# Cibiv/NextGenMap

Measured on AMD Instinct MI355X. Metric: mapped reads/sec + SW Gcells/sec, 150bp vs GRCh38, at 1/2/4/8 MI355X, higher is better.
Workload: dtype int32

## Files before the change

### include/ngm_pipeline.h

```cpp
#ifndef NGM_PIPELINE_H
#define NGM_PIPELINE_H

#include <stddef.h>
#include <stdint.h>

#ifdef __cplusplus
extern "C" {
#endif

typedef struct ngm_ref ngm_ref;
typedef struct ngm_mapper ngm_mapper;

typedef struct ngm_ref_params {
	int kmer;
	int kmer_skip;
	int bin_size;
} ngm_ref_params;

const char *ngm_pipeline_last_error(void);

ngm_ref *ngm_ref_create(int device, const ngm_ref_params *p, int n_contigs, const char *const *names,
		const uint8_t *const *seqs, const uint64_t *lens);
ngm_ref *ngm_ref_create_from_fasta(int device, const ngm_ref_params *p, const char *path);
ngm_ref *ngm_ref_create_from_cache(int device, const ngm_ref_params *params, const char *fasta_path);
// ... 150 lines not shown
int ngm_coverage_finish(ngm_coverage *c);
long long ngm_coverage_next(ngm_coverage *c, void *out, size_t out_cap);
int ngm_coverage_stats(const ngm_coverage *c, uint64_t counts[4], float ms[4]);
int ngm_mapper_set_coverage(ngm_mapper *m, ngm_coverage *c);

typedef struct ngm_snp ngm_snp;
typedef struct ngm_snp_params {
	int device;
	int n_ref;
	const uint32_t *ref_len;
	const char *const *ref_name;
	const char *const *ref_seq;
	uint32_t min_cov;
	double min_frac;
	int min_qual;
	const char *min_frac_text;
	size_t scan_chunk;
} ngm_snp_params;
ngm_snp *ngm_snp_create(const ngm_snp_params *p);
ngm_snp *ngm_snp_create_for_ref(const ngm_ref *r, const ngm_snp_params *p);
void ngm_snp_destroy(ngm_snp *s);
int ngm_snp_add(ngm_snp *s, const int32_t *ref_id, const int32_t *pos0, const uint32_t *cigar_off , const char *cigar_text,
                const uint32_t *seq_off , const char *seq_text, const char *qual_text, size_t n);
int ngm_snp_finish(ngm_snp *s);
long long ngm_snp_next(ngm_snp *s, void *out, size_t out_cap);
int ngm_snp_stats(const ngm_snp *s, uint64_t counts[5], float ms[4]);
int ngm_mapper_set_snp(ngm_mapper *m, ngm_snp *s);

void *ngm_host_alloc(size_t bytes);
void ngm_host_free(void *p);

int ngm_host_pin_to_device_node(int device);

int ngm_mapper_set_reference_score_buffer(ngm_mapper *m, int entries);
int ngm_mapper_lost_pairs(ngm_mapper *m, uint64_t *out);
int ngm_mapper_set_reference_cs_batch(ngm_mapper *m, int reads);

int ngm_mapper_path_counters(ngm_mapper *m, uint64_t out[8]);

int ngm_mapper_order_table_reads(ngm_mapper *m, uint64_t *out);

int ngm_debug_pair_walk(uint32_t cnt_a, int len_a, uint32_t cnt_b, int len_b, const uint32_t *loc, const uint32_t *sv, const float *score, const uint32_t *rank,
		float cutoff, int min_insert, int max_insert, uint32_t *out_a, uint32_t *out_b, int *mq_a, int *mq_b, uint64_t cap, float *combo_score, int *combo_dist, int *combo_a, int *combo_b,
		uint64_t *n_combo);

int ngm_debug_pair_eval(uint64_t n, const float *pair_score, const int *dist, const int *ia, const int *ib, int avg, int out_all[6], int out_kept[6]);

int ngm_debug_select_top1(int device, int n_reads, const uint32_t *base, const uint32_t *count, uint64_t n_cand, const float *scores, const uint32_t *loc,
		const uint32_t *strand_votes, uint32_t *winner, int32_t *mapq, int32_t *n_best, float *best_score);

int ngm_debug_align_finish(void *engine , int mode, int n, const char *const *ref, const char *const *qry, void *out ,
		uint64_t *n_fallback);

int ngm_debug_expand_pairs(int device, int n_reads, const uint32_t *base, const uint32_t *count, uint64_t n_cand, uint32_t *out);

int ngm_debug_pair_select(int device, int n_pairs, const uint32_t *base, const uint32_t *count, uint64_t n_cand, const float *scores, const uint32_t *loc,
		const uint16_t *read_len, int min_insert, int max_insert, float cutoff, int32_t *info, int32_t *mapq, int32_t *n_best, uint32_t counts[4], void *entries, void *tops);

int ngm_mapper_heavy_counters(ngm_mapper *m, uint64_t out[4]);

int ngm_mapper_search_turn_counters(ngm_mapper *m, uint64_t out[3]);

int ngm_mapper_cs_counters(ngm_mapper *m, uint64_t out[3]);

typedef struct ngm_stats_comm ngm_stats_comm;
int ngm_stats_unique_id(char hex[257]);
ngm_stats_comm *ngm_stats_comm_create(int device, int rank, int world, const char *hex);
int ngm_stats_allreduce(ngm_stats_comm *c, int64_t v[8]);
void ngm_stats_comm_destroy(ngm_stats_comm *c);
int ngm_mapper_last_pair_stats(ngm_mapper *m, uint64_t out[3]);

int ngm_mapper_last_kernel_ms(ngm_mapper *m, float ms[8]);
float ngm_mapper_last_order_replay_ms(ngm_mapper *m);

int ngm_mapper_set_argos(ngm_mapper *m, float min_score);
long long ngm_mapper_map_argos(ngm_mapper *m, int n, const char *reads, const char *names, size_t names_bytes, const ngm_sam_read *meta,
		char *out, size_t out_cap, uint64_t stats[3], float *kernel_ms);
int ngm_argos_prolog(const ngm_ref *ref, uint64_t total_reads, char *out, size_t cap);
int ngm_mapper_argos_counters(ngm_mapper *m, uint64_t out[4]);
int ngm_mapper_argos_path_counters(ngm_mapper *m, uint64_t out[2]);
int ngm_debug_argos_order(uint32_t n, const float *score, const uint32_t *rank, float min_score, int read_len, int match_bonus, uint32_t *order, uint32_t out[3]);

#ifdef __cplusplus
}
#endif
#endif
```

### nextgenmap_amd/csrc/affine_device.h

```cpp
#pragma once

#include <hip/hip_runtime.h>
#include <stdint.h>

#include "sw_device.h"

namespace ngm {

struct AffConst {
	int tM;
	int tZ;
	int open;
	int ext;
	int vopen;
	int vext;
};

constexpr int kAffNeg = -(1 << 28);
__host__ __device__ constexpr int aff_dir_words(int CP) { return (CP + 3) / 4; }

enum { kTDiag = 1, kTHori = 2, kTVert = 4, kTHoriOpen = 8, kTVertOpen = 16, kTMaxH = 32, kTMaxV = 64 };

__device__ __forceinline__ uint2 aff_row_table(int rc, const AffConst &K) {
	uint32_t b[8];
// ... 108 lines not shown
					tr = none ? 0u : tr;
					dw[d >> 2] |= tr << (8 * (d & 3));
				}
				const int key = ((sc - fl) << 8) | (255 - d);
				if (!ENDFREE) {
					if (key > rowkey) { rowkey = key; rowflags = ((ev == sc) ? 1 : 0) | ((eh == sc) ? 2 : 0); }
				}
				if (ENDFREE && ALIGN) ehq[d >> 5] |= (eh == sc) ? (1u << (d & 31)) : 0u;
				S[d] = sc;
				Ev[d] = ev;
				leftS = sc;
				leftEh = eh;
			}
			if (ALIGN && i < q) {
#pragma unroll
				for (int w = 0; w < DW; ++w) dout[((size_t) i * DW + w) * kSlots] = dw[w];
			}
			if (!ENDFREE) {
				const int rs = rowkey >> 8, rd_ = 255 - (rowkey & 255), rh = i + 1 + rd_;
				if (i < lenV && (rs > best || (rs == best && rs > 0 && rh < bh))) { best = rs; bh = rh; bv = i + 1; bflags = rowflags; }
			} else if (i + 1 == lenV) {
				const int dlim = lenH - lenV;
				const int kv = -fl;
#pragma unroll
				for (int d = 0; d < CP; ++d) {
					const int v = S[d] + kv;
					if (d <= dlim && v > best) {
						best = v; bh = lenV + d; bv = lenV;
						bflags = ((Ev[d] == S[d]) ? 1 : 0) | ((ALIGN && ((ehq[d >> 5] >> (d & 31)) & 1u)) ? 2 : 0);
					}
				}
			}
			fl += K.tZ;
		}
#pragma unroll
		for (int r = 0; r + 2 < NRG; ++r) RG[r] = RG[r + 2];
		RG[NRG - 2] = fx & 0x0F0F0F0Fu;
		RG[NRG - 1] = (fx >> 4) & 0x0F0F0F0Fu;
	}

	if (pair < n) {
		if (lenV < 1 || lenH < 1) { best = 0; bh = bv = 0; bflags = 0; }
		if (!ALIGN) {
			scores[pair] = (float) best;
		} else {
			int32_t *rec = records + (size_t) pair * 8;
			rec[0] = 0; rec[1] = 0; rec[2] = 0; rec[3] = bflags; rec[4] = 0; rec[5] = best; rec[6] = bh; rec[7] = bv;
		}
	}
}

constexpr int kAffNeg16 = -20000;

template <int CP, bool ENDFREE>
__global__ __launch_bounds__(256) void sw_affine_score_pk_kernel(const uint32_t *__restrict__ packed, const uint16_t *__restrict__ lens,
		const uint16_t *__restrict__ blk_rows, float *__restrict__ scores, int n, int n_blocks, int RW, AffConst K) {
	__shared__ uint2 s_tab[8];
	if (threadIdx.x < 8) s_tab[threadIdx.x] = aff_row_table(threadIdx.x, K);
	__syncthreads();
	const int lane = threadIdx.x & 63;
	const int blkA = 2 * (blockIdx.x * 4 + (threadIdx.x >> 6));
	if (blkA >= n_blocks) return;
	const bool hasB = blkA + 1 < n_blocks;
	const int blkB = hasB ? blkA + 1 : blkA;
	constexpr int NRG = sel_regs(CP);
	const int FW = RW + NRG / 2;
	const uint32_t *rdA = packed + (size_t) blkA * (RW + FW) * kSlots + lane, *rdB = packed + (size_t) blkB * (RW + FW) * kSlots + lane;
	const uint32_t *fdA = rdA + (size_t) RW * kSlots, *fdB = rdB + (size_t) RW * kSlots;
	const int pairA = blkA * kSlots + lane, pairB = blkB * kSlots + lane;
	const int lenVA = (pairA < n) ? (int) lens[pairA] : 0, lenVB = (pairB < n) ? (int) lens[pairB] : 0;
	const int rows = max(__builtin_amdgcn_readfirstlane((int) blk_rows[blkA]), __builtin_amdgcn_readfirstlane((int) blk_rows[blkB]));
	const int ngroups = (rows + 7) >> 3;

	auto window_len = [&](const uint32_t *fd) {
		int len = FW * 8;
		for (int m = FW - 1; m >= 0; --m) {
			const uint32_t x = fd[(size_t) m * kSlots];
			const uint32_t lo = x & 0x0F0F0F0Fu, hi = (x >> 4) & 0x0F0F0F0Fu;
#pragma unroll
			for (int j = 7; j >= 0; --j) {
				const uint32_t cls = (j < 4) ? (lo >> (8 * j)) & 15u : (hi >> (8 * (j - 4))) & 15u;
				if (cls == 6u) len = m * 8 + j;
			}
		}
		return len;
	};
	const int lenHA = ENDFREE ? window_len(fdA) : FW * 8, lenHB = ENDFREE ? window_len(fdB) : FW * 8;

	v2s S[CP], Ev[CP];
#pragma unroll
	for (int d = 0; d < CP; ++d) { S[d] = pk_splat(0); Ev[d] = pk_splat(ENDFREE ? kAffNeg16 : 0); }
	uint32_t RGA[NRG], RGB[NRG];
#pragma unroll
	for (int r = 0; r < NRG / 2; ++r) {
		const uint32_t xa = fdA[(size_t) r * kSlots], xb = fdB[(size_t) r * kSlots];
		RGA[2 * r] = xa & 0x0F0F0F0Fu; RGA[2 * r + 1] = (xa >> 4) & 0x0F0F0F0Fu;
		RGB[2 * r] = xb & 0x0F0F0F0Fu; RGB[2 * r + 1] = (xb >> 4) & 0x0F0F0F0Fu;
	}
	int fl = K.tZ;
	v2s best2 = pk_splat(0);
	int bestA = kAffNeg, bestB = kAffNeg;
	const v2s ext2 = pk_splat(K.ext), open2 = pk_splat(K.open), vext2 = pk_splat(K.vext), vopen2 = pk_splat(K.vopen);
	const v2s neg2 = pk_splat(kAffNeg16), one2 = pk_splat(1), zero2 = pk_splat(0);
	uint32_t rnA = (ngroups > 0) ? rdA[0] : 0x66666666u, rnB = (ngroups > 0) ? rdB[0] : 0x66666666u;

	for (int g = 0; g < ngroups; ++g) {
		const uint32_t rxA = rnA, rxB = rnB;
		rnA = (g + 1 < ngroups) ? rdA[(size_t) (g + 1) * kSlots] : 0x66666666u;
		rnB = (g + 1 < ngroups) ? rdB[(size_t) (g + 1) * kSlots] : 0x66666666u;
		const uint32_t fxA = fdA[(size_t) (g + NRG / 2) * kSlots], fxB = fdB[(size_t) (g + NRG / 2) * kSlots];
		const uint32_t rsA[2] = {rxA & 0x0F0F0F0Fu, (rxA >> 4) & 0x0F0F0F0Fu}, rsB[2] = {rxB & 0x0F0F0F0Fu, (rxB >> 4) & 0x0F0F0F0Fu};
#pragma unroll
		for (int s = 0; s < 8; ++s) {
			const int i = g * 8 + s;
			uint32_t rcA = (rsA[s >> 2] >> (8 * (s & 3))) & 0xFFu, rcB = (rsB[s >> 2] >> (8 * (s & 3))) & 0xFFu;
			rcA = (i < lenVA) ? rcA : 6u;
			rcB = (i < lenVB) ? rcB : 6u;
			const uint2 TA = s_tab[rcA], TB = s_tab[rcB];
			uint32_t PA[NRG], PB[NRG];
#pragma unroll
			for (int r = 0; r < NRG; ++r) {
				const bool used = (s + CP - 1) / 4 >= r && s / 4 <= r;
				PA[r] = used ? __builtin_amdgcn_perm(TA.y, TA.x, RGA[r]) : 0u;
				PB[r] = used ? __builtin_amdgcn_perm(TB.y, TB.x, RGB[r]) : 0u;
			}
			const v2s fl2 = pk_splat(fl);
			v2s leftS = neg2, leftEh = neg2;
			v2s rowmax = fl2;
#pragma unroll
			for (int d = 0; d < CP; ++d) {
				const int bi = s + d, kb = bi & 3;
				const uint32_t sel = 0x0C000C00u | (uint32_t) kb | ((uint32_t) (4 + kb) << 16);
				const v2s t = __builtin_bit_cast(v2s, __builtin_amdgcn_perm(PB[bi >> 2], PA[bi >> 2], sel));
				const v2s dg = S[d] + t;
				v2s eh = (d == 0) ? neg2 : pk_max(leftEh + ext2, leftS + open2);
				v2s ev = (d < CP - 1) ? pk_max(Ev[d + 1] + vext2, S[d + 1] + vopen2) : neg2;
				v2s sc = pk_max(pk_max(ev, eh), dg);
				if (!ENDFREE) {
					sc = pk_max(sc, fl2);
					rowmax = pk_max(rowmax, sc);
				}
				S[d] = sc;
				Ev[d] = ev;
				leftS = sc;
				leftEh = eh;
			}
			if (!ENDFREE) {
				best2 = pk_max(best2, rowmax - fl2);
			} else if (i + 1 == lenVA || i + 1 == lenVB) {
				const int kv = -fl;
				if (i + 1 == lenVA) {
					const int dlim = lenHA - lenVA;
#pragma unroll
					for (int d = 0; d < CP; ++d) { const int v = (int) S[d].x + kv; if (d <= dlim && v > bestA) bestA = v; }
				}
				if (i + 1 == lenVB) {
					const int dlim = lenHB - lenVB;
#pragma unroll
					for (int d = 0; d < CP; ++d) { const int v = (int) S[d].y + kv; if (d <= dlim && v > bestB) bestB = v; }
				}
			}
			fl += K.tZ;
		}
#pragma unroll
		for (int r = 0; r + 2 < NRG; ++r) { RGA[r] = RGA[r + 2]; RGB[r] = RGB[r + 2]; }
		RGA[NRG - 2] = fxA & 0x0F0F0F0Fu; RGA[NRG - 1] = (fxA >> 4) & 0x0F0F0F0Fu;
		RGB[NRG - 2] = fxB & 0x0F0F0F0Fu; RGB[NRG - 1] = (fxB >> 4) & 0x0F0F0F0Fu;
	}
	if (!ENDFREE) { bestA = best2.x; bestB = best2.y; }
	if (pairA < n) { if (lenVA < 1 || lenHA < 1) bestA = 0; scores[pairA] = (float) bestA; }
	if (hasB && pairB < n) { if (lenVB < 1 || lenHB < 1) bestB = 0; scores[pairB] = (float) bestB; }
}

template <int CP>
__global__ __launch_bounds__(256) void sw_affine_score_pk_split_kernel(const uint32_t *__restrict__ packed, const uint16_t *__restrict__ lens,
		const uint16_t *__restrict__ blk_rows, float *__restrict__ scores, int n, int n_blocks, int RW, AffConst K) {
	__shared__ uint2 s_tab[8];
	if (threadIdx.x < 8) s_tab[threadIdx.x] = aff_row_table(threadIdx.x, K);
	__syncthreads();
	constexpr int CL = ((CP + 1) / 2 + 6) / 8 * 8 + 1;
	constexpr int CR = CP - CL;
	static_assert(CR >= 1 && CR <= CL, "band too narrow to split");
	constexpr int NRG = sel_regs(CL);
	constexpr int WOFF = (CL - 1) / 8;
	const int lane = threadIdx.x & 63;
	const bool isR = (lane & 1) != 0;
	const int unit = blockIdx.x * 4 + (threadIdx.x >> 6);
	const int blkA = 2 * (unit >> 1);
	if (blkA >= n_blocks) return;
	const bool hasB = blkA + 1 < n_blocks;
	const int blkB = hasB ? blkA + 1 : blkA;
	const int slot = (lane >> 1) + 32 * (unit & 1);
	const int FW = RW + sel_regs(CP) / 2;
	const uint32_t *rdA = packed + (size_t) blkA * (RW + FW) * kSlots + slot, *rdB = packed + (size_t) blkB * (RW + FW) * kSlots + slot;
	const uint32_t *fdA = rdA + (size_t) RW * kSlots, *fdB = rdB + (size_t) RW * kSlots;
	const int pairA = blkA * kSlots + slot, pairB = blkB * kSlots + slot;
	const int lenVA = (pairA < n) ? (int) lens[pairA] : 0, lenVB = (pairB < n) ? (int) lens[pairB] : 0;
	const int rows = max(__builtin_amdgcn_readfirstlane((int) blk_rows[blkA]), __builtin_amdgcn_readfirstlane((int) blk_rows[blkB]));
	const int ngroups = (rows + 7) >> 3, ngroups2 = (rows + 1 + 7) >> 3;
	const int woff = isR ? WOFF : 0;
	auto swap2 = [](v2s x) -> v2s { return __builtin_bit_cast(v2s, __builtin_amdgcn_update_dpp(0, __builtin_bit_cast(int, x), 0xB1, 0xf, 0xf, false)); };

	v2s S[CL], Ev[CL];
#pragma unroll
	for (int d = 0; d < CL; ++d) { S[d] = pk_splat(0); Ev[d] = pk_splat(0); }
	uint32_t RGA[NRG], RGB[NRG];
#pragma unroll
	for (int r = 0; r < NRG / 2; ++r) {
		const int w = min(r + woff, FW - 1);
		const uint32_t xa = fdA[(size_t) w * kSlots], xb = fdB[(size_t) w * kSlots];
		RGA[2 * r] = xa & 0x0F0F0F0Fu; RGA[2 * r + 1] = (xa >> 4) & 0x0F0F0F0Fu;
		RGB[2 * r] = xb & 0x0F0F0F0Fu; RGB[2 * r + 1] = (xb >> 4) & 0x0F0F0F0Fu;
	}
	int fl = K.tZ;
	const int rz = isR ? K.tZ : 0;
	v2s best2 = pk_splat(0);
	const v2s ext2 = pk_splat(K.ext), open2 = pk_splat(K.open), vext2 = pk_splat(K.vext), vopen2 = pk_splat(K.vopen);
	const v2s neg2 = pk_splat(kAffNeg16), zero2 = pk_splat(0);
	v2s saveS = neg2, saveEh = neg2;
	uint32_t prevA = 6u, prevB = 6u;
	uint32_t rnA = (ngroups > 0) ? rdA[0] : 0x66666666u, rnB = (ngroups > 0) ? rdB[0] : 0x66666666u;

// ... 21 lines not shown
				PB[r] = used ? __builtin_amdgcn_perm(TB.y, TB.x, RGB[r]) : 0u;
			}
			const v2s fl2 = pk_splat(fl - rz);
			const v2s gotS = swap2(saveS), gotEh = swap2(saveEh);
			v2s leftS = isR ? gotS : neg2, leftEh = isR ? gotEh : neg2;
			v2s nxS = neg2, nxEv = neg2;
			v2s rowmax = fl2;
#pragma unroll
			for (int d = 0; d < CL; ++d) {
				const int bi = s + d, kb = bi & 3;
				const uint32_t sel = 0x0C000C00u | (uint32_t) kb | ((uint32_t) (4 + kb) << 16);
				const v2s t = __builtin_bit_cast(v2s, __builtin_amdgcn_perm(PB[bi >> 2], PA[bi >> 2], sel));
				const v2s dg = S[d] + t;
				const v2s eh = pk_max(leftEh + ext2, leftS + open2);
				v2s ev = (d < CL - 1) ? pk_max(Ev[d + 1] + vext2, S[d + 1] + vopen2) : pk_max(nxEv + vext2, nxS + vopen2);
				v2s sc = pk_max(pk_max(pk_max(ev, eh), dg), fl2);
				if (d >= CR) { sc = isR ? neg2 : sc; ev = isR ? neg2 : ev; }
				rowmax = pk_max(rowmax, sc);
				S[d] = sc;
				Ev[d] = ev;
				leftS = sc;
				leftEh = eh;
				if (d == 0) {
					v2s xS = swap2(sc), xEv = swap2(ev);
					if (s == 0 && g == 0) { xS = zero2; xEv = zero2; }
					nxS = isR ? neg2 : xS; nxEv = isR ? neg2 : xEv;
				}
				if (d == CL - 1) { saveS = sc; saveEh = eh; }
			}
			best2 = pk_max(best2, rowmax - fl2);
			if (s == 0 && g == 0) {
#pragma unroll
				for (int d = 0; d < CL; ++d) { S[d] = isR ? zero2 : S[d]; Ev[d] = isR ? zero2 : Ev[d]; }
				best2 = isR ? zero2 : best2;
			}
			fl += K.tZ;
		}
#pragma unroll
		for (int r = 0; r + 2 < NRG; ++r) { RGA[r] = RGA[r + 2]; RGB[r] = RGB[r + 2]; }
		RGA[NRG - 2] = fxA & 0x0F0F0F0Fu; RGA[NRG - 1] = (fxA >> 4) & 0x0F0F0F0Fu;
		RGB[NRG - 2] = fxB & 0x0F0F0F0Fu; RGB[NRG - 1] = (fxB >> 4) & 0x0F0F0F0Fu;
	}
	best2 = pk_max(best2, swap2(best2));
	if (isR) return;
	int bestA = best2.x, bestB = best2.y;
	if (pairA < n) { if (lenVA < 1) bestA = 0; scores[pairA] = (float) bestA; }
	if (hasB && pairB < n) { if (lenVB < 1) bestB = 0; scores[pairB] = (float) bestB; }
}

__host__ __device__ constexpr int aff_nib_words(int CP) { return (CP + 7) / 8; }

template <int CP, bool WINDOW>
__global__ __launch_bounds__(256) void sw_affine_align_pk_kernel(const uint32_t *__restrict__ packed, const uint16_t *__restrict__ lens,
		const uint16_t *__restrict__ blk_rows, uint32_t *__restrict__ dirs, int32_t *__restrict__ records, int n, int n_blocks, int RW, int q, AffConst K) {
	static_assert(WINDOW ? CP <= 128 : CP <= 32, "the row key keeps the band column in 7 / 5 bits");
	__shared__ uint2 s_tab[8];
	if (threadIdx.x < 8) s_tab[threadIdx.x] = aff_row_table(threadIdx.x, K);
	__syncthreads();
	const int lane = threadIdx.x & 63;
	const int blkA = 2 * (blockIdx.x * 4 + (threadIdx.x >> 6));
	if (blkA >= n_blocks) return;
	const bool hasB = blkA + 1 < n_blocks;
	const int blkB = hasB ? blkA + 1 : blkA;
	constexpr int NRG = sel_regs(CP);
	constexpr int DW = aff_nib_words(CP);
	const int FW = RW + NRG / 2;
	const uint32_t *rdA = packed + (size_t) blkA * (RW + FW) * kSlots + lane, *rdB = packed + (size_t) blkB * (RW + FW) * kSlots + lane;
	const uint32_t *fdA = rdA + (size_t) RW * kSlots, *fdB = rdB + (size_t) RW * kSlots;
	uint32_t *doutA = dirs + (size_t) blkA * q * DW * kSlots + lane, *doutB = dirs + (size_t) blkB * q * DW * kSlots + lane;
	const int pairA = blkA * kSlots + lane, pairB = blkB * kSlots + lane;
	const int lenVA = (pairA < n) ? (int) lens[pairA] : 0, lenVB = (pairB < n) ? (int) lens[pairB] : 0;
	const int rows = max(__builtin_amdgcn_readfirstlane((int) blk_rows[blkA]), __builtin_amdgcn_readfirstlane((int) blk_rows[blkB]));
	const int ngroups = (rows + 7) >> 3;

	v2s S[CP], Ev[CP];
#pragma unroll
	for (int d = 0; d < CP; ++d) { S[d] = pk_splat(0); Ev[d] = pk_splat(0); }
	uint32_t RGA[NRG], RGB[NRG];
#pragma unroll
	for (int r = 0; r < NRG / 2; ++r) {
		const uint32_t xa = fdA[(size_t) r * kSlots], xb = fdB[(size_t) r * kSlots];
		RGA[2 * r] = xa & 0x0F0F0F0Fu; RGA[2 * r + 1] = (xa >> 4) & 0x0F0F0F0Fu;
		RGB[2 * r] = xb & 0x0F0F0F0Fu; RGB[2 * r + 1] = (xb >> 4) & 0x0F0F0F0Fu;
	}
	int fl = K.tZ;
	int bestA = 0, bhA = 0, bvA = 0, bestB = 0, bhB = 0, bvB = 0;
	const v2s ext2 = pk_splat(K.ext), open2 = pk_splat(K.open), vext2 = pk_splat(K.vext), vopen2 = pk_splat(K.vopen);
	const v2s neg2 = pk_splat(kAffNeg16), one2 = pk_splat(1), zero2 = pk_splat(0), two2 = pk_splat(2), four2 = pk_splat(4), k32 = pk_splat(WINDOW ? 128 : 32);
	const v2s win_lo2 = pk_splat(K.tZ + 1), win_max2 = pk_splat(63);
	v2s prevmax2 = pk_splat(0);
	uint32_t rnA = (ngroups > 0) ? rdA[0] : 0x66666666u, rnB = (ngroups > 0) ? rdB[0] : 0x66666666u;

	for (int g = 0; g < ngroups; ++g) {
		const uint32_t rxA = rnA, rxB = rnB;
		rnA = (g + 1 < ngroups) ? rdA[(size_t) (g + 1) * kSlots] : 0x66666666u;
		rnB = (g + 1 < ngroups) ? rdB[(size_t) (g + 1) * kSlots] : 0x66666666u;
		const uint32_t fxA = fdA[(size_t) (g + NRG / 2) * kSlots], fxB = fdB[(size_t) (g + NRG / 2) * kSlots];
		const uint32_t rsA[2] = {rxA & 0x0F0F0F0Fu, (rxA >> 4) & 0x0F0F0F0Fu}, rsB[2] = {rxB & 0x0F0F0F0Fu, (rxB >> 4) & 0x0F0F0F0Fu};
#pragma unroll
		for (int s = 0; s < 8; ++s) {
			const int i = g * 8 + s;
			uint32_t rcA = (rsA[s >> 2] >> (8 * (s & 3))) & 0xFFu, rcB = (rsB[s >> 2] >> (8 * (s & 3))) & 0xFFu;
			rcA = (i < lenVA) ? rcA : 6u;
			rcB = (i < lenVB) ? rcB : 6u;
			const uint2 TA = s_tab[rcA], TB = s_tab[rcB];
			uint32_t PA[NRG], PB[NRG];
#pragma unroll
			for (int r = 0; r < NRG; ++r) {
// ... 147 lines not shown
```

### nextgenmap_amd/csrc/cigar_device.h

```cpp
#pragma once

#include <hip/hip_runtime.h>
#include <stdint.h>

#include "sw_device.h"
#include "affine_device.h"

namespace ngm {

struct CigarDevOut {
	uint32_t cig_off, md_off;
	uint16_t cig_len, md_len;
	int32_t position_offset, qstart, qend, nm;
	float identity, score_token;
	int32_t flags;
};

__device__ __forceinline__ uint32_t packed_class(const uint32_t *base, int m_base, int j) {
	const uint32_t w = base[(size_t) (m_base + (j >> 3)) * kSlots];
	const int b = j & 7;
	return (b < 4) ? (w >> (8 * b)) & 15u : (w >> (8 * (b - 4) + 4)) & 15u;
}
__device__ __forceinline__ char class_to_char(uint32_t c) {
	switch (c) { case 0: return 'A'; case 1: return 'C'; case 2: return 'G'; case 3: return 'T'; case 4: return 'x'; case 5: return 'N'; default: return 0; }
// ... 108 lines not shown
				if (m_len > 0) { co += dev_put_num(cg + co, m_len); cg[co++] = 'M'; }
				if (trail > 0) {
					if (hard_clip == 1) { co += dev_put_num(cg + co, trail); cg[co++] = 'H'; }
					else if (silent_clip != 1) { co += dev_put_num(cg + co, trail); cg[co++] = 'S'; }
					o.qend = trail;
				}
			}
			o.identity = (float) match * 1.0f / (float) total;
			o.nm = mismatch;
			o.score_token = (float) read_i;
			o.position_offset = ref0;
			o.flags = ((fits && !odd_symbol) ? 1 : 0) | 2;
		}
	}
	}
	o.cig_len = (uint16_t) co; o.md_len = (uint16_t) mo;
	const uint32_t need = (live && (o.flags & 1)) ? (uint32_t) (co + mo) : 0u;
	uint32_t incl = need;
	const int lane = threadIdx.x & 63, wv = threadIdx.x >> 6;
#pragma unroll
	for (int d = 1; d < 64; d <<= 1) { const uint32_t t = __shfl_up(incl, d); if (lane >= d) incl += t; }
	if (lane == 63) s_wave[wv] = incl;
	__syncthreads();
	uint32_t before = incl - need, total = 0;
#pragma unroll
	for (int w2 = 0; w2 < 4; ++w2) { if (w2 < wv) before += s_wave[w2]; total += s_wave[w2]; }
	if (threadIdx.x == 0) s_base = total ? atomicAdd(cursor, (unsigned long long) total) : 0ull;
	__syncthreads();
	const unsigned long long base = s_base;
	if (!live) return;
	if (need) {
		if (base + total > capacity) o.flags &= ~1;
		else {
			const unsigned long long off = base + before;
			o.cig_off = (uint32_t) off; o.md_off = (uint32_t) off + o.cig_len;
			for (int t = 0; t < co; ++t) bytes[off + t] = cg[t];
			for (int t = 0; t < mo; ++t) bytes[off + co + t] = mdp[t];
		}
	}
	out[j] = o;
}

constexpr int kFinishRows = 8;

__device__ __forceinline__ uint32_t finish_sel8(uint32_t w0, uint32_t w1, uint32_t w2, uint32_t w3, uint32_t w4, uint32_t w5, uint32_t w6, uint32_t w7, int k) {
	const uint32_t a0 = (k & 1) ? w1 : w0, a1 = (k & 1) ? w3 : w2, a2 = (k & 1) ? w5 : w4, a3 = (k & 1) ? w7 : w6;
	const uint32_t b0 = (k & 2) ? a1 : a0, b1 = (k & 2) ? a3 : a2;
	return (k & 4) ? b1 : b0;
}

template <bool NIBBLES>
__global__ __launch_bounds__(256) void affine_finish_kernel(int n, const uint32_t *__restrict__ dirs, const int32_t *__restrict__ records,
		const uint32_t *__restrict__ packed, const uint16_t *__restrict__ lens, int q, int CP, int RW, int FW, CigarDevOut *__restrict__ out,
		char *__restrict__ bytes, unsigned long long capacity, unsigned long long *__restrict__ counters) {
	__shared__ char s_rows[256 * kCigarRow];
	__shared__ uint32_t s_wave[4];
	__shared__ unsigned long long s_base;
	const int j = blockIdx.x * blockDim.x + threadIdx.x;
	const bool live = j < n;
	const int lane = threadIdx.x & 63, wv = threadIdx.x >> 6;
	constexpr int lim = kCigarRow - 16;
	constexpr int WS = NIBBLES ? 3 : 2;
	const int DW = NIBBLES ? aff_nib_words(CP) : aff_dir_words(CP);
	char *row = s_rows + (size_t) threadIdx.x * kCigarRow;
	int pos = kCigarRow;
	auto put_back = [&](int num, char tag) {
		row[--pos] = tag;
		unsigned u = (unsigned) num;
		do { row[--pos] = (char) ('0' + u % 10u); u /= 10u; } while (u);
	};
	bool fits = true;
	int h = 0, v = 0, flags = 0, len_v = 0;
	if (live) {
		const int32_t *rec = records + (size_t) j * 8;
		flags = rec[3]; h = rec[6]; v = rec[7];
		len_v = (int) lens[j];
	}
	const int qend = len_v - v;
	if (live && qend > 0) put_back(qend, 'S');
	const int trail = kCigarRow - pos;
	const uint32_t *dp = dirs + (size_t) (j >> 6) * q * DW * kSlots + lane;
	const uint32_t *pk = packed + (size_t) (j >> 6) * (RW + FW) * kSlots + lane;
	int cur = -1, curlen = 0, total = 0, n_match = 0, n_mis = 0;
	bool done = !live, first = true, in_v = false, in_h = false;
	auto flush = [&]() {
		if (cur < 0) return;
		if (kCigarRow - pos - trail > lim) { fits = false; done = true; return; }
		put_back(curlen, cur == 1 ? 'M' : cur == 2 ? 'I' : 'D');
		total += cur == 1 ? curlen : 1;
	};
	auto emit = [&](int op) {
		if (op == cur) { ++curlen; return; }
		flush();
		cur = op; curlen = 1;
	};
	int gtop = (v - 1) >> 3;
#pragma unroll
	for (int s = 1; s < 64; s <<= 1) gtop = max(gtop, __shfl_xor(gtop, s));
	for (int g = gtop; g >= 0; --g) {
		const int r0 = g * kFinishRows;
		const bool act = !done && v - 1 >= r0;
		const int d0 = h - v;
		const int wi = min(max(d0 >> WS, 0), DW - 1);
		const int f0 = min(max((r0 + d0) >> 3, 0), FW - 1);
		uint32_t W[kFinishRows];
#pragma unroll
		for (int k = 0; k < kFinishRows; ++k) W[k] = (act && r0 + k <= v - 1) ? dp[((size_t) (r0 + k) * DW + wi) * kSlots] : 0u;
		const uint32_t rdw = act ? pk[(size_t) g * kSlots] : 0u;
		const uint32_t fw0 = act ? pk[(size_t) (RW + f0) * kSlots] : 0u;
		const uint32_t fw1 = (act && f0 + 1 < FW) ? pk[(size_t) (RW + f0 + 1) * kSlots] : 0u;
// ... 44 lines not shown
					emit(1);
					const int jr = (v - 1) & 7, jf = (h - 1) & 7, fi = (h - 1) >> 3;
					const uint32_t fx = (fi == f0) ? fw0 : (fi == f0 + 1) ? fw1 : pk[(size_t) (RW + fi) * kSlots];
					const uint32_t rc = (rdw >> (4 * ((jr & 3) * 2 + (jr >> 2)))) & 15u, fc = (fx >> (4 * ((jf & 3) * 2 + (jf >> 2)))) & 15u;
					if (rc == fc && rc <= 5u && rc != 4u) ++n_match; else ++n_mis;
					--h; --v;
					continue;
				}
				if ((tv & kTMaxV) && (tv & kTVert)) in_v = true;
				else if ((tv & kTMaxV) && (tv & kTVertOpen)) { emit(2); --v; continue; }
				else if ((tv & kTMaxH) && (tv & kTHori)) in_h = true;
				else if ((tv & kTMaxH) && (tv & kTHoriOpen)) { emit(3); --h; continue; }
				else { done = true; break; }
			}
			if (in_v) { in_v = (!(tv & kTVertOpen) || (tv & kTVert)) && v != 1; emit(2); --v; }
			else { in_h = (!(tv & kTHoriOpen) || (tv & kTHori)) && h != 1; emit(3); --h; }
		}
	}
	int co = 0;
	if (live) {
		if (fits) flush();
		int lead = 0;
		if (v > 0) { lead = 2; for (int t = v; t >= 10; t /= 10) ++lead; }
		if (kCigarRow - pos - trail + lead > lim) fits = false;
		if (fits && v > 0) put_back(v, 'S');
		co = kCigarRow - pos;
	}
	constexpr int mo = 3;
	const uint32_t need = (live && fits) ? (uint32_t) (co + mo) : 0u;
	uint32_t incl = need;
#pragma unroll
	for (int d = 1; d < 64; d <<= 1) { const uint32_t t = __shfl_up(incl, d); if (lane >= d) incl += t; }
	if (lane == 63) s_wave[wv] = incl;
	__syncthreads();
	uint32_t before = incl - need, total_b = 0;
#pragma unroll
	for (int w2 = 0; w2 < 4; ++w2) { if (w2 < wv) before += s_wave[w2]; total_b += s_wave[w2]; }
	if (threadIdx.x == 0) s_base = total_b ? atomicAdd(&counters[0], (unsigned long long) total_b) : 0ull;
	__syncthreads();
	const unsigned long long base = s_base;
	if (!live) return;
	uint32_t cig_off = 0;
	if (need) {
		if (base + total_b > capacity) fits = false;
		else {
			const unsigned long long off = base + before;
			cig_off = (uint32_t) off;
			const char *cg = row + pos;
			for (int t = 0; t < co; ++t) bytes[off + t] = cg[t];
			for (int t = 0; t < mo; ++t) bytes[off + co + t] = '!';
		}
	}
	if (!fits) atomicAdd(&counters[1], 1ull);
	CigarDevOut *o = out + j;
	o->cig_off = cig_off; o->md_off = fits ? cig_off + (uint32_t) co : 0u;
	o->cig_len = (uint16_t) co; o->md_len = (uint16_t) mo;
	o->position_offset = h; o->qstart = v; o->qend = qend; o->nm = n_mis;
	o->identity = (float) n_match * 1.0f / (float) total;
	o->score_token = 0.f;
	o->flags = (fits ? 1 : 0) | 2;
}

}
```

### nextgenmap_amd/csrc/engine_internal.h

```cpp
#pragma once

#include <algorithm>

#include <hip/hip_runtime.h>

#include <cstdint>
#include <string>

#include "../../include/ngm_hip.h"
#include "sw_device.h"
#include "affine_device.h"
#include "cigar_device.h"
#include "jit.h"

namespace ngm {
template <typename T>
struct DevBuf {
	T *p = nullptr;
	size_t cap = 0;
	int reserve(size_t n) {
		if (n <= cap) return 0;
		if (p) (void) hipFree(p);
		p = nullptr;
		cap = 0;
// ... 6 lines not shown
	void release() { if (p) (void) hipFree(p); p = nullptr; cap = 0; }
};

template <typename T>
struct PinnedBuf {
	T *p = nullptr;
	size_t cap = 0;
	int reserve(size_t n) {
		if (n <= cap) return 0;
		if (p) (void) hipHostFree(p);
		p = nullptr;
		cap = 0;
		const size_t want = n + std::min<size_t>(n / 8, ((size_t) 64 << 20) / sizeof(T));
		if (hipHostMalloc(&p, want * sizeof(T), hipHostMallocDefault) == hipSuccess) { cap = want; return 0; }
		if (hipHostMalloc(&p, n * sizeof(T), hipHostMallocDefault) != hipSuccess) return -1;
		cap = n;
		return 0;
	}
	void release() { if (p) (void) hipHostFree(p); p = nullptr; cap = 0; }
};

}

struct ngm_hip_ctx {
	int device = 0;
	ngm_hip_params prm{};
	ngm::SwConst K{};
	ngm::AffConst KA{};
	const ngm::JitKernels *jit = nullptr;
	int q = 0, c = 0, rl = 0, RW = 0, FW = 0;
	int max_batch = 0;
	hipStream_t stream = nullptr;
	ngm::DevBuf<uint32_t> packed;
	ngm::DevBuf<uint16_t> lens, blk_rows;
	ngm::DevBuf<uint8_t> d_ref, d_qry, d_pair_dir;
	const uint8_t *pair_dir = nullptr;
	ngm::DevBuf<float> d_scores;
	ngm::DevBuf<uint32_t> dirs;
	ngm::DevBuf<int32_t> d_records;
	ngm::DevBuf<uint16_t> d_runs;
	ngm::PinnedBuf<uint8_t> h_ref, h_qry;
	ngm::PinnedBuf<float> h_scores;
	ngm::PinnedBuf<int32_t> h_records;
	ngm::PinnedBuf<uint16_t> h_runs;
	bool profiling = false;
	hipEvent_t ev[4] = {nullptr, nullptr, nullptr, nullptr};
	bool ev_valid[3] = {false, false, false};
	bool trace_nibbles = false;
	std::string error;
};

namespace ngm {
int engine_reserve(ngm_hip_ctx *ctx, int n);
int engine_score_packed(ngm_hip_ctx *ctx, int mode, int n, float *d_scores, hipStream_t st);
struct AlignFinish {
	CigarDevOut *out;
	char *bytes;
	unsigned long long capacity;
	unsigned long long *counters;
};
int engine_align_packed(ngm_hip_ctx *ctx, int mode, int n, int32_t *d_records, uint16_t *d_runs, int run_stride, hipStream_t st, const AlignFinish *fin = nullptr);
int engine_affine_traceback_packed(ngm_hip_ctx *ctx, int n, int32_t *d_records, uint16_t *d_runs, int run_stride, hipStream_t st);
}
```

### nextgenmap_amd/csrc/gather_device.h

```cpp
#pragma once

#include <hip/hip_runtime.h>
#include <stdint.h>

#include "sw_device.h"

namespace ngm {

struct WindowGeom {
	uint64_t concat_len;
	int buffer_len;
	int half_corridor;
};

__device__ __forceinline__ uint32_t window_class(const uint32_t *__restrict__ genome, const WindowGeom &G, uint64_t offset, int j) {
	uint64_t len = (uint64_t) G.buffer_len - 2;
	if (offset >= G.concat_len) return 5u;
	uint64_t end = 0;
	if (offset + len > G.concat_len) { end = offset + len - G.concat_len; len -= end; }
	const uint64_t emitted = ((offset & 1) ? 1 : 0) + 2 * ((len + 1) / 2);
	const uint64_t jj = (uint64_t) j;
	if (jj < emitted) {
		if ((len & 1) && jj == emitted - 1) return 4u;
		const uint64_t pos = offset + jj;
		return (genome[pos >> 3] >> (4 * (pos & 7))) & 15u;
	}
	if (jj < emitted + end) return 4u;
	return 6u;
}

__device__ __forceinline__ uint32_t read_class_fwd(uint32_t ch) {
	uint32_t k = 5;
	k = (ch == 'A') ? 0u : k;
	k = (ch == 'C') ? 1u : k;
	k = (ch == 'G') ? 2u : k;
	k = (ch == 'T') ? 3u : k;
	k = (ch == 0) ? 6u : k;
	return k;
}

__global__ __launch_bounds__(256) void gather_pairs_kernel(const uint8_t *__restrict__ reads, const uint16_t *__restrict__ read_len,
		int q, const uint32_t *__restrict__ genome, WindowGeom G, const uint32_t *__restrict__ pair_read,
		const uint32_t *__restrict__ pair_loc, const uint32_t *__restrict__ pair_sv, int n_pairs, int RW, int FW,
		uint32_t *__restrict__ out, uint16_t *__restrict__ lens, uint16_t *__restrict__ blk_rows, int alt_dir = 0) {
	__shared__ int s_rows;
	const int tid = threadIdx.x;
	const int blk = blockIdx.x;
	const int slot = tid & 63, part = tid >> 6;
	const int pair = blk * kSlots + slot;
	if (tid == 0) s_rows = 0;
	__syncthreads();
	uint32_t *ob = out + (size_t) blk * (RW + FW) * kSlots + slot;
	const bool live = pair < n_pairs;
	const uint32_t ridx = live ? pair_read[pair] : 0u;
	const bool rev = live ? (pair_sv[pair] & 1u) : false;
	const int L = live ? (int) read_len[ridx] : 0;
	const uint8_t *rp = reads + (size_t) ridx * q;
	uint32_t dbit = 0;
	if (alt_dir && live) { const bool second = alt_dir == 2 && (ridx & 1u); dbit = (rev ? !second : second) ? 8u : 0u; }
	struct __attribute__((packed, aligned(1))) U32 { uint32_t v; };
	for (int m = part; m < RW; m += 4) {
		uint32_t k[8];
		const int first = rev ? L - 8 * m - 8 : 8 * m;
		uint32_t lo4 = 0, hi4 = 0;
		const bool fast = live && first >= 0 && first + 8 <= q;
		if (fast) { lo4 = reinterpret_cast<const U32 *>(rp + first)->v; hi4 = reinterpret_cast<const U32 *>(rp + first + 4)->v; }
#pragma unroll
		for (int j = 0; j < 8; ++j) {
			const int i = m * 8 + j;
			uint32_t c = 6u;
			if (live && i < L) {
				uint32_t ch;
				if (fast) { const int b = rev ? 7 - j : j; ch = ((b < 4 ? lo4 : hi4) >> (8 * (b & 3))) & 0xFFu; }
				else ch = rev ? rp[L - 1 - i] : rp[i];
				c = read_class_fwd(ch);
				if (rev) c = (c <= 3u) ? 3u - c : c;
			}
			k[j] = c | dbit;
		}
		ob[(size_t) m * kSlots] = pack8(k);
	}
	const uint64_t offset = live ? (uint64_t) pair_loc[pair] - (uint64_t) G.half_corridor : 0;
	uint64_t plain = 0;
	if (live && offset < G.concat_len) {
		uint64_t len = (uint64_t) G.buffer_len - 2, end = 0;
		if (offset + len > G.concat_len) { end = offset + len - G.concat_len; len -= end; }
		const uint64_t emitted = ((offset & 1) ? 1 : 0) + 2 * ((len + 1) / 2);
		plain = (len & 1) ? emitted - 1 : emitted;
	}
	for (int m = part; m < FW; m += 4) {
		uint32_t word;
		if ((uint64_t) (m * 8 + 8) <= plain) {
			const uint64_t pos = offset + (uint64_t) m * 8;
			const uint32_t w0 = genome[pos >> 3], w1 = genome[(pos >> 3) + 1];
			const uint32_t r = 4u * (uint32_t) (pos & 7);
			const uint32_t v = r ? ((w0 >> r) | (w1 << (32u - r))) : w0;
			uint32_t lo = v & 0xFFFFu, hi = v >> 16;
			lo = (lo | (lo << 8)) & 0x00FF00FFu; lo = (lo | (lo << 4)) & 0x0F0F0F0Fu;
			hi = (hi | (hi << 8)) & 0x00FF00FFu; hi = (hi | (hi << 4)) & 0x0F0F0F0Fu;
			word = lo | (hi << 4);
// ... 194 lines not shown
```

### nextgenmap_amd/csrc/mapper.cpp

```cpp
#define NGM_SAM_KERNELS
#include "mapper_internal.h"
#define NGM_COV_BATCH_KERNELS
#include "coverage_device.h"
#include "snp_device.h"
#include <rocprim/rocprim.hpp>
#include "align_device.h"
#include "gather_device.h"

using ngm::DevGuard;
using ngm::GpuStage;
using ngm::run_cs;
using ngm::cs_host_arrays;
using ngm::candidate_order;
using ngm::candidate_order_wait;

namespace ngm {
StageLock g_stage_lock[16][2];
std::atomic<long long> g_stage_hold_us[3], g_stage_wait_us[3];
}
using ngm::g_stage_hold_us;
using ngm::g_stage_wait_us;

namespace {

int upload_reads(ngm_mapper *m, int n, const char *reads) {
	const size_t bytes = (size_t) n * m->prm.qry_max_len;
	if (m->d_reads.reserve(bytes)) { ngm::pipeline_set_error("out of device memory (reads)"); return -12; }
	MAP_HIP_TRY(hipMemcpyAsync(m->d_reads.p, reads, bytes, hipMemcpyHostToDevice, m->st));
	return 0;
}

std::atomic<int> g_live_mappers{0};
template <typename F>
void parallel_for(int n, F f, int min_grain = 0) {
	ngm::ThreadPool::instance().parallel_for(n, f, min_grain > 0 ? min_grain : 2048);
}

char class_char(uint8_t c) {
	static const char t[8] = {'A', 'C', 'G', 'T', 'x', 'N', 0, 0};
	return t[c & 7];
}

void host_window(const ngm_ref *r, uint64_t offset, int buffer_len, int want, char *out) {
	const uint64_t concat_len = r->n_bases - 1;
	uint64_t len = (uint64_t) buffer_len - 2;
	if (offset >= concat_len) { memset(out, 'N', want); return; }
	uint64_t end = 0;
	if (offset + len > concat_len) { end = offset + len - concat_len; len -= end; }
	const uint64_t emitted = ((offset & 1) ? 1 : 0) + 2 * ((len + 1) / 2);
	for (int j = 0; j < want; ++j) {
		const uint64_t jj = (uint64_t) j;
		char ch;
		if (jj < emitted) ch = ((len & 1) && jj == emitted - 1) ? 'x' : class_char(r->host_cls[offset + jj]);
		else if (jj < emitted + end) ch = 'x';
		else ch = 0;
		out[j] = ch;
	}
}

}

namespace ngm {
int score_candidates(ngm_mapper *m, int n, uint64_t np, int alt_dir) {
	const ngm_ref *r = m->ref;
	ngm_hip_ctx *eng = m->eng;
	const int q = m->prm.qry_max_len, c = m->prm.corridor;
	hipLaunchKernelGGL(ngm::expand_pairs_kernel, dim3((n + 255) / 256), dim3(256), 0, m->st, n, m->d_cand_base.p, m->d_cand_count.p, m->d_pair_read.p);
	const int nb = (int) ((np + ngm::kSlots - 1) / ngm::kSlots);
	ngm::WindowGeom Gs{r->n_bases - 1, ((q + c) | 1) + 1, c >> 1};
	hipLaunchKernelGGL(ngm::gather_pairs_kernel, dim3(nb), dim3(256), 0, m->st, m->d_reads.p, m->d_read_len.p, q, r->d_genome, Gs,
			m->d_pair_read.p, m->d_out_loc.p, m->d_out_sv.p, (int) np, eng->RW, eng->FW, eng->packed.p, eng->lens.p, eng->blk_rows.p, alt_dir);
	MAP_HIP_TRY(hipGetLastError());
	MAP_HIP_TRY(hipEventRecord(m->ev[2], m->st));
	if (int rc = ngm::engine_score_packed(eng, m->prm.mode, (int) np, m->d_scores.p, m->st)) { ngm::pipeline_set_error("%s", ngm_hip_last_error(eng)); return rc; }
	MAP_HIP_TRY(hipEventRecord(m->ev[3], m->st));
	return 0;
}
}

extern "C" {

int ngm_ref_decode(const ngm_ref *r, uint64_t offset, int buffer_len, char *out) {
	DevGuard g(r->device);
	if (buffer_len < 2) return -22;
	const uint64_t concat_len = r->n_bases - 1;
	if (offset >= concat_len) { memset(out, 0, buffer_len); return 0; }
	const int q = 8, c = buffer_len;
	const int RW = ngm::read_words(q), FW = (q + c + 7) / 8 + 1;
	uint32_t *d_out; uint16_t *d_lens, *d_rows, *d_rl; uint8_t *d_reads; uint32_t *d_pr, *d_pl, *d_ps;
	MAP_HIP_TRY(hipMalloc(&d_out, (size_t) (RW + FW) * 64 * 4)); MAP_HIP_TRY(hipMalloc(&d_lens, 128)); MAP_HIP_TRY(hipMalloc(&d_rows, 8));
	MAP_HIP_TRY(hipMalloc(&d_rl, 8)); MAP_HIP_TRY(hipMalloc(&d_reads, q)); MAP_HIP_TRY(hipMalloc(&d_pr, 4)); MAP_HIP_TRY(hipMalloc(&d_pl, 4)); MAP_HIP_TRY(hipMalloc(&d_ps, 4));
	MAP_HIP_TRY(hipMemset(d_rl, 0, 8)); MAP_HIP_TRY(hipMemset(d_reads, 0, q)); MAP_HIP_TRY(hipMemset(d_pr, 0, 4)); MAP_HIP_TRY(hipMemset(d_ps, 0, 4));
	const uint32_t loc = (uint32_t) offset;
	MAP_HIP_TRY(hipMemcpy(d_pl, &loc, 4, hipMemcpyHostToDevice));
	ngm::WindowGeom G{concat_len, buffer_len, 0};
	hipLaunchKernelGGL(ngm::gather_pairs_kernel, dim3(1), dim3(256), 0, 0, d_reads, d_rl, q, r->d_genome, G, d_pr, d_pl, d_ps, 1, RW, FW, d_out, d_lens, d_rows);
	MAP_HIP_TRY(hipGetLastError());
	std::vector<uint32_t> h((size_t) (RW + FW) * 64);
	MAP_HIP_TRY(hipMemcpy(h.data(), d_out, h.size() * 4, hipMemcpyDeviceToHost));
	for (int j = 0; j < buffer_len; ++j) {
		const uint32_t w = h[(size_t) (RW + j / 8) * 64];
		const int b = j & 7;
		const uint32_t cls = (b < 4) ? (w >> (8 * b)) & 15u : (w >> (8 * (b - 4) + 4)) & 15u;
		out[j] = class_char((uint8_t) cls);
	}
	(void) hipFree(d_out); (void) hipFree(d_lens); (void) hipFree(d_rows); (void) hipFree(d_rl); (void) hipFree(d_reads); (void) hipFree(d_pr); (void) hipFree(d_pl); (void) hipFree(d_ps);
	return 1;
}

ngm_mapper *ngm_mapper_create(const ngm_ref *ref, const ngm_mapper_params *p) {
	if (!ref || !p) { ngm::pipeline_set_error("ngm_mapper_create: null argument"); return nullptr; }
	DevGuard g(ref->device);
	if (p->qry_max_len < ref->prm.kmer + 1 || p->qry_max_len > 1024) { ngm::pipeline_set_error("ngm_mapper_create: qry_max_len %d out of range", p->qry_max_len); return nullptr; }
	ngm_hip_params ep{};
	ep.abi_version = NGM_HIP_ABI_VERSION;
	ep.qry_max_len = p->qry_max_len; ep.corridor = p->corridor;
	ep.match_bonus = p->match_bonus; ep.mismatch_penalty = p->mismatch_penalty; ep.gap_read_penalty = p->gap_read_penalty; ep.gap_ref_penalty = p->gap_ref_penalty;
	ep.variant = p->variant; ep.hard_clip = p->hard_clip; ep.silent_clip = p->silent_clip; ep.max_batch = 0;
	ep.personality = p->personality; ep.gap_extend_penalty = p->gap_extend_penalty;
	if (p->bs_mapping) {
		if (ref->prm.kmer_skip != 0) { ngm::pipeline_set_error("ngm_mapper_create: bisulfite mapping needs a reference index built with kmer_skip 0 (src/PrefixTable.cpp:199-207)"); return nullptr; }
		if (p->mode != 0) { ngm::pipeline_set_error("ngm_mapper_create: '--bs-mapping' and '--end-to-end' can't be used at the same time"); return nullptr; }
		ep.alt_scoring = ep.alt_cigar = NGM_ALT_BISULFITE; ep.match_bonus_tt = p->match_bonus_tt; ep.match_bonus_tc = p->match_bonus_tc;
	}
	if (p->slam_seq) {
		if (p->bs_mapping) { ngm::pipeline_set_error("ngm_mapper_create: '--bs-mapping' and '--slam-seq' can't be used at the same time!"); return nullptr; }
		if (p->personality != NGM_PERSONALITY_LINEAR) { ngm::pipeline_set_error("ngm_mapper_create: '--slam-seq' needs the default (linear-gap) personality: EndToEndAffine produces no per-base records (Align::ExtendedData)"); return nullptr; }
		ep.alt_cigar = NGM_ALT_SLAMSEQ;
		if (p->slam_seq & 2) { ep.alt_scoring = NGM_ALT_SLAMSEQ; ep.match_bonus_tt = p->match_bonus_tt; ep.match_bonus_tc = p->match_bonus_tc; }
	}
	ngm_hip_ctx *eng = ngm_hip_create(ref->device, &ep);
	if (!eng) { ngm::pipeline_set_error("%s", ngm_hip_last_error(nullptr)); return nullptr; }
	ngm_mapper *m = new ngm_mapper();
	++g_live_mappers;
	m->ref = ref; m->prm = *p; m->eng = eng; m->st = eng->stream;
	{
		int lo = 0, hi = 0;
		(void) hipDeviceGetStreamPriorityRange(&lo, &hi);
		if (hipStreamCreateWithPriority(&m->st_hi, hipStreamNonBlocking, hi) != hipSuccess) m->st_hi = nullptr;
	}
	m->max_kfreq = p->max_kfreq > 0 ? p->max_kfreq : ref->auto_max_kfreq;
	for (auto &e : m->ev) (void) hipEventCreate(&e);
	for (auto &e : m->cev) (void) hipEventCreate(&e);
	for (auto &e : m->oev) (void) hipEventCreate(&e);
	if (const char *e = getenv("NGM_HIP_CS_EAGER_ARRAYS")) m->cs_eager_arrays = atoi(e) != 0;
	if (ngm::cs_configure(m, p) != 0) { ngm_mapper_destroy(m); return nullptr; }
	return m;
}

void ngm_mapper_destroy(ngm_mapper *m) {
	if (!m) return;
	if (--g_live_mappers == 0 && getenv("NGM_HIP_HOST_TIMING"))
		fprintf(stderr, "[ngm-hip] GPU stage lock, ms summed over all mappers: search + score held %.1f (waited %.1f) | align held %.1f (waited %.1f) | SAM text held %.1f (waited %.1f)\n",
				g_stage_hold_us[0] / 1e3, g_stage_wait_us[0] / 1e3, g_stage_hold_us[1] / 1e3, g_stage_wait_us[1] / 1e3, g_stage_hold_us[2] / 1e3, g_stage_wait_us[2] / 1e3);
	DevGuard g(m->ref->device);
	(void) hipStreamSynchronize(m->st);
	ngm_bgzf_destroy(m->bz);
	if (m->st_hi) { (void) hipStreamSynchronize(m->st_hi); (void) hipStreamDestroy(m->st_hi); }
	ngm::cs_release(m);
	ngm::argos_release(m);
	m->d_reads.release(); m->d_scores.release(); m->d_best.release(); m->d_pair_read.release();
	m->d_winner.release(); m->d_a_read.release(); m->d_a_loc.release(); m->d_a_sv.release(); m->d_mapq.release(); m->d_nbest.release();
	m->d_records.release(); m->d_runs.release(); m->d_runs_c.release();
	m->d_pair_info.release(); m->p_pair_info.release(); m->d_sam_contig_start.release();
	m->d_pair_out.release(); m->d_pair_top.release(); m->d_pair_tied_n.release(); m->d_pair_list.release(); m->p_pair_out.release(); m->p_pair_top.release(); m->p_pair_tied_n.release();
	m->d_sam_contig_names.release(); m->d_sam_rg.release(); m->d_sam_names.release(); m->d_sam_text.release(); m->d_sam_contig_off.release(); m->d_sam_len.release(); m->d_sam_off.release();
	m->d_sam_quals.release(); m->d_sam_polya.release(); m->d_sam_meta.release(); m->d_sam_refs.release(); m->d_sam_hits.release(); m->p_sam_hits.release(); m->p_sam_refs.release(); m->p_sam_extra.release();
	for (auto &e : m->ev) if (e) (void) hipEventDestroy(e);
	for (auto &e : m->cev) if (e) (void) hipEventDestroy(e);
	for (auto &e : m->oev) if (e) (void) hipEventDestroy(e);
	m->p_winner.release(); m->p_loc.release(); m->p_sv.release(); m->p_mapq.release(); m->p_nbest.release(); m->p_rec.release();
	m->p_best.release(); m->p_scores.release(); m->p_runs.release();
	m->d_str.release(); m->d_cigout.release(); m->p_cigout.release(); m->p_str.release();
	ngm_hip_destroy(m->eng);
	delete m;
}

int ngm_mapper_cs(ngm_mapper *m, int n, const char *reads, uint32_t *cand_offsets, float *max_votes) {
	if (!m || n < 0) return -22;
	DevGuard g(m->ref->device);
	if (n == 0) { cand_offsets[0] = 0; m->n_reads = 0; m->n_cand = 0; return 0; }
	if (int r = upload_reads(m, n, reads)) return r;
	m->cs_paired = false;
	if (int r = run_cs(m, n)) return r;
	if (int r = cs_host_arrays(m)) return r;
	uint32_t acc = 0;
	for (int i = 0; i < n; ++i) { cand_offsets[i] = acc; acc += m->h_count[i]; max_votes[i] = m->h_maxv[i]; }
	cand_offsets[n] = acc;
	return 0;
}

int ngm_mapper_cs_fetch(ngm_mapper *m, uint64_t *loc, uint8_t *strand, float *votes) {
	if (!m) return -22;
	DevGuard g(m->ref->device);
	if (m->n_cand == 0) return 0;
	std::vector<uint32_t> hl(m->n_cand), hs(m->n_cand);
	MAP_HIP_TRY(hipMemcpy(hl.data(), m->d_out_loc.p, m->n_cand * 4, hipMemcpyDeviceToHost));
	MAP_HIP_TRY(hipMemcpy(hs.data(), m->d_out_sv.p, m->n_cand * 4, hipMemcpyDeviceToHost));
	size_t w = 0;
	std::vector<uint32_t> order;
	for (int i = 0; i < m->n_reads; ++i) {
		const uint32_t b = m->h_base[i], c = m->h_count[i];
		order.resize(c);
		std::iota(order.begin(), order.end(), b);
		std::sort(order.begin(), order.end(), [&](uint32_t x, uint32_t y) {
			const uint64_t kx = ((uint64_t) hl[x] << 1) | (hs[x] & 1), ky = ((uint64_t) hl[y] << 1) | (hs[y] & 1);
			return kx < ky;
		});
		for (uint32_t j : order) { loc[w] = hl[j]; strand[w] = (uint8_t) (hs[j] & 1); votes[w] = (float) (hs[j] >> 1); ++w; }
	}
	return 0;
}

struct SamCall { const char *quals; const char *names; size_t names_bytes; const ngm::SamMeta *meta; const uint16_t *polya; char *out; size_t out_cap; uint64_t *stats; long long text_bytes; float kernel_ms; };
static int map_impl(ngm_mapper *m, int n, const char *reads, const void *d_reads_ext, ngm_hit *hits, char *cigars, char *mds, bool paired, SamCall *sam = nullptr);

// ... 355 lines not shown
			m->pair_dist_sum = m->ps->dist_sum; m->pair_dist_count = m->ps->dist_count; m->scores_so_far = m->ps->scores_so_far; m->reads_so_far = m->ps->reads_so_far;
			held = true;
		}
		void release() {
			if (!active || released) return;
			acquire();
			{ std::lock_guard<std::mutex> lk(m->ps->mu); m->ps->dist_sum = m->pair_dist_sum; m->ps->dist_count = m->pair_dist_count; m->ps->scores_so_far = m->scores_so_far; m->ps->reads_so_far = m->reads_so_far; m->ps->next = m->batch_seq + 1; }
			m->ps->cv.notify_all();
			released = true;
		}
		bool released = false;
		~PairTurn() { release(); }
	} pair_turn{m, paired && m->ps != nullptr};
	if (n < 0) return -22;
	if (paired && m->prm.topn > 1) { ngm::pipeline_set_error("Paired end mode with topn > 1 not yet supported."); return -38; }
	if (paired && (n & 1)) { ngm::pipeline_set_error("paired-end batches need an even number of reads"); return -22; }
	if (n == 0) return 0;
	const ngm_ref *r = m->ref;
	DevGuard g(r->device);
	ngm_hip_ctx *eng = m->eng;
	const int q = m->prm.qry_max_len, c = m->prm.corridor, mode = m->prm.mode;
	const size_t str_stride = (size_t) 4 * std::max(1, q);
	for (auto &x : m->ms) x = 0.f;
	m->order_ms = 0.f;

	ngm::DevBuf<uint8_t> own = m->d_reads;
	struct Restore { ngm_mapper *m; ngm::DevBuf<uint8_t> own; bool on; ~Restore() { if (on) m->d_reads = own; } } restore{m, own, d_reads_ext != nullptr};
	if (d_reads_ext) { m->d_reads.p = (uint8_t *) d_reads_ext; m->d_reads.cap = (size_t) n * q; }
	const bool host_timing = getenv("NGM_HIP_HOST_TIMING") != nullptr;
	const int alt_cigar = m->prm.bs_mapping ? NGM_ALT_BISULFITE : (m->prm.slam_seq ? NGM_ALT_SLAMSEQ : NGM_ALT_NONE);
	const int alt_dir = alt_cigar ? (paired ? 2 : 1) : 0;
	auto now = [] { return std::chrono::steady_clock::now(); };
	auto tp0 = now();
	double t_stage[6] = {0, 0, 0, 0, 0, 0};
	auto lap = [&](int k) { auto t = now(); t_stage[k] += std::chrono::duration<double, std::milli>(t - tp0).count(); tp0 = t; };
	MAP_HIP_TRY(hipEventRecord(m->ev[0], m->st));
	if (!d_reads_ext) if (int rc = upload_reads(m, n, reads)) return rc;
	if (sam) {
		if (!m->sam_ready || (!paired) != (!m->sam_opt.paired) || m->prm.topn > 1) { ngm::pipeline_set_error("ngm_mapper_map_sam: call ngm_mapper_set_sam_options first (single alignments only; paired as configured)"); return -22; }
		if ((unsigned long long) n * (unsigned long long) (2 * q + 1024) + sam->names_bytes >= 0xFFFFFFFFull) { ngm::pipeline_set_error("ngm_mapper_map_sam: the text of %d reads may exceed the 32-bit offsets of a batch: use smaller batches", n); return -75; }
		if (m->d_sam_quals.reserve((size_t) n * q) || m->d_sam_names.reserve(sam->names_bytes + 16) || m->d_sam_meta.reserve(n) || m->p_sam_hits.reserve(n) || m->p_sam_refs.reserve(n) ||
				m->d_sam_hits.reserve(n) || m->d_sam_refs.reserve(n)) { ngm::pipeline_set_error("out of memory (SAM stage)"); return -12; }
		MAP_HIP_TRY(hipMemcpyAsync(m->d_sam_quals.p, sam->quals, (size_t) n * q, hipMemcpyHostToDevice, m->st));
		if (sam->names_bytes) MAP_HIP_TRY(hipMemcpyAsync(m->d_sam_names.p, sam->names, sam->names_bytes, hipMemcpyHostToDevice, m->st));
		MAP_HIP_TRY(hipMemcpyAsync(m->d_sam_meta.p, sam->meta, (size_t) n * sizeof(ngm::SamMeta), hipMemcpyHostToDevice, m->st));
		if (sam->polya && n > 0) {
			if (m->d_sam_polya.reserve((size_t) n)) { ngm::pipeline_set_error("out of memory (SAM stage)"); return -12; }
			MAP_HIP_TRY(hipMemcpyAsync(m->d_sam_polya.p, sam->polya, (size_t) n * sizeof(uint16_t), hipMemcpyHostToDevice, m->st));
		}
		hits = m->p_sam_hits.p;
	}
	if (m->p_winner.reserve(n) || m->p_mapq.reserve(n) || m->p_nbest.reserve(n) || m->p_best.reserve(n)) { ngm::pipeline_set_error("out of pinned host memory"); return -12; }
	if (m->d_winner.reserve(n) || m->d_mapq.reserve(n) || m->d_nbest.reserve(n) || m->d_best.reserve(n)) { ngm::pipeline_set_error("out of device memory (score stage)"); return -12; }
	uint64_t regrown = 0;
	auto reserve_for_candidates = [&](uint64_t cnt, bool device, bool count) -> int {
		auto grow = [&](auto &buf, size_t want) { if (count && buf.cap < want) ++regrown; return buf.reserve(want); };
		if (grow(m->p_loc, cnt + 1) || grow(m->p_sv, cnt + 1) || (paired && grow(m->p_scores, cnt + 1))) { ngm::pipeline_set_error("out of pinned host memory"); return -12; }
		if (!device) return 0;
		if (grow(m->d_pair_read, cnt) || grow(m->d_scores, cnt)) { ngm::pipeline_set_error("out of device memory (score stage)"); return -12; }
		const size_t had = eng->packed.cap + eng->lens.cap + eng->blk_rows.cap;
		if (int rc = ngm::engine_reserve(eng, (int) cnt)) { ngm::pipeline_set_error("%s", ngm_hip_last_error(eng)); return rc; }
		if (count && eng->packed.cap + eng->lens.cap + eng->blk_rows.cap != had) ++regrown;
		return 0;
	};
	if (int rc = reserve_for_candidates(std::min<uint64_t>(std::max<uint64_t>((uint64_t) n, m->np_seen_max + m->np_seen_max / 4), 0x7FFFFFFFull), true, false)) return rc;
	uint32_t *h_winner = m->p_winner.p, *h_loc = nullptr, *h_sv = nullptr;
	int32_t *h_mapq = m->p_mapq.p, *h_nbest = m->p_nbest.p;
	float *h_best = m->p_best.p, *h_scores = nullptr;
	std::vector<int> pair_flags(n, 0);
	auto reference_buffer_walk = [&]() {
		uint64_t tot = m->scores_so_far, at = m->reads_so_far;
		const uint64_t rb = m->ref_cs_batch > 0 ? (uint64_t) m->ref_cs_batch : 0;
		const uint64_t sb = m->ref_score_buffer > 0 ? (uint64_t) m->ref_score_buffer : 0;
		uint64_t next_flush = rb ? (at + rb - 1) / rb * rb : ~0ull;
		uint64_t fill = sb ? tot % sb : 0;
		for (int pi = 0; pi < n / 2; ++pi, at += 2) {
			while (at > next_flush) next_flush += rb;
			if (at == next_flush) { tot = 0; fill = 0; next_flush += rb; }
			const uint32_t c1 = m->h_count[2 * pi], c2 = m->h_count[2 * pi + 1];
			tot += (uint64_t) c1 + c2;
			if (!sb) continue;
			fill += c1;
			const bool full_at_first_mate = c1 > 0 && fill % sb == 0;
			fill = (fill + c2) % sb;
			if (full_at_first_mate && c2 == 0) {
				++m->lost_pairs;
				pair_flags[2 * pi] = pair_flags[2 * pi + 1] = NGM_PAIR_LOST;
				h_winner[2 * pi] = h_winner[2 * pi + 1] = 0xFFFFFFFFu;
			}
		}
		m->scores_so_far = tot; m->reads_so_far = at;
	};
	GpuStage stage_cs(m, 0, false);
	m->cs_paired = paired;
	m->turn_dbg[2] = 0;
	if (int rc = run_cs(m, n, &stage_cs, true)) return rc;
	MAP_HIP_TRY(hipEventRecord(m->ev[1], m->st));
	const uint64_t np = m->n_cand;
	m->np_seen_max = std::max(m->np_seen_max, np);
	lap(0);
	if (const char *dump = getenv("NGM_HIP_DUMP_COUNTS")) {
		if (int rc = cs_host_arrays(m)) return rc;
		if (FILE *f = fopen(dump, "ab")) { fwrite(m->h_count.data(), 4, (size_t) n, f); fclose(f); }
	}

	if (int rc = reserve_for_candidates(np, np > 0, true)) return rc;
	m->turn_dbg[2] = regrown;
	h_loc = m->p_loc.p; h_sv = m->p_sv.p; h_scores = m->p_scores.p;
	if (np == 0) { if (int rc = cs_host_arrays(m)) return rc; for (int i = 0; i < n; ++i) { h_winner[i] = 0xFFFFFFFFu; h_mapq[i] = 0; h_nbest[i] = 0; h_best[i] = 0.f; } }
	if (np > 0) {
		stage_cs.acquire();
		if (int rc = ngm::score_candidates(m, n, np, alt_dir)) return rc;
		hipLaunchKernelGGL(ngm::select_top1_kernel, dim3((n + 255) / 256), dim3(256), 0, m->st, n, m->d_cand_base.p, m->d_cand_count.p,
				m->d_scores.p, m->d_out_loc.p, m->d_out_sv.p, m->d_winner.p, m->d_mapq.p, m->d_nbest.p, m->d_best.p);
		MAP_HIP_TRY(hipGetLastError());
		const bool pe_select = paired && !m->fast_pairing;
		const bool simple_on_gpu = pe_select && m->prm.strata == 0;
		static const bool pair_choice_host = getenv("NGM_HIP_HOST_PAIR_CHOICE") != nullptr, pair_choice_force = getenv("NGM_HIP_GPU_PAIR_CHOICE") != nullptr;
		const bool choice_on_gpu = simple_on_gpu && !pair_choice_host && (pair_choice_force || np >= 3ull * (uint64_t) n);
		if (simple_on_gpu) {
			const size_t npairs = (size_t) n / 2;
			if (m->d_pair_info.reserve(npairs + 1) || m->p_pair_info.reserve(npairs + 1)) { ngm::pipeline_set_error("out of memory (pair selection)"); return -12; }
			if (choice_on_gpu) {
				if (m->d_pair_out.reserve(2 * npairs + 2) || m->d_pair_top.reserve(npairs + 1) || m->d_pair_tied_n.reserve(4) || m->p_pair_tied_n.reserve(4) || m->d_pair_list.reserve(3 * npairs + 2)) {
					ngm::pipeline_set_error("out of memory (pair selection)"); return -12; }
			}
			if (int rc = launch_pair_select(m->st, npairs, m->d_cand_base.p, m->d_cand_count.p, m->d_scores.p, m->d_out_loc.p, m->d_read_len.p, m->prm.min_insert_size, m->prm.max_insert_size,
					m->prm.pair_score_cutoff, m->d_mapq.p, m->d_nbest.p, m->d_pair_info.p, choice_on_gpu, m->d_pair_tied_n.p, m->d_pair_list.p, m->d_pair_out.p, m->d_pair_top.p)) return rc;
			if (choice_on_gpu) {
				MAP_HIP_TRY(hipMemcpyAsync(m->p_pair_tied_n.p, m->d_pair_tied_n.p, 16, hipMemcpyDeviceToHost, m->st));
			}
			MAP_HIP_TRY(hipMemcpyAsync(m->p_pair_info.p, m->d_pair_info.p, (size_t) (n / 2) * 4, hipMemcpyDeviceToHost, m->st));
		}
		MAP_HIP_TRY(hipEventRecord(m->ev[4], m->st));
		MAP_HIP_TRY(hipMemcpyAsync(h_winner, m->d_winner.p, (size_t) n * 4, hipMemcpyDeviceToHost, m->st));
		MAP_HIP_TRY(hipMemcpyAsync(h_mapq, m->d_mapq.p, (size_t) n * 4, hipMemcpyDeviceToHost, m->st));
		MAP_HIP_TRY(hipMemcpyAsync(h_nbest, m->d_nbest.p, (size_t) n * 4, hipMemcpyDeviceToHost, m->st));
		MAP_HIP_TRY(hipMemcpyAsync(h_best, m->d_best.p, (size_t) n * 4, hipMemcpyDeviceToHost, m->st));
		MAP_HIP_TRY(hipMemcpyAsync(h_loc, m->d_out_loc.p, np * 4, hipMemcpyDeviceToHost, m->st));
		MAP_HIP_TRY(hipMemcpyAsync(h_sv, m->d_out_sv.p, np * 4, hipMemcpyDeviceToHost, m->st));
		if (paired) MAP_HIP_TRY(hipMemcpyAsync(h_scores, m->d_scores.p, np * 4, hipMemcpyDeviceToHost, m->st));
		if (int rc = ngm::cs_enqueue_host_arrays(m)) return rc;
		stage_cs.done_after(m->ev[4]);
		MAP_HIP_TRY(hipStreamSynchronize(m->st));
		if (int rc = cs_host_arrays(m)) return rc;
		if (choice_on_gpu) {
			const size_t npairs = (size_t) n / 2;
			const size_t n_small = std::min<size_t>(m->p_pair_tied_n.p[1], npairs), n_large = std::min<size_t>(m->p_pair_tied_n.p[2], npairs), nt = std::min<size_t>(m->p_pair_tied_n.p[0], npairs);
			if (m->p_pair_out.reserve(2 * npairs + 2) || m->p_pair_top.reserve(nt + 1)) { ngm::pipeline_set_error("out of pinned host memory"); return -12; }
			if (n_small) MAP_HIP_TRY(hipMemcpyAsync(m->p_pair_out.p, m->d_pair_out.p, n_small * sizeof(ngm::PairOut), hipMemcpyDeviceToHost, m->st));
			if (n_large) MAP_HIP_TRY(hipMemcpyAsync(m->p_pair_out.p + npairs, m->d_pair_out.p + npairs, n_large * sizeof(ngm::PairOut), hipMemcpyDeviceToHost, m->st));
			if (nt) MAP_HIP_TRY(hipMemcpyAsync(m->p_pair_top.p, m->d_pair_top.p, nt * sizeof(ngm::PairTop), hipMemcpyDeviceToHost, m->st));
			MAP_HIP_TRY(hipStreamSynchronize(m->st));
		}
		lap(1);
		if ((!paired || m->fast_pairing) && m->prm.topn <= 1) {
			std::vector<uint32_t> tied;
			for (int i = 0; i < n; ++i) if (h_nbest[i] != 1 && m->h_count[i] > 1) tied.push_back((uint32_t) i);
			if (!tied.empty()) {
				uint32_t *h_rank = nullptr;
				if (int rc = candidate_order(m, tied, np, &h_rank)) return rc;
				if (m->p_scores.reserve(np + 1)) { ngm::pipeline_set_error("out of pinned host memory"); return -12; }
				h_scores = m->p_scores.p;
				MAP_HIP_TRY(hipMemcpy(h_scores, m->d_scores.p, np * 4, hipMemcpyDeviceToHost));
				for (uint32_t i : tied) {
// ... 274 lines not shown
					int ns = 0;
					if (ntop <= topn || !m->prm.strata) {
						ns = m->prm.strata ? ntop : std::min<int>((int) cnt, topn);
						int mq = 60;
						if (cnt > 1) { const float bs = h_scores[v[0]], s2 = h_scores[v[1]]; mq = (bs > 0 && s2 >= 0) ? (int) ceilf(60.0f * (bs - s2) / bs) : 0; }
						h_mapq[i] = mq;
					} else {
						h_mapq[i] = 0;
					}
					for (int t = 0; t < ns; ++t) tn_pairs[(size_t) i * topn + t] = v[t];
					h_winner[i] = ns > 0 ? v[0] : 0xFFFFFFFFu;
					h_best[i] = h_scores[v[0]];
				}
			});
		}
	}
	stage_cs.done();
	lap(2);
	std::vector<uint32_t> a_read((size_t) n * topn), a_loc((size_t) n * topn), a_sv((size_t) n * topn), a_out((size_t) n * topn), a_pair((size_t) n * topn);
	int na = 0;
	if (topn == 1 || np == 0) {
		const int slices = std::max(1, std::min(256, n / 4096));
		std::vector<int> first(slices + 1, 0);
		parallel_for(slices, [&](int lo, int hi) {
			for (int s2 = lo; s2 < hi; ++s2) {
				const int i0 = (int) ((long long) n * s2 / slices), i1 = (int) ((long long) n * (s2 + 1) / slices);
				int cnt = 0;
				for (int i = i0; i < i1; ++i) cnt += h_winner[i] != 0xFFFFFFFFu;
				first[s2 + 1] = cnt;
			}
		}, 1);
		for (int s2 = 0; s2 < slices; ++s2) first[s2 + 1] += first[s2];
		na = first[slices];
		parallel_for(slices, [&](int lo, int hi) {
			for (int s2 = lo; s2 < hi; ++s2) {
				const int i0 = (int) ((long long) n * s2 / slices), i1 = (int) ((long long) n * (s2 + 1) / slices);
				int at = first[s2];
				for (int i = i0; i < i1; ++i) if (h_winner[i] != 0xFFFFFFFFu) {
					a_read[at] = (uint32_t) i; a_out[at] = (uint32_t) i; a_pair[at] = h_winner[i]; a_loc[at] = h_loc[h_winner[i]]; a_sv[at] = h_sv[h_winner[i]]; ++at;
				}
			}
		}, 1);
	} else {
		for (int i = 0; i < n; ++i) for (int t = 0; t < topn; ++t) {
			const uint32_t w = tn_pairs[(size_t) i * topn + t];
			if (w == 0xFFFFFFFFu) break;
			a_read[na] = i; a_out[na] = (uint32_t) (i * topn + t); a_pair[na] = w; a_loc[na] = h_loc[w]; a_sv[na] = h_sv[w]; ++na;
		}
	}
	const int rs = ngm::run_stride(q, c);
	if (m->p_rec.reserve((size_t) na * 8 + 8)) { ngm::pipeline_set_error("out of pinned host memory"); return -12; }
	int32_t *h_rec = m->p_rec.p;
	uint16_t *h_runs = nullptr;
	const int align_buf_len = (q + c) | 2;
	static const bool dev_strings = !getenv("NGM_HIP_HOST_CIGAR");
	uint64_t str_base = 0;
	GpuStage stage_align(m, 1, false);
	if (na > 0) {
		if (m->d_a_read.reserve(na) || m->d_a_loc.reserve(na) || m->d_a_sv.reserve(na) || m->d_records.reserve((size_t) na * 8) ||
				m->d_runs.reserve((size_t) na * rs)) { ngm::pipeline_set_error("out of device memory (align stage)"); return -12; }
		if (int rc = ngm::engine_reserve(eng, na)) { ngm::pipeline_set_error("%s", ngm_hip_last_error(eng)); return rc; }
		MAP_HIP_TRY(hipMemcpyAsync(m->d_a_read.p, a_read.data(), (size_t) na * 4, hipMemcpyHostToDevice, m->st));
		MAP_HIP_TRY(hipMemcpyAsync(m->d_a_loc.p, a_loc.data(), (size_t) na * 4, hipMemcpyHostToDevice, m->st));
		MAP_HIP_TRY(hipMemcpyAsync(m->d_a_sv.p, a_sv.data(), (size_t) na * 4, hipMemcpyHostToDevice, m->st));
		static const bool tail_split = getenv("NGM_HIP_ALIGN_TAIL_SPLIT") != nullptr;
		const bool affine = m->prm.personality == NGM_PERSONALITY_AFFINE;
		const bool finish = affine && dev_strings && topn == 1 && !tail_split;
		const unsigned long long scap = (unsigned long long) na * 96ull + 4096ull;
		if (dev_strings && (m->d_cigout.reserve(na) || m->d_str.reserve(scap) || m->p_cigout.reserve(na))) { ngm::pipeline_set_error("out of memory (CIGAR strings)"); return -12; }
		if (finish) MAP_HIP_TRY(hipMemsetAsync(m->d_total.p + 8, 0, 16, m->st));
		MAP_HIP_TRY(hipStreamSynchronize(m->st));
		stage_align.acquire();
		MAP_HIP_TRY(hipEventRecord(m->ev[5], m->st));
		ngm::WindowGeom Ga{r->n_bases - 1, align_buf_len, c >> 1};
		hipLaunchKernelGGL(ngm::gather_pairs_kernel, dim3((na + ngm::kSlots - 1) / ngm::kSlots), dim3(256), 0, m->st, m->d_reads.p, m->d_read_len.p, q,
				r->d_genome, Ga, m->d_a_read.p, m->d_a_loc.p, m->d_a_sv.p, na, eng->RW, eng->FW, eng->packed.p, eng->lens.p, eng->blk_rows.p, alt_dir);
		MAP_HIP_TRY(hipGetLastError());
		MAP_HIP_TRY(hipEventRecord(m->ev[6], m->st));
		const bool was_prof = eng->profiling;
		unsigned long long n_runs_total = 0, n_str_total = 0;
		if (finish) {
			unsigned long long ctr[2] = {0, 0};
			const ngm::AlignFinish fin{m->d_cigout.p, m->d_str.p, scap, m->d_total.p + 8};
			eng->profiling = true;
			if (int rc = ngm::engine_align_packed(eng, mode, na, m->d_records.p, m->d_runs.p, rs, m->st, &fin)) { eng->profiling = was_prof; ngm::pipeline_set_error("%s", ngm_hip_last_error(eng)); return rc; }
			eng->profiling = was_prof;
			MAP_HIP_TRY(hipEventRecord(m->ev[7], m->st));
			MAP_HIP_TRY(hipEventRecord(m->ev[8], m->st));
			MAP_HIP_TRY(hipMemcpyAsync(m->p_cigout.p, m->d_cigout.p, (size_t) na * sizeof(ngm::CigarDevOut), hipMemcpyDeviceToHost, m->st));
			MAP_HIP_TRY(hipMemcpyAsync(ctr, m->d_total.p + 8, 16, hipMemcpyDeviceToHost, m->st));
			stage_align.done_after(m->ev[8]);
			MAP_HIP_TRY(hipStreamSynchronize(m->st));
			n_str_total = std::min<unsigned long long>(ctr[0], scap);
			str_base = n_str_total;
			if (m->p_str.reserve(n_str_total + 1)) { ngm::pipeline_set_error("out of pinned host memory"); return -12; }
			if (n_str_total && !sam) MAP_HIP_TRY(hipMemcpy(m->p_str.p, m->d_str.p, n_str_total, hipMemcpyDeviceToHost));
			if (ctr[1]) {
				if (m->d_runs_c.reserve((size_t) na * rs)) { ngm::pipeline_set_error("out of device memory (runs)"); return -12; }
				MAP_HIP_TRY(hipMemsetAsync(m->d_total.p, 0, 8, m->st));
				if (int rc = ngm::engine_affine_traceback_packed(eng, na, m->d_records.p, m->d_runs.p, rs, m->st)) { ngm::pipeline_set_error("%s", ngm_hip_last_error(eng)); return rc; }
				hipLaunchKernelGGL(ngm::compact_runs_kernel, dim3((na + 255) / 256), dim3(256), 0, m->st, na, m->d_records.p, m->d_runs.p, rs,
						m->d_runs_c.p, m->d_total.p);
				MAP_HIP_TRY(hipGetLastError());
				MAP_HIP_TRY(hipMemcpyAsync(h_rec, m->d_records.p, (size_t) na * 8 * 4, hipMemcpyDeviceToHost, m->st));
				MAP_HIP_TRY(hipMemcpyAsync(&n_runs_total, m->d_total.p, 8, hipMemcpyDeviceToHost, m->st));
				MAP_HIP_TRY(hipStreamSynchronize(m->st));
				if (m->p_runs.reserve(n_runs_total + 1)) { ngm::pipeline_set_error("out of pinned host memory"); return -12; }
				h_runs = m->p_runs.p;
				MAP_HIP_TRY(hipMemcpy(h_runs, m->d_runs_c.p, n_runs_total * 2, hipMemcpyDeviceToHost));
			}
		} else {
		eng->profiling = true;
		if (int rc = ngm::engine_align_packed(eng, mode, na, m->d_records.p, m->d_runs.p, rs, m->st)) { eng->profiling = was_prof; ngm::pipeline_set_error("%s", ngm_hip_last_error(eng)); return rc; }
		eng->profiling = was_prof;
		MAP_HIP_TRY(hipEventRecord(m->ev[7], m->st));
		if (m->d_runs_c.reserve((size_t) na * rs)) { ngm::pipeline_set_error("out of device memory (runs)"); return -12; }
		MAP_HIP_TRY(hipMemsetAsync(m->d_total.p, 0, 8, m->st));
		hipLaunchKernelGGL(ngm::compact_runs_kernel, dim3((na + 255) / 256), dim3(256), 0, m->st, na, m->d_records.p, m->d_runs.p, rs,
				m->d_runs_c.p, m->d_total.p);
		MAP_HIP_TRY(hipGetLastError());
		if (!dev_strings) { MAP_HIP_TRY(hipEventRecord(m->ev[8], m->st)); }
		if (dev_strings) {
			MAP_HIP_TRY(hipMemsetAsync(m->d_total.p + 8, 0, 8, m->st));
			if (affine) hipLaunchKernelGGL(ngm::cigar_strings_kernel<true>, dim3((na + 255) / 256), dim3(256), 0, m->st, na, m->d_records.p, m->d_runs_c.p, eng->packed.p, eng->RW, eng->FW,
					m->d_read_len.p, m->d_a_read.p, m->prm.variant == NGM_VARIANT_OCL_CPU ? 1 : 0, m->prm.hard_clip, m->prm.silent_clip, m->d_cigout.p, m->d_str.p, scap,
					(unsigned long long *) (m->d_total.p + 8), 0);
			else hipLaunchKernelGGL(ngm::cigar_strings_kernel<false>, dim3((na + 255) / 256), dim3(256), 0, m->st, na, m->d_records.p, m->d_runs_c.p, eng->packed.p, eng->RW, eng->FW,
					m->d_read_len.p, m->d_a_read.p, m->prm.variant == NGM_VARIANT_OCL_CPU ? 1 : 0, m->prm.hard_clip, m->prm.silent_clip, m->d_cigout.p, m->d_str.p, scap,
					(unsigned long long *) (m->d_total.p + 8), alt_cigar);
			MAP_HIP_TRY(hipGetLastError());
			MAP_HIP_TRY(hipEventRecord(m->ev[8], m->st));
			MAP_HIP_TRY(hipMemcpyAsync(m->p_cigout.p, m->d_cigout.p, (size_t) na * sizeof(ngm::CigarDevOut), hipMemcpyDeviceToHost, m->st));
			MAP_HIP_TRY(hipMemcpyAsync(&n_str_total, m->d_total.p + 8, 8, hipMemcpyDeviceToHost, m->st));
		}
		MAP_HIP_TRY(hipMemcpyAsync(h_rec, m->d_records.p, (size_t) na * 8 * 4, hipMemcpyDeviceToHost, m->st));
		MAP_HIP_TRY(hipMemcpyAsync(&n_runs_total, m->d_total.p, 8, hipMemcpyDeviceToHost, m->st));
		stage_align.done_after(m->ev[8]);
		MAP_HIP_TRY(hipStreamSynchronize(m->st));
		if (m->p_runs.reserve(n_runs_total + 1)) { ngm::pipeline_set_error("out of pinned host memory"); return -12; }
		h_runs = m->p_runs.p;
		MAP_HIP_TRY(hipMemcpy(h_runs, m->d_runs_c.p, n_runs_total * 2, hipMemcpyDeviceToHost));
		if (dev_strings) {
			n_str_total = std::min<unsigned long long>(n_str_total, scap);
			str_base = n_str_total;
			if (m->p_str.reserve(n_str_total + 1)) { ngm::pipeline_set_error("out of pinned host memory"); return -12; }
			if (n_str_total && !sam) MAP_HIP_TRY(hipMemcpy(m->p_str.p, m->d_str.p, n_str_total, hipMemcpyDeviceToHost));
		}
		}
	}
	stage_align.done();

	lap(3);
	ngm::SamRef *sam_refs = sam ? m->p_sam_refs.p : nullptr;
	std::mutex extra_mu;
	std::vector<char> extra;
	parallel_for(n, [&](int lo, int hi) {
		for (int i = lo; i < hi; ++i) for (int t = 0; t < topn; ++t) {
			const size_t o = (size_t) i * topn + t;
			ngm_hit &h = hits[o];
			memset(&h, 0, sizeof(h));
			h.n_candidates = (int) m->h_count[i];
			h.max_votes = m->h_maxv[i];
			h.mapq = h_mapq[i];
			h.n_best = h_nbest[i];
			h.score = h_best[i];
			h.pair_flags = pair_flags[i];
			if (!sam) { cigars[o * str_stride] = 0; mds[o * str_stride] = 0; }
			else sam_refs[o] = ngm::SamRef{0, 0, 0, 0};
		}
	});
	ngm::CigarParams cp{m->prm.match_bonus, -m->prm.mismatch_penalty, m->prm.variant, m->prm.hard_clip, m->prm.silent_clip, alt_cigar};
	parallel_for(na, [&](int lo, int hi) {
		std::vector<char> win((size_t) q + c + 8), qry((size_t) q + 8), scr(sam ? 2 * str_stride : 0);
		for (int j = lo; j < hi; ++j) {
			const int i = (int) a_read[j];
			const size_t o = a_out[j];
			ngm_hit &h = hits[o];
			if (topn > 1) h.score = h_scores[a_pair[j]];
			const bool rev = a_sv[j] & 1u;
			h.reverse = rev;
			const char *rd = reads + (size_t) i * q;
			int L_cached = -1;
			auto read_length = [&]() { if (L_cached < 0) L_cached = (int) strnlen(rd, q); return L_cached; };
			ngm_hip_align_out ao{};
			ao.cigar = sam ? scr.data() : cigars + o * str_stride;
			ao.md = sam ? scr.data() + str_stride : mds + o * str_stride;
			bool host_strings = true;
			const ngm::CigarDevOut *dv = dev_strings ? &m->p_cigout.p[j] : nullptr;
			if (dv && (dv->flags & 1)) {
				if (!(dv->flags & 2)) { h.mapped = 0; continue; }
				if (sam) { sam_refs[o] = ngm::SamRef{dv->cig_off, dv->md_off, dv->cig_len, dv->md_len}; host_strings = false; }
				else {
					memcpy(ao.cigar, m->p_str.p + dv->cig_off, dv->cig_len); ao.cigar[dv->cig_len] = 0;
					memcpy(ao.md, m->p_str.p + dv->md_off, dv->md_len); ao.md[dv->md_len] = 0;
				}
				ao.identity = dv->identity; ao.nm = dv->nm; ao.qstart = dv->qstart; ao.qend = dv->qend; ao.position_offset = dv->position_offset;
				ao.score_token = dv->score_token;
			} else if (m->prm.personality == NGM_PERSONALITY_AFFINE) {
				ngm::build_cigar_affine(&h_rec[(size_t) j * 8], &h_runs[(size_t) (uint32_t) h_rec[(size_t) j * 8 + 6]], nullptr, nullptr, q, &ao, read_length());
				memcpy(ao.md, "!!!", 4);
			} else {
				const uint64_t offset = (uint64_t) a_loc[j] - (uint64_t) (c >> 1);
				host_window(r, offset, align_buf_len, q + c, win.data());
				memset(qry.data(), 0, qry.size());
				const int L = read_length();
				if (!rev) memcpy(qry.data(), rd, L);
				else for (int t = 0; t < L; ++t) {
					const char ch = rd[L - 1 - t];
					qry[t] = ch == 'A' ? 'T' : ch == 'T' ? 'A' : ch == 'C' ? 'G' : ch == 'G' ? 'C' : ch;
				}
				const bool second = paired && (i & 1);
				ngm::build_cigar_md(cp, &h_rec[(size_t) j * 8], &h_runs[(size_t) (uint32_t) h_rec[(size_t) j * 8 + 6]], win.data(), qry.data(), &ao, cp.alt ? ((rev ? !second : second) ? 1 : 0) : 0);
				if (ao.score_token < 0) { h.mapped = 0; continue; }
			}
			if (sam && host_strings) {
				const size_t cl = strlen(ao.cigar), ml = strlen(ao.md);
				std::lock_guard<std::mutex> lk(extra_mu);
				const size_t at = extra.size();
				extra.insert(extra.end(), ao.cigar, ao.cigar + cl);
				extra.insert(extra.end(), ao.md, ao.md + ml);
				sam_refs[o] = ngm::SamRef{(uint32_t) (str_base + at), (uint32_t) (str_base + at + cl), (uint16_t) cl, (uint16_t) ml};
			}
			h.identity = ao.identity; h.nm = ao.nm; h.qstart = ao.qstart; h.qend = ao.qend;
			const uint64_t final_loc = (uint64_t) a_loc[j] + (uint64_t) (int64_t) ao.position_offset - (uint64_t) (c >> 1);
			int contig = 0; uint64_t cpos = 0;
			if (!ngm_ref_convert(r, final_loc, &contig, &cpos)) { h.mapped = 0; continue; }
			h.mapped = 1; h.contig = contig; h.pos = cpos;
		}
	});

	lap(4);
	if (sam) {
		GpuStage stage_sam(m, 1, false, 2);
		const int units = paired ? n / 2 : n;
		if (!extra.empty()) {
			const size_t need = (size_t) str_base + extra.size();
			if (need > m->d_str.cap) {
				ngm::DevBuf<char> bigger;
				if (bigger.reserve(need + 4096)) { ngm::pipeline_set_error("out of device memory (SAM strings)"); return -12; }
				if (str_base) MAP_HIP_TRY(hipMemcpyAsync(bigger.p, m->d_str.p, (size_t) str_base, hipMemcpyDeviceToDevice, m->st));
				MAP_HIP_TRY(hipStreamSynchronize(m->st));
				std::swap(bigger, m->d_str);
				bigger.release();
			}
			if (m->p_sam_extra.reserve(extra.size())) { ngm::pipeline_set_error("out of pinned host memory"); return -12; }
			memcpy(m->p_sam_extra.p, extra.data(), extra.size());
			MAP_HIP_TRY(hipMemcpyAsync(m->d_str.p + str_base, m->p_sam_extra.p, extra.size(), hipMemcpyHostToDevice, m->st));
		}
		if (m->d_sam_len.reserve((size_t) units + 1) || m->d_sam_off.reserve((size_t) units + 1)) { ngm::pipeline_set_error("out of device memory (SAM stage)"); return -12; }
		MAP_HIP_TRY(hipMemcpyAsync(m->d_sam_hits.p, hits, (size_t) n * sizeof(ngm_hit), hipMemcpyHostToDevice, m->st));
		MAP_HIP_TRY(hipMemcpyAsync(m->d_sam_refs.p, sam_refs, (size_t) n * sizeof(ngm::SamRef), hipMemcpyHostToDevice, m->st));
		MAP_HIP_TRY(hipMemsetAsync(m->d_total.p + 16, 0, 64, m->st));
// ... 351 lines not shown
	DevGuard g(device);
	ngm::DevBuf<uint32_t> d_base, d_count, d_loc, d_tied_n, d_list;
	ngm::DevBuf<uint16_t> d_len;
	ngm::DevBuf<float> d_sc;
	ngm::DevBuf<int32_t> d_mq, d_nb, d_info;
	ngm::DevBuf<ngm::PairOut> d_out;
	ngm::DevBuf<ngm::PairTop> d_top;
	auto run = [&]() -> int {
		if (d_base.reserve(n) || d_count.reserve(n) || d_len.reserve(n) || d_loc.reserve(nc) || d_sc.reserve(nc) || d_mq.reserve(n) || d_nb.reserve(n) || d_info.reserve(npairs + 1) ||
				d_tied_n.reserve(4) || d_list.reserve(3 * npairs + 2) || d_out.reserve(2 * npairs + 2) || d_top.reserve(npairs + 1)) {
			ngm::pipeline_set_error("out of device memory (ngm_debug_pair_select)"); return -12; }
		MAP_HIP_TRY(hipMemcpy(d_base.p, base, n * 4, hipMemcpyHostToDevice));
		MAP_HIP_TRY(hipMemcpy(d_count.p, count, n * 4, hipMemcpyHostToDevice));
		MAP_HIP_TRY(hipMemcpy(d_len.p, read_len, n * 2, hipMemcpyHostToDevice));
		MAP_HIP_TRY(hipMemcpy(d_mq.p, mapq, n * 4, hipMemcpyHostToDevice));
		MAP_HIP_TRY(hipMemcpy(d_nb.p, n_best, n * 4, hipMemcpyHostToDevice));
		if (n_cand) {
			MAP_HIP_TRY(hipMemcpy(d_sc.p, scores, (size_t) n_cand * 4, hipMemcpyHostToDevice));
			MAP_HIP_TRY(hipMemcpy(d_loc.p, loc, (size_t) n_cand * 4, hipMemcpyHostToDevice));
		}
		MAP_HIP_TRY(hipMemset(d_info.p, 0xFF, (npairs + 1) * 4));
		MAP_HIP_TRY(hipMemset(d_out.p, 0xFF, (2 * npairs + 2) * sizeof(ngm::PairOut)));
		MAP_HIP_TRY(hipMemset(d_top.p, 0xFF, (npairs + 1) * sizeof(ngm::PairTop)));
		MAP_HIP_TRY(hipDeviceSynchronize());
		if (int rc = launch_pair_select(0, npairs, d_base.p, d_count.p, d_sc.p, d_loc.p, d_len.p, min_insert, max_insert, cutoff, d_mq.p, d_nb.p, d_info.p, true,
				d_tied_n.p, d_list.p, d_out.p, d_top.p)) return rc;
		MAP_HIP_TRY(hipDeviceSynchronize());
		MAP_HIP_TRY(hipMemcpy(info, d_info.p, npairs * 4, hipMemcpyDeviceToHost));
		MAP_HIP_TRY(hipMemcpy(mapq, d_mq.p, n * 4, hipMemcpyDeviceToHost));
		MAP_HIP_TRY(hipMemcpy(n_best, d_nb.p, n * 4, hipMemcpyDeviceToHost));
		MAP_HIP_TRY(hipMemcpy(counts, d_tied_n.p, 16, hipMemcpyDeviceToHost));
		MAP_HIP_TRY(hipMemcpy(entries, d_out.p, (2 * npairs + 2) * sizeof(ngm::PairOut), hipMemcpyDeviceToHost));
		MAP_HIP_TRY(hipMemcpy(tops, d_top.p, (npairs + 1) * sizeof(ngm::PairTop), hipMemcpyDeviceToHost));
		return 0;
	};
	const int rc = run();
	d_base.release(); d_count.release(); d_loc.release(); d_tied_n.release(); d_list.release(); d_len.release(); d_sc.release(); d_mq.release(); d_nb.release(); d_info.release();
	d_out.release(); d_top.release();
	return rc;
}

int ngm_mapper_heavy_counters(ngm_mapper *m, uint64_t out[4]) {
	if (!m || !out) return -22;
	out[0] = m->st_heavy_second; out[1] = m->st_heavy_restart; out[2] = m->st_heavy_sent_on; out[3] = m->st_pool_regrown;
	return 0;
}

int ngm_mapper_order_table_reads(ngm_mapper *m, uint64_t *out) {
	if (!m || !out) return -22;
	*out = m->st_order_table;
	return 0;
}

int ngm_mapper_search_turn_counters(ngm_mapper *m, uint64_t out[3]) {
	if (!m || !out) return -22;
	out[0] = m->turn_dbg[0]; out[1] = m->turn_dbg[1]; out[2] = m->turn_dbg[2];
	return 0;
}

int ngm_mapper_cs_counters(ngm_mapper *m, uint64_t out[3]) {
	if (!m) return -22;
	out[0] = m->cs_kmers; out[1] = m->cs_hits; out[2] = m->n_cand;
	return 0;
}

float ngm_mapper_last_order_replay_ms(ngm_mapper *m) { return m ? m->order_ms : 0.f; }

int ngm_mapper_last_pair_stats(ngm_mapper *m, uint64_t out[3]) {
	if (!m || !out) return -22;
	out[0] = m->pair_stats[0]; out[1] = m->pair_stats[1]; out[2] = m->pair_stats[2];
	return 0;
}

int ngm_mapper_last_kernel_ms(ngm_mapper *m, float ms[8]) {
	if (!m) return -22;
	for (int i = 0; i < 8; ++i) ms[i] = m->ms[i];
	return 0;
}

}
```

### nextgenmap_amd/csrc/mapper_internal.h

```cpp
#pragma once

#include <algorithm>
#include <atomic>
#include <chrono>
#include <climits>
#include <cmath>
#include <cstdlib>
#include <cstdio>
#include <cstring>
#include <condition_variable>
#include <mutex>
#include <numeric>
#include <thread>
#include <vector>

#include <string.h>
#include <ctype.h>
#include <sched.h>
#include "../../include/ngm_pipeline.h"
#include "refindex.h"
#include "engine_internal.h"
#include "cigar_md.h"
#include "cigar_device.h"
#include "cs_device.h"
// ... 97 lines not shown
	ngm_coverage *coverage = nullptr;
	ngm::DevBuf<uint8_t> d_cov_mask;
	std::vector<uint8_t> cov_mask;
	std::vector<char> cov_text;
	std::vector<int32_t> cov_ref, cov_pos;
	std::vector<uint32_t> cov_off;
	ngm_snp *snp = nullptr;
	std::vector<uint8_t> snp_rows;
	bool sam_ready = false;
	std::string sam_rg;
	ngm::DevBuf<char> d_sam_contig_names, d_sam_rg, d_sam_names, d_sam_text;
	ngm::DevBuf<uint32_t> d_sam_contig_off, d_sam_len, d_sam_off;
	ngm::DevBuf<uint64_t> d_sam_contig_start;
	ngm::DevBuf<uint8_t> d_sam_quals;
	ngm::DevBuf<uint16_t> d_sam_polya;
	ngm::DevBuf<ngm::SamMeta> d_sam_meta;
	ngm::DevBuf<ngm::SamRef> d_sam_refs;
	ngm::DevBuf<ngm_hit> d_sam_hits;
	ngm::PinnedBuf<ngm_hit> p_sam_hits;
	ngm::PinnedBuf<ngm::SamRef> p_sam_refs;
	ngm::PinnedBuf<char> p_sam_extra;
	uint64_t sam_text_bytes = 0;
	bool argos_on = false;
	bool argos_text = false;
	float argos_min = 0.f;
	int argos_n_starts = 0;
	ngm::DevBuf<uint64_t> d_argos_starts, d_argos_loff, d_argos_gkeys;
	ngm::DevBuf<uint32_t> d_argos_ord, d_argos_nsurv, d_argos_npos, d_argos_list, d_argos_llist, d_argos_gvals, d_argos_hord, d_argos_hoff;
	ngm::DevBuf<uint8_t> d_argos_cls;
	ngm::DevBuf<unsigned long long> d_argos_ctr;
	ngm::PinnedBuf<uint8_t> p_argos_cls;
	ngm::PinnedBuf<uint32_t> p_argos_nsurv;
	uint64_t argos_ctr[4] = {0, 0, 0, 0};
	uint64_t argos_long = 0, argos_unknown = 0;
	hipEvent_t aev[4] = {};
	uint64_t pair_stats[3] = {0, 0, 0};
	int n_reads = 0;
	template <typename T> struct HostArr {
		ngm::PinnedBuf<T> b;
		T &operator[](size_t i) { return b.p[i]; }
		const T &operator[](size_t i) const { return b.p[i]; }
		T *data() { return b.p; }
	};
	HostArr<uint32_t> h_base, h_count;
	HostArr<float> h_maxv;
	uint64_t n_cand = 0;
	bool cs_eager_arrays = false;
	int cs_arrays_state = 0;
	int canon_per_cu = 0;
	const void *canon_fn = nullptr;
	size_t canon_lds = 0;
	uint64_t np_seen_max = 0;
	uint64_t turn_dbg[3] = {0, 0, 0};
	hipEvent_t ev[10] = {};
	float ms[8] = {};
};

namespace ngm {

struct DevGuard {
	int prev = -1;
	explicit DevGuard(int d) { if (hipGetDevice(&prev) != hipSuccess) prev = -1; if (prev != d) (void) hipSetDevice(d); else prev = -1; }
	~DevGuard() { if (prev >= 0) (void) hipSetDevice(prev); }
};

struct StageLock { std::mutex mu; };
extern StageLock g_stage_lock[16][2];
extern std::atomic<long long> g_stage_hold_us[3], g_stage_wait_us[3];
struct GpuStage {
	ngm_mapper *m;
	int kind, slot;
	bool held = false;
	StageLock *ch = nullptr;
	std::chrono::steady_clock::time_point t_acq;
	static int mode() { static const int v = getenv("NGM_HIP_GPU_STAGE_LOCK") ? atoi(getenv("NGM_HIP_GPU_STAGE_LOCK")) : 1; return v; }
	GpuStage(ngm_mapper *m_, int kind_ = 0, bool now = true, int slot_ = -1) : m(m_), kind(kind_), slot(slot_ < 0 ? kind_ : slot_) {
		ch = &g_stage_lock[(unsigned) m->ref->device & 15u][mode() == 2 ? kind : 0];
		if (now) acquire();
	}
	~GpuStage() { release(); }
	void acquire() {
		if (mode() == 0 || held) return;
		const auto t0 = std::chrono::steady_clock::now();
		ch->mu.lock();
		held = true;
		t_acq = std::chrono::steady_clock::now();
		g_stage_wait_us[slot] += std::chrono::duration_cast<std::chrono::microseconds>(t_acq - t0).count();
	}
	void release() {
		if (!held) return;
		g_stage_hold_us[slot] += std::chrono::duration_cast<std::chrono::microseconds>(std::chrono::steady_clock::now() - t_acq).count();
		held = false;
		ch->mu.unlock();
	}
	void done_after(hipEvent_t ev) { if (held) (void) hipEventSynchronize(ev); release(); }
	void done() { release(); }
};

int cs_configure(ngm_mapper *m, const ngm_mapper_params *p);
int run_cs(ngm_mapper *m, int n, GpuStage *stage = nullptr, bool defer_host_arrays = false);
int cs_enqueue_host_arrays(ngm_mapper *m);
int cs_host_arrays(ngm_mapper *m);
int candidate_order(ngm_mapper *m, const std::vector<uint32_t> &list, uint64_t np, uint32_t **h_rank, bool wait = true);
int candidate_order_wait(ngm_mapper *m, uint32_t **h_rank);
void cs_release(ngm_mapper *m);
long test_limit(const char *key, long dflt);

int score_candidates(ngm_mapper *m, int n, uint64_t np, int alt_dir);
void argos_release(ngm_mapper *m);

}
```

### nextgenmap_amd/csrc/ngm_hip.cpp

```cpp
#include "../../include/ngm_hip.h"
#include "../../include/ngm_pipeline.h"

#include <hip/hip_runtime.h>

#include <algorithm>

#include <cstdarg>
#include <cstdio>
#include <cstdlib>
#include <cstring>
#include <mutex>
#include <string>
#include <vector>

#define NGM_ENGINE_KERNELS
#include "engine_internal.h"
#include "align_device.h"
#include "affine_device.h"
#include "cigar_md.h"
#include "jit.h"

namespace {

thread_local std::string g_last_error;
// ... 7 lines not shown
			set_error(ctx, "%s failed: %s (%s:%d)", #expr, hipGetErrorString(e_), __FILE__, __LINE__); \
			return -5;                                                                             \
		}                                                                                          \
	} while (0)

}


namespace {

void set_error(ngm_hip_ctx *ctx, const char *fmt, ...) {
	char buf[1024];
	va_list ap;
	va_start(ap, fmt);
	vsnprintf(buf, sizeof(buf), fmt, ap);
	va_end(ap);
	g_last_error = buf;
	if (ctx) ctx->error = buf;
}

#define NGM_CORRIDORS(X) X(8) X(12) X(19) X(20) X(27) X(42) X(80)

struct KernelRef {
	const void *aot = nullptr;
	hipFunction_t jit = nullptr;
	explicit operator bool() const { return aot || jit; }
};

const void *find_aot_kernel(int c, int kind) {
#define X(C) if (c == C) switch (kind) { \
		case 0: return (const void *) ngm::sw_score_kernel<C, false>; case 1: return (const void *) ngm::sw_score_kernel<C, true>; \
		case 2: return (const void *) ngm::sw_align_kernel<C, false>; case 3: return (const void *) ngm::sw_align_kernel<C, true>; \
		case 4: return (const void *) ngm::sw_affine_kernel<C + 1, false, false>; case 5: return (const void *) ngm::sw_affine_kernel<C + 1, true, false>; \
		case 6: return (const void *) ngm::sw_affine_kernel<C + 1, false, true>; default: return (const void *) ngm::sw_affine_kernel<C + 1, true, true>; }
	NGM_CORRIDORS(X)
#undef X
	return nullptr;
}

const void *find_pk_score_kernel(int c, bool endfree) {
#define X(C) if (c == C) return endfree ? (const void *) ngm::sw_score_pk_kernel<C, true> : (const void *) ngm::sw_score_pk_kernel<C, false>;
	NGM_CORRIDORS(X)
#undef X
	return nullptr;
}

const void *find_pk_affine_score_kernel(int c, bool endfree) {
#define X(C) if (c == C) return endfree ? (const void *) ngm::sw_affine_score_pk_kernel<C + 1, true> : (const void *) ngm::sw_affine_score_pk_kernel<C + 1, false>;
	NGM_CORRIDORS(X)
#undef X
	return nullptr;
}

const void *find_pk_affine_score_split_kernel(int c) {
	if (c == 80) return (const void *) ngm::sw_affine_score_pk_split_kernel<81>;
	return nullptr;
}

template <int CP> const void *pk_affine_align_ptr(bool window) {
	if (!window) { if constexpr (CP <= 32) return (const void *) ngm::sw_affine_align_pk_kernel<CP, false>; else return nullptr; }
	if constexpr (CP <= 128) return (const void *) ngm::sw_affine_align_pk_kernel<CP, true>; else return nullptr;
}
const void *find_pk_affine_align_kernel(int c, bool window) {
#define X(C) if (c == C) return pk_affine_align_ptr<C + 1>(window);
	NGM_CORRIDORS(X)
#undef X
	return nullptr;
}

template <int C> const void *pk_align_ptr(bool window) {
	if (!window) { if constexpr (C <= 32) return (const void *) ngm::sw_align_pk_kernel<C, false>; else return nullptr; }
	if constexpr (C <= 128) return (const void *) ngm::sw_align_pk_kernel<C, true>; else return nullptr;
}
const void *find_pk_align_kernel(int c, bool window) {
#define X(C) if (c == C) return pk_align_ptr<C>(window);
	NGM_CORRIDORS(X)
#undef X
	return nullptr;
}

KernelRef find_kernel(ngm_hip_ctx *ctx, int kind) {
	KernelRef k;
	k.aot = find_aot_kernel(ctx->c, kind);
	if (!k.aot && ctx->jit) k.jit = ctx->jit->fn[kind];
	return k;
}

template <typename... Args>
hipError_t launch_kernel(const KernelRef &k, dim3 grid, dim3 block, hipStream_t st, Args... args) {
	void *argv[] = {(void *) &args...};
	if (k.aot) return hipLaunchKernel(k.aot, grid, block, argv, 0, st);
	return hipModuleLaunchKernel(k.jit, grid.x, grid.y, grid.z, block.x, block.y, block.z, 0, st, argv, nullptr);
}

int n_blocks_of(int n) { return (n + ngm::kSlots - 1) / ngm::kSlots; }

}
namespace ngm {
int engine_reserve(ngm_hip_ctx *ctx, int n) {
	const size_t nb = (size_t) n_blocks_of(n);
	if (ctx->packed.reserve(nb * (size_t) (ctx->RW + ctx->FW) * ngm::kSlots) || ctx->lens.reserve(nb * ngm::kSlots) ||
			ctx->blk_rows.reserve(nb)) {
		set_error(ctx, "out of device memory reserving the packed workspace for %d pairs", n);
		return -12;
	}
	return 0;
}

int engine_score_packed(ngm_hip_ctx *ctx, int mode, int n, float *d_scores, hipStream_t st) {
	const int nb = n_blocks_of(n);
	static const bool force32 = getenv("NGM_HIP_SCORE_32BIT") != nullptr;
	if (ctx->prm.personality == NGM_PERSONALITY_AFFINE) {
		const bool ef = (mode & NGM_MODE_ALIGN_MASK) == NGM_MODE_END_TO_END;
		if (!force32 && (long) ctx->q * ctx->KA.tM < 30000 && ctx->prm.gap_read_penalty + (long) ctx->q * (ctx->prm.gap_extend_penalty + ctx->KA.tZ) < 19000) {
			if (const void *sp = ef ? nullptr : find_pk_affine_score_split_kernel(ctx->c)) {
				KernelRef kp; kp.aot = sp;
				const int units = 2 * ((nb + 1) / 2);
				HIP_TRY(ctx, launch_kernel(kp, dim3((units + 3) / 4), dim3(256), st, (const uint32_t *) ctx->packed.p, (const uint16_t *) ctx->lens.p,
						(const uint16_t *) ctx->blk_rows.p, d_scores, n, nb, ctx->RW, ctx->KA));
				return 0;
			}
			if (const void *pk = find_pk_affine_score_kernel(ctx->c, ef)) {
				KernelRef kp; kp.aot = pk;
				HIP_TRY(ctx, launch_kernel(kp, dim3((nb + 7) / 8), dim3(256), st, (const uint32_t *) ctx->packed.p, (const uint16_t *) ctx->lens.p,
						(const uint16_t *) ctx->blk_rows.p, d_scores, n, nb, ctx->RW, ctx->KA));
				return 0;
			}
		}
		const KernelRef ka = find_kernel(ctx, 4 + ((mode & NGM_MODE_ALIGN_MASK) == NGM_MODE_END_TO_END ? 1 : 0));
		HIP_TRY(ctx, launch_kernel(ka, dim3((nb + 3) / 4), dim3(256), st, (const uint32_t *) ctx->packed.p, (const uint16_t *) ctx->lens.p,
				(const uint16_t *) ctx->blk_rows.p, d_scores, (uint32_t *) nullptr, (int32_t *) nullptr, n, nb, ctx->RW, ctx->q, ctx->KA));
		return 0;
	}
	const bool endfree = (mode & NGM_MODE_ALIGN_MASK) == NGM_MODE_END_TO_END;
	if (!force32 && (long) ctx->q * std::max(ctx->K.tM, ctx->K.alt ? std::max(ctx->K.tMA, ctx->K.tXA) : 0) < 30000 && (long) ctx->q * ctx->K.tZ < 14000) {
		if (const void *pk = find_pk_score_kernel(ctx->c, endfree)) {
			KernelRef kp; kp.aot = pk;
			HIP_TRY(ctx, launch_kernel(kp, dim3((nb + 7) / 8), dim3(256), st, (const uint32_t *) ctx->packed.p, (const uint16_t *) ctx->lens.p,
					(const uint16_t *) ctx->blk_rows.p, d_scores, n, nb, ctx->RW, ctx->K));
			return 0;
		}
	}
	const KernelRef k = find_kernel(ctx, endfree ? 1 : 0);
	HIP_TRY(ctx, launch_kernel(k, dim3((nb + 3) / 4), dim3(256), st, (const uint32_t *) ctx->packed.p, (const uint16_t *) ctx->lens.p,
			(const uint16_t *) ctx->blk_rows.p, d_scores, n, nb, ctx->RW, ctx->K));
	return 0;
}

int engine_affine_traceback_packed(ngm_hip_ctx *ctx, int n, int32_t *d_records, uint16_t *d_runs, int run_stride, hipStream_t st) {
	hipLaunchKernelGGL(ngm::affine_traceback_kernel, dim3((n + 255) / 256), dim3(256), 0, st, ctx->dirs.p, d_records, d_runs, n,
			ctx->q, ctx->c + 1, run_stride, (const uint32_t *) ctx->packed.p, ctx->RW, ctx->FW, ctx->trace_nibbles ? 1 : 0);
	HIP_TRY(ctx, hipGetLastError());
	return 0;
}

int engine_align_packed(ngm_hip_ctx *ctx, int mode, int n, int32_t *d_records, uint16_t *d_runs, int run_stride, hipStream_t st, const AlignFinish *fin) {
	const int am = mode & NGM_MODE_ALIGN_MASK;
	const int nb = n_blocks_of(n);
	if (ctx->prm.personality == NGM_PERSONALITY_AFFINE) {
		const int CP = ctx->c + 1, ADW = ngm::aff_dir_words(CP);
		if (ctx->dirs.reserve((size_t) nb * ctx->q * ADW * ngm::kSlots)) { set_error(ctx, "out of device memory for the trace matrix"); return -12; }
		static const bool force32 = getenv("NGM_HIP_ALIGN_32BIT") != nullptr;
		const void *pk = nullptr;
		if (!force32 && am != NGM_MODE_END_TO_END && ctx->KA.open < 0 && ctx->KA.ext < 0 && (long) ctx->q * ctx->KA.tM < 30000 &&
				ctx->prm.gap_read_penalty + (long) ctx->q * (ctx->prm.gap_extend_penalty + ctx->KA.tZ) < 19000) {
			const bool plain_key = (long) ctx->q * ctx->prm.match_bonus < 2048 && ctx->c + 1 <= 32;
			if (plain_key) pk = find_pk_affine_align_kernel(ctx->c, false);
			else if (ctx->KA.tZ > 0 && ctx->KA.tM > 0 && ctx->KA.tM + 1 <= 63) pk = find_pk_affine_align_kernel(ctx->c, true);
		}
		if (pk) {
			KernelRef kp; kp.aot = pk;
			HIP_TRY(ctx, launch_kernel(kp, dim3((nb + 7) / 8), dim3(256), st, (const uint32_t *) ctx->packed.p, (const uint16_t *) ctx->lens.p,
					(const uint16_t *) ctx->blk_rows.p, ctx->dirs.p, d_records, n, nb, ctx->RW, ctx->q, ctx->KA));
		} else {
			const KernelRef ka = find_kernel(ctx, 6 + (am == NGM_MODE_END_TO_END ? 1 : 0));
			HIP_TRY(ctx, launch_kernel(ka, dim3((nb + 3) / 4), dim3(256), st, (const uint32_t *) ctx->packed.p, (const uint16_t *) ctx->lens.p,
					(const uint16_t *) ctx->blk_rows.p, (float *) nullptr, ctx->dirs.p, d_records, n, nb, ctx->RW, ctx->q, ctx->KA));
		}
		if (ctx->profiling) HIP_TRY(ctx, hipEventRecord(ctx->ev[2], st));
		ctx->trace_nibbles = pk != nullptr;
		if (!fin) return engine_affine_traceback_packed(ctx, n, d_records, d_runs, run_stride, st);
		if (pk) hipLaunchKernelGGL(ngm::affine_finish_kernel<true>, dim3((n + 255) / 256), dim3(256), 0, st, n, (const uint32_t *) ctx->dirs.p, (const int32_t *) d_records,
				(const uint32_t *) ctx->packed.p, (const uint16_t *) ctx->lens.p, ctx->q, CP, ctx->RW, ctx->FW, fin->out, fin->bytes, fin->capacity, fin->counters);
		else hipLaunchKernelGGL(ngm::affine_finish_kernel<false>, dim3((n + 255) / 256), dim3(256), 0, st, n, (const uint32_t *) ctx->dirs.p, (const int32_t *) d_records,
				(const uint32_t *) ctx->packed.p, (const uint16_t *) ctx->lens.p, ctx->q, CP, ctx->RW, ctx->FW, fin->out, fin->bytes, fin->capacity, fin->counters);
		HIP_TRY(ctx, hipGetLastError());
		return 0;
	}
	if (fin) { set_error(ctx, "the finishing kernel serves the affine personality only"); return -22; }
	const int DW = ngm::dir_words(ctx->c);
	if (ctx->dirs.reserve((size_t) nb * ctx->q * DW * ngm::kSlots)) { set_error(ctx, "out of device memory for the direction matrix"); return -12; }
	static const bool force32 = getenv("NGM_HIP_ALIGN_32BIT") != nullptr;
	const void *pk = nullptr;
	const int max_gain = std::max(ctx->K.tM, ctx->K.alt ? std::max(ctx->K.tMA, ctx->K.tXA) : 0);
	if (!force32 && am != NGM_MODE_END_TO_END && (long) ctx->q * max_gain < 30000 && (long) ctx->q * ctx->K.tZ < 14000 && ctx->K.gl < 0 && ctx->K.gap_read < 0) {
		const bool plain_key = (long) ctx->q * (max_gain - ctx->K.tZ) < 2048 && ctx->c <= 32;
		if (plain_key) pk = find_pk_align_kernel(ctx->c, false);
		else if (ctx->K.tZ > 0 && max_gain + 1 <= 63) pk = find_pk_align_kernel(ctx->c, true);
	}
	if (pk) {
		KernelRef kp; kp.aot = pk;
		HIP_TRY(ctx, launch_kernel(kp, dim3((nb + 7) / 8), dim3(256), st, (const uint32_t *) ctx->packed.p, (const uint16_t *) ctx->lens.p,
				(const uint16_t *) ctx->blk_rows.p, ctx->dirs.p, d_records, n, nb, ctx->RW, ctx->q, ctx->K));
	} else {
		const KernelRef k = find_kernel(ctx, 2 + (am == NGM_MODE_END_TO_END ? 1 : 0));
		HIP_TRY(ctx, launch_kernel(k, dim3((nb + 3) / 4), dim3(256), st, (const uint32_t *) ctx->packed.p, (const uint16_t *) ctx->lens.p,
				(const uint16_t *) ctx->blk_rows.p, ctx->dirs.p, d_records, n, nb, ctx->RW, ctx->q, ctx->K));
	}
	if (ctx->profiling) HIP_TRY(ctx, hipEventRecord(ctx->ev[2], st));
	hipLaunchKernelGGL(ngm::sw_traceback_kernel, dim3((n + 255) / 256), dim3(256), 0, st, ctx->dirs.p, ctx->lens.p, d_records,
			d_runs, n, ctx->q, ctx->c, run_stride, am == NGM_MODE_END_TO_END ? 1 : 0);
	HIP_TRY(ctx, hipGetLastError());
	return 0;
}
}
namespace {
using ngm::engine_reserve;

struct ScopedDevice {
	int prev = -1;
	explicit ScopedDevice(int dev) { if (hipGetDevice(&prev) != hipSuccess) prev = -1; if (prev != dev) (void) hipSetDevice(dev); else prev = -1; }
	~ScopedDevice() { if (prev >= 0) (void) hipSetDevice(prev); }
};

int launch_pack(ngm_hip_ctx *ctx, int n, const void *d_ref, const void *d_qry, hipStream_t st) {
	const int nb = n_blocks_of(n);
	const size_t lds = (size_t) ngm::kSlots * (ctx->rl + ctx->q);
	hipLaunchKernelGGL(ngm::pack_pairs_kernel, dim3(nb), dim3(256), lds, st, (const uint8_t *) d_ref,
			(const uint8_t *) d_qry, n, ctx->q, ctx->rl, ctx->RW, ctx->FW, ctx->packed.p, ctx->lens.p, ctx->blk_rows.p,
			ctx->prm.personality == NGM_PERSONALITY_AFFINE ? 1 : 0, (ctx->K.alt || ctx->prm.alt_cigar) ? ctx->pair_dir : nullptr);
	HIP_TRY(ctx, hipGetLastError());
	return 0;
}

int stage_dirs(ngm_hip_ctx *ctx, int n, const char *dir) {
	ctx->pair_dir = nullptr;
// ... 242 lines not shown
			ctx->d_qry.reserve((size_t) n * q) || ctx->d_records.reserve((size_t) n * 8) || ctx->d_runs.reserve((size_t) n * rs) ||
			ctx->h_records.reserve((size_t) n * 8) || ctx->h_runs.reserve((size_t) n * rs)) {
		set_error(ctx, "out of memory staging %d pairs", n);
		return -12;
	}
	for (int i = 0; i < n; ++i) {
		memcpy(ctx->h_ref.p + (size_t) i * rl, ref[i], rl);
		memcpy(ctx->h_qry.p + (size_t) i * q, qry[i], q);
	}
	const unsigned long long scap = (unsigned long long) n * ngm::kCigarRow + 4096ull;
	ngm::DevBuf<ngm::CigarDevOut> d_out;
	ngm::DevBuf<char> d_str;
	ngm::DevBuf<unsigned long long> d_ctr;
	std::vector<ngm::CigarDevOut> h_out((size_t) n);
	std::vector<char> h_str((size_t) scap);
	unsigned long long ctr[2] = {0, 0};
	auto run = [&]() -> int {
		if (d_out.reserve(n) || d_str.reserve(scap) || d_ctr.reserve(2)) { set_error(ctx, "out of device memory (ngm_debug_align_finish)"); return -12; }
		HIP_TRY(ctx, hipMemcpyAsync(ctx->d_ref.p, ctx->h_ref.p, (size_t) n * rl, hipMemcpyHostToDevice, ctx->stream));
		HIP_TRY(ctx, hipMemcpyAsync(ctx->d_qry.p, ctx->h_qry.p, (size_t) n * q, hipMemcpyHostToDevice, ctx->stream));
		HIP_TRY(ctx, hipMemsetAsync(d_ctr.p, 0, 16, ctx->stream));
		if (int r = engine_reserve(ctx, n)) return r;
		if (int r = launch_pack(ctx, n, ctx->d_ref.p, ctx->d_qry.p, ctx->stream)) return r;
		const ngm::AlignFinish fin{d_out.p, d_str.p, scap, d_ctr.p};
		if (int r = ngm::engine_align_packed(ctx, mode, n, ctx->d_records.p, ctx->d_runs.p, rs, ctx->stream, &fin)) return r;
		HIP_TRY(ctx, hipMemcpyAsync(h_out.data(), d_out.p, (size_t) n * sizeof(ngm::CigarDevOut), hipMemcpyDeviceToHost, ctx->stream));
		HIP_TRY(ctx, hipMemcpyAsync(ctr, d_ctr.p, 16, hipMemcpyDeviceToHost, ctx->stream));
		HIP_TRY(ctx, hipStreamSynchronize(ctx->stream));
		const unsigned long long used = std::min(ctr[0], scap);
		if (used) HIP_TRY(ctx, hipMemcpy(h_str.data(), d_str.p, (size_t) used, hipMemcpyDeviceToHost));
		if (ctr[1]) {
			if (int r = ngm::engine_affine_traceback_packed(ctx, n, ctx->d_records.p, ctx->d_runs.p, rs, ctx->stream)) return r;
			HIP_TRY(ctx, hipMemcpyAsync(ctx->h_records.p, ctx->d_records.p, sizeof(int32_t) * 8 * (size_t) n, hipMemcpyDeviceToHost, ctx->stream));
			HIP_TRY(ctx, hipMemcpyAsync(ctx->h_runs.p, ctx->d_runs.p, sizeof(uint16_t) * (size_t) rs * n, hipMemcpyDeviceToHost, ctx->stream));
			HIP_TRY(ctx, hipStreamSynchronize(ctx->stream));
		}
		return 0;
	};
	const int rc = run();
	d_out.release(); d_str.release(); d_ctr.release();
	if (rc) return rc;
	*n_fallback = ctr[1];
	for (int i = 0; i < n; ++i) {
		const ngm::CigarDevOut &dv = h_out[(size_t) i];
		if (!(dv.flags & 1)) { ngm::build_cigar_affine(ctx->h_records.p + (size_t) i * 8, ctx->h_runs.p + (size_t) i * rs, ref[i], qry[i], ctx->q, &out[i]); continue; }
		memcpy(out[i].cigar, h_str.data() + dv.cig_off, dv.cig_len); out[i].cigar[dv.cig_len] = 0;
		memcpy(out[i].md, h_str.data() + dv.md_off, dv.md_len); out[i].md[dv.md_len] = 0;
		out[i].position_offset = dv.position_offset; out[i].qstart = dv.qstart; out[i].qend = dv.qend;
		out[i].score_token = dv.score_token; out[i].identity = dv.identity; out[i].nm = dv.nm;
	}
	return n;
}

}
```

### nextgenmap_amd/csrc/sw_device.h

```cpp
#pragma once

#include <hip/hip_runtime.h>
#include <stdint.h>

namespace ngm {

constexpr int kSlots = 64;
constexpr int kShortMin = -16000;

__host__ __device__ constexpr int sel_regs(int C) { return (((C + 7 + 3) / 4) + 1) & ~1; }
__host__ __device__ constexpr int read_words(int q) { return (q + 7) / 8; }
__host__ __device__ constexpr int ref_words(int q, int C) { return read_words(q) + sel_regs(C) / 2; }

struct SwConst {
	int tM;
	int tZ;
	int gl;
	int gu;
	int gap_read;
	int variant;
	int alt;
	int tMA;
	int tXA;
};
// ... 204 lines not shown
			if (!ENDFREE) best = max(best, rowmax - fl);
			fl += K.tZ;
		}
#pragma unroll
		for (int r = 0; r + 2 < NRG; ++r) RG[r] = RG[r + 2];
		RG[NRG - 2] = fx & 0x0F0F0F0Fu;
		RG[NRG - 1] = (fx >> 4) & 0x0F0F0F0Fu;
	}

	const int pair = blk * kSlots + lane;
	if (pair < n) {
		int result;
		if (ENDFREE) {
			const int klast = -(fl - K.tZ);
			int m = kShortMin;
#pragma unroll
			for (int d = 0; d < C; ++d) m = max(m, H[d] + klast);
			result = m;
		} else {
			result = best;
		}
		if (K.variant == 1 && lens[pair] == 0) result = ENDFREE ? kShortMin : -1;
		scores[pair] = (float) result;
	}
}

typedef short v2s __attribute__((ext_vector_type(2)));

__device__ __forceinline__ v2s pk_splat(int x) { v2s r; r.x = (short) x; r.y = (short) x; return r; }
__device__ __forceinline__ v2s pk_max(v2s a, v2s b) { return __builtin_elementwise_max(a, b); }
typedef unsigned short v2u __attribute__((ext_vector_type(2)));
__device__ __forceinline__ v2s pk_min(v2s a, v2s b) { return __builtin_elementwise_min(a, b); }
__device__ __forceinline__ v2s pk_min_op(v2s a, v2s b) {
	v2s r;
	asm("v_pk_min_i16 %0, %1, %2" : "=v"(r) : "v"(a), "v"(b));
	return r;
}
__device__ __forceinline__ v2s pk_mul(v2s a, v2s b) {
	v2s r;
	asm("v_pk_mul_lo_u16 %0, %1, %2" : "=v"(r) : "v"(a), "v"(b));
	return r;
}
__device__ __forceinline__ v2s pk_mad(v2s a, v2s b, v2s c) {
	v2s r;
	asm("v_pk_mad_u16 %0, %1, %2, %3" : "=v"(r) : "v"(a), "v"(b), "v"(c));
	return r;
}
__device__ __forceinline__ v2s pk_mad_k(v2s a, v2s b, int k) {
	v2s r;
	const uint32_t kk = ((uint32_t) k & 0xFFFFu) * 0x10001u;
	asm("v_pk_mad_u16 %0, %1, %2, %3" : "=v"(r) : "v"(a), "v"(b), "s"(kk));
	return r;
}
__device__ __forceinline__ v2s pk_min1_op(v2s a) {
	v2s r;
	asm("v_pk_min_i16 %0, %1, 1 op_sel_hi:[1,0]" : "=v"(r) : "v"(a));
	return r;
}
__device__ __forceinline__ v2s pk_min1_u_op(v2s a) {
	v2s r;
	asm("v_pk_min_u16 %0, %1, 1 op_sel_hi:[1,0]" : "=v"(r) : "v"(a));
	return r;
}
__device__ __forceinline__ v2s pk_sub_sat(v2s a, v2s b) { return __builtin_elementwise_sub_sat(a, b); }
__device__ __forceinline__ v2s pk_min_u_op(v2s a, v2s b) {
	v2s r;
	asm("v_pk_min_u16 %0, %1, %2" : "=v"(r) : "v"(a), "v"(b));
	return r;
}

template <int C, bool ENDFREE>
__global__ __launch_bounds__(256) void sw_score_pk_kernel(const uint32_t *__restrict__ packed,
		const uint16_t *__restrict__ lens, const uint16_t *__restrict__ blk_rows,
		float *__restrict__ scores, int n, int n_blocks, int RW, SwConst K) {
	__shared__ uint2 s_tab[16];
	if (threadIdx.x < 16) s_tab[threadIdx.x] = make_row_table(threadIdx.x, K);
	__syncthreads();
	const int lane = threadIdx.x & 63;
	const int blkA = 2 * (blockIdx.x * 4 + (threadIdx.x >> 6));
	if (blkA >= n_blocks) return;
	const bool hasB = blkA + 1 < n_blocks;
	const int blkB = hasB ? blkA + 1 : blkA;
	constexpr int NRG = sel_regs(C);
	const int FW = RW + NRG / 2;
	const uint32_t *rdA = packed + (size_t) blkA * (RW + FW) * kSlots + lane, *rdB = packed + (size_t) blkB * (RW + FW) * kSlots + lane;
	const uint32_t *fdA = rdA + (size_t) RW * kSlots, *fdB = rdB + (size_t) RW * kSlots;
	const int rows = max(__builtin_amdgcn_readfirstlane((int) blk_rows[blkA]), __builtin_amdgcn_readfirstlane((int) blk_rows[blkB]));
	const int ngroups = (rows + 7) >> 3;

	v2s H[C];
#pragma unroll
	for (int d = 0; d < C; ++d) H[d] = pk_splat(0);
	uint32_t RGA[NRG], RGB[NRG];
#pragma unroll
	for (int r = 0; r < NRG / 2; ++r) {
		const uint32_t xa = fdA[(size_t) r * kSlots], xb = fdB[(size_t) r * kSlots];
		RGA[2 * r] = xa & 0x0F0F0F0Fu; RGA[2 * r + 1] = (xa >> 4) & 0x0F0F0F0Fu;
		RGB[2 * r] = xb & 0x0F0F0F0Fu; RGB[2 * r + 1] = (xb >> 4) & 0x0F0F0F0Fu;
	}
	int fl = K.tZ;
	v2s best = pk_splat(0);
	const v2s gl2 = pk_splat(K.gl), gu2 = pk_splat(K.gu);
	uint32_t rnA = (ngroups > 0) ? rdA[0] : 0x66666666u, rnB = (ngroups > 0) ? rdB[0] : 0x66666666u;

	for (int g = 0; g < ngroups; ++g) {
		const uint32_t rxA = rnA, rxB = rnB;
// ... 65 lines not shown
```

### nextgenmap_amd/engine.py

```python
import ctypes as C
import os

import numpy as np

MODE_LOCAL = 0
MODE_END_TO_END = 1
VARIANT_OCL_GPU = 0
VARIANT_OCL_CPU = 1
PERSONALITY_LINEAR = 0
PERSONALITY_AFFINE = 1
ABI_VERSION = 3

_HERE = os.path.dirname(os.path.abspath(__file__))


class NgmHipError(RuntimeError):
    pass


class Params(C.Structure):
    _fields_ = [("abi_version", C.c_int), ("qry_max_len", C.c_int), ("corridor", C.c_int),
                ("match_bonus", C.c_int), ("mismatch_penalty", C.c_int), ("gap_read_penalty", C.c_int),
                ("gap_ref_penalty", C.c_int), ("variant", C.c_int), ("hard_clip", C.c_int),
                ("silent_clip", C.c_int), ("max_batch", C.c_int), ("personality", C.c_int),
                ("gap_extend_penalty", C.c_int), ("alt_scoring", C.c_int), ("match_bonus_tt", C.c_int), ("match_bonus_tc", C.c_int), ("alt_cigar", C.c_int)]


class AlignOut(C.Structure):
    _fields_ = [("cigar", C.c_void_p), ("md", C.c_void_p), ("position_offset", C.c_int), ("qstart", C.c_int),
                ("qend", C.c_int), ("score_token", C.c_float), ("identity", C.c_float), ("nm", C.c_int)]


def library_path():
    return os.path.join(_HERE, "libngm_hip.so")


_lib = None


def load_library():
    global _lib
    if _lib is not None:
        return _lib
    try:
        import torch
    except ImportError:
        pass
    path = library_path()
    if not os.path.exists(path):
        raise NgmHipError("HIP extension missing: %s (run `python -m nextgenmap_amd.build`)" % path)
    lib = C.CDLL(path)
    lib.ngm_hip_create.restype = C.c_void_p
    lib.ngm_hip_create.argtypes = [C.c_int, C.POINTER(Params)]
    lib.ngm_hip_destroy.argtypes = [C.c_void_p]
    lib.ngm_hip_last_error.restype = C.c_char_p
    lib.ngm_hip_last_error.argtypes = [C.c_void_p]
    lib.ngm_hip_device_count.restype = C.c_int
    lib.ngm_hip_score_batch_size.argtypes = [C.c_void_p]
    lib.ngm_hip_align_batch_size.argtypes = [C.c_void_p]
    lib.ngm_hip_batch_score.argtypes = [C.c_void_p, C.c_int, C.c_int, C.c_void_p, C.c_void_p, C.c_void_p, C.c_void_p]
    lib.ngm_hip_batch_align.argtypes = [C.c_void_p, C.c_int, C.c_int, C.c_void_p, C.c_void_p, C.c_void_p, C.c_void_p]
    lib.ngm_hip_score_device.argtypes = [C.c_void_p, C.c_int, C.c_int, C.c_void_p, C.c_void_p, C.c_void_p, C.c_void_p]
    lib.ngm_hip_align_run_stride.argtypes = [C.c_void_p]
    lib.ngm_hip_align_device.argtypes = [C.c_void_p, C.c_int, C.c_int, C.c_void_p, C.c_void_p, C.c_void_p, C.c_void_p,
                                         C.c_int, C.c_void_p]
    lib.ngm_hip_last_kernel_ms.argtypes = [C.c_void_p, C.POINTER(C.c_float)]
    lib.ngm_hip_set_profiling.argtypes = [C.c_void_p, C.c_int]
    lib.ngm_debug_align_finish.argtypes = [C.c_void_p, C.c_int, C.c_int, C.c_void_p, C.c_void_p, C.c_void_p, C.POINTER(C.c_uint64)]
    _lib = lib
    return lib


def _ptr(x):
    if x is None:
        return None
    if hasattr(x, "data_ptr"):
        return x.data_ptr()
    return int(x)


class Engine:

    def __init__(self, qry_max_len, corridor, match=10, mismatch=15, gap_read=20, gap_ref=20, device=0,
                 variant=VARIANT_OCL_GPU, hard_clip=0, silent_clip=0, max_batch=0, personality=PERSONALITY_LINEAR,
                 gap_extend=0, alt_scoring=0, match_bonus_tt=0, match_bonus_tc=0, alt_cigar=None):
        self.lib = load_library()
        self.q, self.c = int(qry_max_len), int(corridor)
        self.personality = int(personality)
        p = Params(ABI_VERSION, self.q, self.c, match, mismatch, gap_read, gap_ref, variant, hard_clip, silent_clip, max_batch,
                   self.personality, gap_extend, alt_scoring, match_bonus_tt, match_bonus_tc, alt_scoring if alt_cigar is None else alt_cigar)
        self.h = self.lib.ngm_hip_create(device, C.byref(p))
        if not self.h:
            raise NgmHipError(self.lib.ngm_hip_last_error(None).decode())

    def close(self):
        if getattr(self, "h", None):
            self.lib.ngm_hip_destroy(self.h)
            self.h = None

    def __del__(self):
        try:
            self.close()
        except Exception:
            pass

    def _check(self, r, n):
        if r < 0:
            raise NgmHipError(self.lib.ngm_hip_last_error(self.h).decode())
        return r

    def GetScoreBatchSize(self):
        return self.lib.ngm_hip_score_batch_size(self.h)

    def GetAlignBatchSize(self):
        return self.lib.ngm_hip_align_batch_size(self.h)

    def _ptr_lists(self, ref, qry):
        ref = np.ascontiguousarray(ref, dtype=np.uint8)
        qry = np.ascontiguousarray(qry, dtype=np.uint8)
        n = qry.shape[0]
        assert qry.shape[1] >= self.q and ref.shape[1] >= self.q + self.c and ref.shape[0] == n
        rp = (C.c_void_p * n)(*[ref.ctypes.data + i * ref.strides[0] for i in range(n)])
        qp = (C.c_void_p * n)(*[qry.ctypes.data + i * qry.strides[0] for i in range(n)])
        return n, ref, qry, rp, qp

    def BatchScore(self, mode, ref, qry, dirs=None):
        n, ref, qry, rp, qp = self._ptr_lists(ref, qry)
        out = np.full(n, -1.0, dtype=np.float32)
        d = None if dirs is None else np.ascontiguousarray(dirs, dtype=np.uint8)
        r = self._check(self.lib.ngm_hip_batch_score(self.h, mode, n, rp, qp, out.ctypes.data, None if d is None else d.ctypes.data), n)
        assert r == n
        return out

    def BatchAlign(self, mode, ref, qry, dirs=None, finish=False):
        n, ref, qry, rp, qp = self._ptr_lists(ref, qry)
        stride = 4 * max(1, self.q)
        cig = np.zeros((n, stride), dtype=np.uint8)
        md = np.zeros((n, stride), dtype=np.uint8)
        cig[:, :3] = ord("!")
        md[:, :3] = ord("!")
        outs = (AlignOut * n)()
        for i in range(n):
            outs[i].cigar = cig.ctypes.data + i * stride
            outs[i].md = md.ctypes.data + i * stride
        d = None if dirs is None else np.ascontiguousarray(dirs, dtype=np.uint8)
        if finish:
            fb = C.c_uint64(0)
            r = self._check(self.lib.ngm_debug_align_finish(self.h, mode, n, rp, qp, outs, C.byref(fb)), n)
            self.last_fallback = int(fb.value)
        else:
            r = self._check(self.lib.ngm_hip_batch_align(self.h, mode, n, rp, qp, outs, None if d is None else d.ctypes.data), n)
        assert r == n
        res = []
        for i in range(n):
            o = outs[i]
            res.append(dict(cigar=bytes(cig[i]).split(b"\0", 1)[0], md=bytes(md[i]).split(b"\0", 1)[0],
                            position_offset=o.position_offset, qstart=o.qstart, qend=o.qend,
                            score_token=o.score_token, identity=o.identity, nm=o.nm))
        return res

    def set_profiling(self, on):
        self.lib.ngm_hip_set_profiling(self.h, 1 if on else 0)

    def score_device(self, mode, n, d_ref, d_qry, d_scores, stream=None):
        return self._check(self.lib.ngm_hip_score_device(self.h, mode, n, _ptr(d_ref), _ptr(d_qry), _ptr(d_scores),
                                                          _ptr(stream)), n)

    def align_run_stride(self):
        return self.lib.ngm_hip_align_run_stride(self.h)

    def align_device(self, mode, n, d_ref, d_qry, d_records, d_runs, run_stride, stream=None):
        return self._check(self.lib.ngm_hip_align_device(self.h, mode, n, _ptr(d_ref), _ptr(d_qry), _ptr(d_records),
                                                          _ptr(d_runs), run_stride, _ptr(stream)), n)

    def last_kernel_ms(self):
        ms = (C.c_float * 3)()
        self._check(self.lib.ngm_hip_last_kernel_ms(self.h, ms), 0)
        return [ms[0], ms[1], ms[2]]
```

### nextgenmap_amd/pipeline.py

```python
import ctypes as C

import numpy as np

from .engine import NgmHipError, load_library


class RefParams(C.Structure):
    _fields_ = [("kmer", C.c_int), ("kmer_skip", C.c_int), ("bin_size", C.c_int)]


class MapperParams(C.Structure):
    _fields_ = [("qry_max_len", C.c_int), ("corridor", C.c_int), ("match_bonus", C.c_int), ("mismatch_penalty", C.c_int),
                ("gap_read_penalty", C.c_int), ("gap_ref_penalty", C.c_int), ("mode", C.c_int), ("variant", C.c_int),
                ("sensitivity", C.c_float), ("kmer_min", C.c_float), ("max_cmrs", C.c_int), ("max_kfreq", C.c_int),
                ("hard_clip", C.c_int), ("silent_clip", C.c_int), ("personality", C.c_int), ("gap_extend_penalty", C.c_int),
                ("min_insert_size", C.c_int), ("max_insert_size", C.c_int), ("pair_score_cutoff", C.c_float),
                ("topn", C.c_int), ("strata", C.c_int), ("bs_mapping", C.c_int), ("bs_cutoff", C.c_int), ("bs_read_skip", C.c_int),
                ("match_bonus_tt", C.c_int), ("match_bonus_tc", C.c_int), ("slam_seq", C.c_int)]


class SamOptions(C.Structure):
    _fields_ = [("paired", C.c_int), ("min_insert_size", C.c_int), ("max_insert_size", C.c_int), ("min_mq", C.c_int),
                ("min_identity", C.c_float), ("min_residues", C.c_float), ("no_unal", C.c_int), ("rg_id", C.c_char_p),
                ("bs_mapping", C.c_int), ("slam_seq", C.c_int), ("bam", C.c_int)]
# ... 15 lines not shown


class SnpParams(C.Structure):
    _fields_ = [("device", C.c_int), ("n_ref", C.c_int), ("ref_len", C.POINTER(C.c_uint32)), ("ref_name", C.POINTER(C.c_char_p)), ("ref_seq", C.POINTER(C.c_char_p)),
                ("min_cov", C.c_uint32), ("min_frac", C.c_double), ("min_qual", C.c_int), ("min_frac_text", C.c_char_p), ("scan_chunk", C.c_size_t)]


def _lib():
    global _bound
    lib = load_library()
    if not _bound:
        lib.ngm_pipeline_last_error.restype = C.c_char_p
        lib.ngm_ref_create.restype = C.c_void_p
        lib.ngm_ref_create.argtypes = [C.c_int, C.POINTER(RefParams), C.c_int, C.c_void_p, C.c_void_p, C.c_void_p]
        lib.ngm_ref_create_from_fasta.restype = C.c_void_p
        lib.ngm_ref_create_from_fasta.argtypes = [C.c_int, C.POINTER(RefParams), C.c_char_p]
        lib.ngm_ref_create_from_fasta_vcf.restype = C.c_void_p
        lib.ngm_ref_create_from_fasta_vcf.argtypes = [C.c_int, C.POINTER(RefParams), C.c_char_p, C.c_char_p]
        lib.ngm_ref_vcf_summary.argtypes = [C.c_void_p, C.c_void_p]
        lib.ngm_vcf_parse_text.restype = C.c_longlong
        lib.ngm_vcf_parse_text.argtypes = [C.c_int, C.c_void_p, C.c_void_p, C.c_char_p, C.c_void_p, C.c_size_t, C.POINTER(C.c_size_t)]
        lib.ngm_ref_create_from_cache.restype = C.c_void_p
        lib.ngm_ref_create_from_cache.argtypes = [C.c_int, C.POINTER(RefParams), C.c_char_p]
        lib.ngm_ref_destroy.argtypes = [C.c_void_p]
        lib.ngm_ref_contig_count.argtypes = [C.c_void_p]
        lib.ngm_ref_contig_name.restype = C.c_char_p
        lib.ngm_ref_contig_name.argtypes = [C.c_void_p, C.c_int]
        for f in ("ngm_ref_contig_start", "ngm_ref_contig_len"):
            getattr(lib, f).restype = C.c_uint64
            getattr(lib, f).argtypes = [C.c_void_p, C.c_int]
        for f in ("ngm_ref_concat_len", "ngm_ref_index_entries"):
            getattr(lib, f).restype = C.c_uint64
            getattr(lib, f).argtypes = [C.c_void_p]
        lib.ngm_ref_auto_max_kfreq.argtypes = [C.c_void_p]
        lib.ngm_ref_index_copy.argtypes = [C.c_void_p, C.c_void_p, C.c_void_p, C.c_void_p]
        if not hasattr(lib, "ngm_mapper_create"):
            raise NgmHipError("libngm_hip.so was built without the mapping pipeline")
        lib.ngm_ref_write_ngm_cache.argtypes = [C.c_void_p, C.c_char_p]
        lib.ngm_ref_decode.argtypes = [C.c_void_p, C.c_uint64, C.c_int, C.c_void_p]
        lib.ngm_ref_convert.argtypes = [C.c_void_p, C.c_uint64, C.POINTER(C.c_int), C.POINTER(C.c_uint64)]
        lib.ngm_mapper_create.restype = C.c_void_p
        lib.ngm_mapper_create.argtypes = [C.c_void_p, C.POINTER(MapperParams)]
        lib.ngm_mapper_destroy.argtypes = [C.c_void_p]
        lib.ngm_mapper_cs.argtypes = [C.c_void_p, C.c_int, C.c_void_p, C.c_void_p, C.c_void_p]
        lib.ngm_mapper_cs_fetch.argtypes = [C.c_void_p, C.c_void_p, C.c_void_p, C.c_void_p]
        lib.ngm_mapper_map_se.argtypes = [C.c_void_p, C.c_int, C.c_void_p, C.c_void_p, C.c_void_p, C.c_void_p]
        lib.ngm_mapper_map_se_resident.argtypes = [C.c_void_p, C.c_int, C.c_void_p, C.c_void_p, C.c_void_p, C.c_void_p, C.c_void_p]
        lib.ngm_mapper_map_pe_resident.argtypes = [C.c_void_p, C.c_int, C.c_void_p, C.c_void_p, C.c_void_p, C.c_void_p, C.c_void_p]
        lib.ngm_mapper_cs_counters.argtypes = [C.c_void_p, C.c_void_p]
        lib.ngm_mapper_path_counters.argtypes = [C.c_void_p, C.c_void_p]
        lib.ngm_mapper_order_table_reads.argtypes = [C.c_void_p, C.c_void_p]
        lib.ngm_mapper_heavy_counters.argtypes = [C.c_void_p, C.c_void_p]
        lib.ngm_mapper_search_turn_counters.argtypes = [C.c_void_p, C.c_void_p]
        lib.ngm_mapper_last_kernel_ms.argtypes = [C.c_void_p, C.POINTER(C.c_float)]
        lib.ngm_mapper_last_order_replay_ms.restype = C.c_float
        lib.ngm_mapper_last_order_replay_ms.argtypes = [C.c_void_p]
        lib.ngm_mapper_set_argos.argtypes = [C.c_void_p, C.c_float]
        lib.ngm_mapper_map_argos.restype = C.c_longlong
        lib.ngm_mapper_map_argos.argtypes = [C.c_void_p, C.c_int, C.c_void_p, C.c_void_p, C.c_size_t, C.c_void_p, C.c_void_p, C.c_size_t,
                                             C.c_void_p, C.POINTER(C.c_float)]
        lib.ngm_mapper_sam_fetch.argtypes = [C.c_void_p, C.c_void_p, C.c_size_t]
        lib.ngm_mapper_set_sam_options.argtypes = [C.c_void_p, C.c_void_p]
        lib.ngm_mapper_map_sam_trimmed.restype = C.c_longlong
        lib.ngm_mapper_map_sam_trimmed.argtypes = [C.c_void_p, C.c_int, C.c_void_p, C.c_void_p, C.c_void_p, C.c_size_t, C.c_void_p, C.c_void_p,
                                                   C.c_void_p, C.c_size_t, C.c_void_p, C.POINTER(C.c_float)]
        lib.ngm_argos_prolog.argtypes = [C.c_void_p, C.c_uint64, C.c_void_p, C.c_size_t]
        lib.ngm_mapper_argos_counters.argtypes = [C.c_void_p, C.c_void_p]
        lib.ngm_mapper_argos_path_counters.argtypes = [C.c_void_p, C.c_void_p]
        lib.ngm_debug_argos_order.argtypes = [C.c_uint32, C.c_void_p, C.c_void_p, C.c_float, C.c_int, C.c_int, C.c_void_p, C.c_void_p]
        lib.ngm_bgzf_create.restype = C.c_void_p
        lib.ngm_bgzf_create.argtypes = [C.c_int]
        lib.ngm_bgzf_destroy.argtypes = [C.c_void_p]
        lib.ngm_bgzf_bound.restype = C.c_size_t
        lib.ngm_bgzf_bound.argtypes = [C.c_size_t]
        lib.ngm_bgzf_compress.restype = C.c_longlong
        lib.ngm_bgzf_compress.argtypes = [C.c_void_p, C.c_void_p, C.c_size_t, C.c_void_p, C.c_size_t]
        lib.ngm_bgzf_inflated_size.restype = C.c_size_t
        lib.ngm_bgzf_inflated_size.argtypes = [C.c_char_p, C.c_size_t]
        lib.ngm_bgzf_inflate.restype = C.c_longlong
        lib.ngm_bgzf_inflate.argtypes = [C.c_void_p, C.c_char_p, C.c_size_t, C.c_void_p, C.c_size_t]
        lib.ngm_bgzf_last_kernel_ms.restype = C.c_float
        lib.ngm_bgzf_last_kernel_ms.argtypes = [C.c_void_p]
        lib.ngm_bam_sort_create.restype = C.c_void_p
        lib.ngm_bam_sort_create.argtypes = [C.POINTER(BamSortParams)]
        lib.ngm_bam_sort_destroy.argtypes = [C.c_void_p]
        lib.ngm_bam_sort_add.argtypes = [C.c_void_p, C.c_uint64, C.c_char_p, C.c_size_t]
        lib.ngm_bam_sort_finish.argtypes = [C.c_void_p, C.c_int]
        lib.ngm_bam_sort_next.restype = C.c_longlong
        lib.ngm_bam_sort_next.argtypes = [C.c_void_p, C.c_void_p, C.c_size_t]
        lib.ngm_bam_sort_index.restype = C.c_longlong
        lib.ngm_bam_sort_index.argtypes = [C.c_void_p, C.c_uint64, C.c_void_p, C.c_size_t]
        lib.ngm_bam_sort_stats.argtypes = [C.c_void_p, C.c_void_p, C.c_void_p]
        lib.ngm_mapper_set_bam_sorter.argtypes = [C.c_void_p, C.c_void_p]
        lib.ngm_coverage_create.restype = C.c_void_p
        lib.ngm_coverage_create.argtypes = [C.POINTER(CoverageParams)]
        lib.ngm_coverage_destroy.argtypes = [C.c_void_p]
        lib.ngm_coverage_add.argtypes = [C.c_void_p, C.c_void_p, C.c_void_p, C.c_void_p, C.c_char_p, C.c_size_t]
        lib.ngm_coverage_finish.argtypes = [C.c_void_p]
        lib.ngm_coverage_next.restype = C.c_longlong
        lib.ngm_coverage_next.argtypes = [C.c_void_p, C.c_void_p, C.c_size_t]
        lib.ngm_coverage_stats.argtypes = [C.c_void_p, C.c_void_p, C.c_void_p]
        lib.ngm_mapper_set_coverage.argtypes = [C.c_void_p, C.c_void_p]
        lib.ngm_snp_create.restype = C.c_void_p
        lib.ngm_snp_create.argtypes = [C.POINTER(SnpParams)]
        lib.ngm_snp_create_for_ref.restype = C.c_void_p
        lib.ngm_snp_create_for_ref.argtypes = [C.c_void_p, C.POINTER(SnpParams)]
# ... 461 lines not shown
        rows = np.ascontiguousarray(rows, dtype=np.uint8)
        hits, cig, md = self.map_pe_raw(rows)
        return hits, [bytes(r).split(b"\0", 1)[0] for r in cig], [bytes(r).split(b"\0", 1)[0] for r in md]

    def map_se_raw(self, rows, d_rows=None, out=None, paired=False):
        n = rows.shape[0]
        stride = 4 * max(1, self.q)
        if out is None:
            no = n * (1 if paired else self.topn)
            out = (np.zeros(no, HIT_DTYPE), np.zeros((no, stride), np.uint8), np.zeros((no, stride), np.uint8))
        hits, cig, md = out
        dp = None if d_rows is None else (d_rows.data_ptr() if hasattr(d_rows, "data_ptr") else int(d_rows))
        fn = self.lib.ngm_mapper_map_pe_resident if paired else self.lib.ngm_mapper_map_se_resident
        r = fn(self.h, n, rows.ctypes.data, dp, hits.ctypes.data, cig.ctypes.data, md.ctypes.data)
        if r < 0:
            raise _err()
        return hits, cig, md

    def map_se(self, rows):
        rows = np.ascontiguousarray(rows, dtype=np.uint8)
        hits, cig, md = self.map_se_raw(rows)
        return hits, [bytes(r).split(b"\0", 1)[0] for r in cig], [bytes(r).split(b"\0", 1)[0] for r in md]

    def set_coverage(self, coverage):
        if self.lib.ngm_mapper_set_coverage(self.h, coverage._h if coverage is not None else None) < 0:
            raise _err()

    def set_snp(self, snp):
        if self.lib.ngm_mapper_set_snp(self.h, snp._h if snp is not None else None) < 0:
            raise _err()

    def set_bam_sorter(self, sorter):
        if self.lib.ngm_mapper_set_bam_sorter(self.h, sorter._h if sorter is not None else None) < 0:
            raise _err()

    def last_kernel_ms(self):
        ms = (C.c_float * 8)()
        self.lib.ngm_mapper_last_kernel_ms(self.h, ms)
        return list(ms)

    def last_order_replay_ms(self):
        return float(self.lib.ngm_mapper_last_order_replay_ms(self.h))

    def path_counters(self):
        out = np.zeros(8, np.uint64)
        self.lib.ngm_mapper_path_counters(self.h, out.ctypes.data)
        return dict(zip(("reads", "candidates", "exact_lds", "exact_global", "order_replayed", "order_exact_global", "order_undetermined", "heavy"), (int(x) for x in out[:8])))

    def heavy_counters(self):
        out = np.zeros(4, np.uint64)
        self.lib.ngm_mapper_heavy_counters(self.h, out.ctypes.data)
        return dict(zip(("second_passes", "table_pass_restarts", "sent_on", "pool_regrown"), (int(x) for x in out)))

    def search_turn_counters(self):
        out = np.zeros(3, np.uint64)
        self.lib.ngm_mapper_search_turn_counters(self.h, out.ctypes.data)
        return dict(zip(("arrays_deferred", "search_attempts", "buffers_regrown"), (int(x) for x in out)))

    def order_table_reads(self):
        out = np.zeros(1, np.uint64)
        self.lib.ngm_mapper_order_table_reads(self.h, out.ctypes.data)
        return int(out[0])

    def map_argos(self, reads, names, min_score=0.0):
        rows = reads if isinstance(reads, np.ndarray) else self.reads_to_rows(reads, self.q)
        rows = np.ascontiguousarray(rows, dtype=np.uint8)
        n = rows.shape[0]
        if len(names) != n:
            raise ValueError("one name per read")
        if self.lib.ngm_mapper_set_argos(self.h, float(min_score)) < 0:
            raise _err()
        nb = [x.encode() if isinstance(x, str) else bytes(x) for x in names]
        meta = np.zeros((n, 2), np.uint32)
        off = 0
        for i, b in enumerate(nb):
            meta[i, 0], meta[i, 1] = off, min(len(b), 0xFFFF)
            off += len(b)
        blob = np.frombuffer(b"".join(nb) + b"\0", np.uint8)
        stats = np.zeros(3, np.uint64)
        kms = C.c_float(0)
        cap = max(1 << 16, n * 64)
        out = np.zeros(cap, np.uint8)
        total = self.lib.ngm_mapper_map_argos(self.h, n, rows.ctypes.data, blob.ctypes.data, off, meta.ctypes.data, out.ctypes.data, cap,
                                              stats.ctypes.data, C.byref(kms))
        if total < 0:
            raise _err()
        if total > cap:
            out = np.zeros(total, np.uint8)
            if self.lib.ngm_mapper_sam_fetch(self.h, out.ctypes.data, total) < 0:
                raise _err()
        return out[:total].tobytes(), [int(x) for x in stats]

    def map_sam(self, reads, quals, names, polya_trimmed=None, paired=False, rg_id=None, slam_seq=0, bam=False, min_insert_size=0,
                max_insert_size=1000, min_mq=0, min_identity=0.65, min_residues=0.5, no_unal=False):
        rows = reads if isinstance(reads, np.ndarray) else self.reads_to_rows(reads, self.q)
        rows = np.ascontiguousarray(rows, dtype=np.uint8)
        n = rows.shape[0]
        if len(names) != n or len(quals) != n or (polya_trimmed is not None and len(polya_trimmed) != n):
            raise ValueError("one name, one quality string and one poly-A count per read")
        so = SamOptions(int(paired), min_insert_size, max_insert_size, min_mq, min_identity, min_residues, int(no_unal),
                        rg_id.encode() if isinstance(rg_id, str) else rg_id, 0, int(slam_seq), int(bam))
        if self.lib.ngm_mapper_set_sam_options(self.h, C.byref(so)) < 0:
            raise _err()
        nb = [x.encode() if isinstance(x, str) else bytes(x) for x in names]
        qrows = np.zeros((n, self.q), np.uint8)
        meta = np.zeros(n, np.dtype([("name_off", np.uint32), ("name_len", np.uint16), ("qual_len", np.uint16)]))
# ... 37 lines not shown
```

Before: 59.91 million.

## Record SW end cell during scoring and resolve ungapped alignments without gapped traceback

The local-mode affine score kernel gains a variant that also tracks the end cell of the best score, packed into a max-reduced key. A new kernel walks back along the diagonal from that cell to emit a simple CIGAR when an ungapped path reproduces the score exactly. Only the remaining undecided pairs are compacted into a residual set, and the gather, gapped align and finish kernels run on that set using a device-side count. This is meant to skip the expensive gapped traceback for the many 150bp reads that align without indels. It costs extra kernels, a residual compaction pass and a slightly heavier score inner loop.

```diff
diff --git a/include/ngm_pipeline.h b/include/ngm_pipeline.h
--- a/include/ngm_pipeline.h
+++ b/include/ngm_pipeline.h
@@ -226,6 +226,11 @@
 int ngm_debug_align_finish(void *engine , int mode, int n, const char *const *ref, const char *const *qry, void *out ,
 		uint64_t *n_fallback);
 
+int ngm_debug_align_ungapped(void *engine , int mode, int n, const char *const *ref, const char *const *qry, void *out ,
+		uint64_t *n_fallback, uint64_t *n_ungapped);
+int ngm_debug_score_endcell(void *engine , int mode, int n, const char *const *ref, const char *const *qry, int32_t *out6);
+int ngm_mapper_align_ungapped_counters(ngm_mapper *m, uint64_t out[2]);
+
 int ngm_debug_expand_pairs(int device, int n_reads, const uint32_t *base, const uint32_t *count, uint64_t n_cand, uint32_t *out);
 
 int ngm_debug_pair_select(int device, int n_pairs, const uint32_t *base, const uint32_t *count, uint64_t n_cand, const float *scores, const uint32_t *loc,
diff --git a/nextgenmap_amd/csrc/affine_device.h b/nextgenmap_amd/csrc/affine_device.h
--- a/nextgenmap_amd/csrc/affine_device.h
+++ b/nextgenmap_amd/csrc/affine_device.h
@@ -184,9 +184,10 @@
 
 constexpr int kAffNeg16 = -20000;
 
-template <int CP, bool ENDFREE>
+template <int CP, bool ENDFREE, bool ENDCELL = false>
 __global__ __launch_bounds__(256) void sw_affine_score_pk_kernel(const uint32_t *__restrict__ packed, const uint16_t *__restrict__ lens,
-		const uint16_t *__restrict__ blk_rows, float *__restrict__ scores, int n, int n_blocks, int RW, AffConst K) {
+		const uint16_t *__restrict__ blk_rows, float *__restrict__ scores, int n, int n_blocks, int RW, AffConst K, uint32_t *__restrict__ endcell) {
+	static_assert(!ENDCELL || (!ENDFREE && CP <= 32), "the end cell comes from the plain row key of the local-mode align kernel");
 	__shared__ uint2 s_tab[8];
 	if (threadIdx.x < 8) s_tab[threadIdx.x] = aff_row_table(threadIdx.x, K);
 	__syncthreads();
@@ -232,6 +233,7 @@
 	int fl = K.tZ;
 	v2s best2 = pk_splat(0);
 	int bestA = kAffNeg, bestB = kAffNeg;
+	uint32_t cellA = 8191u << 5, cellB = 8191u << 5;
 	const v2s ext2 = pk_splat(K.ext), open2 = pk_splat(K.open), vext2 = pk_splat(K.vext), vopen2 = pk_splat(K.vopen);
 	const v2s neg2 = pk_splat(kAffNeg16), one2 = pk_splat(1), zero2 = pk_splat(0);
 	uint32_t rnA = (ngroups > 0) ? rdA[0] : 0x66666666u, rnB = (ngroups > 0) ? rdB[0] : 0x66666666u;
@@ -259,6 +261,8 @@
 			const v2s fl2 = pk_splat(fl);
 			v2s leftS = neg2, leftEh = neg2;
 			v2s rowmax = fl2;
+			v2u rowkey = __builtin_bit_cast(v2u, zero2);
+			const int keybase = 31 - 32 * fl;
 #pragma unroll
 			for (int d = 0; d < CP; ++d) {
 				const int bi = s + d, kb = bi & 3;
@@ -270,14 +274,22 @@
 				v2s sc = pk_max(pk_max(ev, eh), dg);
 				if (!ENDFREE) {
 					sc = pk_max(sc, fl2);
-					rowmax = pk_max(rowmax, sc);
+					if (ENDCELL) rowkey = __builtin_elementwise_max(rowkey, __builtin_bit_cast(v2u, pk_mad32_k(sc, keybase - d)));
+					else rowmax = pk_max(rowmax, sc);
 				}
 				S[d] = sc;
 				Ev[d] = ev;
 				leftS = sc;
 				leftEh = eh;
 			}
-			if (!ENDFREE) {
+			if (ENDCELL) {
+				const uint32_t ka = rowkey.x, kb2 = rowkey.y;
+				const uint32_t da = 31u - (ka & 31u), db = 31u - (kb2 & 31u);
+				const uint32_t wa = ((ka >> 5) << 18) | ((8191u - ((uint32_t) i + 1u + da)) << 5) | da;
+				const uint32_t wb = ((kb2 >> 5) << 18) | ((8191u - ((uint32_t) i + 1u + db)) << 5) | db;
+				cellA = (i < lenVA && wa > cellA) ? wa : cellA;
+				cellB = (i < lenVB && wb > cellB) ? wb : cellB;
+			} else if (!ENDFREE) {
 				best2 = pk_max(best2, rowmax - fl2);
 			} else if (i + 1 == lenVA || i + 1 == lenVB) {
 				const int kv = -fl;
@@ -300,6 +312,12 @@
 		RGB[NRG - 2] = fxB & 0x0F0F0F0Fu; RGB[NRG - 1] = (fxB >> 4) & 0x0F0F0F0Fu;
 	}
 	if (!ENDFREE) { bestA = best2.x; bestB = best2.y; }
+	if (ENDCELL) {
+		bestA = (int) (cellA >> 18); bestB = (int) (cellB >> 18);
+		const uint32_t ha = 8191u - ((cellA >> 5) & 8191u), hb = 8191u - ((cellB >> 5) & 8191u);
+		if (pairA < n) endcell[pairA] = (ha << 16) | (ha - (cellA & 31u));
+		if (hasB && pairB < n) endcell[pairB] = (hb << 16) | (hb - (cellB & 31u));
+	}
 	if (pairA < n) { if (lenVA < 1 || lenHA < 1) bestA = 0; scores[pairA] = (float) bestA; }
 	if (hasB && pairB < n) { if (lenVB < 1 || lenHB < 1) bestB = 0; scores[pairB] = (float) bestB; }
 }
@@ -427,8 +445,10 @@
 
 template <int CP, bool WINDOW>
 __global__ __launch_bounds__(256) void sw_affine_align_pk_kernel(const uint32_t *__restrict__ packed, const uint16_t *__restrict__ lens,
-		const uint16_t *__restrict__ blk_rows, uint32_t *__restrict__ dirs, int32_t *__restrict__ records, int n, int n_blocks, int RW, int q, AffConst K) {
+		const uint16_t *__restrict__ blk_rows, uint32_t *__restrict__ dirs, int32_t *__restrict__ records, int n, int n_blocks, int RW, int q, AffConst K,
+		const uint32_t *__restrict__ n_dev) {
 	static_assert(WINDOW ? CP <= 128 : CP <= 32, "the row key keeps the band column in 7 / 5 bits");
+	if (n_dev) { n = min(n, (int) *n_dev); n_blocks = (n + kSlots - 1) / kSlots; }
 	__shared__ uint2 s_tab[8];
 	if (threadIdx.x < 8) s_tab[threadIdx.x] = aff_row_table(threadIdx.x, K);
 	__syncthreads();
diff --git a/nextgenmap_amd/csrc/cigar_device.h b/nextgenmap_amd/csrc/cigar_device.h
--- a/nextgenmap_amd/csrc/cigar_device.h
+++ b/nextgenmap_amd/csrc/cigar_device.h
@@ -184,10 +184,12 @@
 template <bool NIBBLES>
 __global__ __launch_bounds__(256) void affine_finish_kernel(int n, const uint32_t *__restrict__ dirs, const int32_t *__restrict__ records,
 		const uint32_t *__restrict__ packed, const uint16_t *__restrict__ lens, int q, int CP, int RW, int FW, CigarDevOut *__restrict__ out,
-		char *__restrict__ bytes, unsigned long long capacity, unsigned long long *__restrict__ counters) {
+		char *__restrict__ bytes, unsigned long long capacity, unsigned long long *__restrict__ counters,
+		const uint32_t *__restrict__ n_dev = nullptr, const uint32_t *__restrict__ residual = nullptr) {
 	__shared__ char s_rows[256 * kCigarRow];
 	__shared__ uint32_t s_wave[4];
 	__shared__ unsigned long long s_base;
+	if (n_dev) { n = min(n, (int) *n_dev); if ((int) (blockIdx.x * blockDim.x) >= n) return; }
 	const int j = blockIdx.x * blockDim.x + threadIdx.x;
 	const bool live = j < n;
 	const int lane = threadIdx.x & 63, wv = threadIdx.x >> 6;
@@ -338,7 +340,7 @@
 		}
 	}
 	if (!fits) atomicAdd(&counters[1], 1ull);
-	CigarDevOut *o = out + j;
+	CigarDevOut *o = out + (residual ? residual[j] : (uint32_t) j);
 	o->cig_off = cig_off; o->md_off = fits ? cig_off + (uint32_t) co : 0u;
 	o->cig_len = (uint16_t) co; o->md_len = (uint16_t) mo;
 	o->position_offset = h; o->qstart = v; o->qend = qend; o->nm = n_mis;
@@ -347,4 +349,133 @@
 	o->flags = (fits ? 1 : 0) | 2;
 }
 
-}
+static __global__ __launch_bounds__(256) void affine_ungapped_kernel(int n, const uint32_t *__restrict__ pair_of, const float *__restrict__ scores,
+		const uint32_t *__restrict__ endcell, const uint32_t *__restrict__ packed, const uint16_t *__restrict__ lens, int RW, int FW, int corridor,
+		int h_safe, int match, int mismatch, CigarDevOut *__restrict__ out, char *__restrict__ bytes, unsigned long long capacity,
+		unsigned long long *__restrict__ counters, uint32_t *__restrict__ undecided, uint32_t *__restrict__ wg_undecided) {
+	__shared__ char s_rows[256 * 32];
+	__shared__ uint32_t s_wave[4], s_und[4];
+	__shared__ unsigned long long s_base;
+	constexpr int kRow = 32;
+	const int j = blockIdx.x * blockDim.x + threadIdx.x;
+	const bool live = j < n;
+	const int lane = threadIdx.x & 63, wv = threadIdx.x >> 6;
+	char *row = s_rows + (size_t) threadIdx.x * kRow;
+	int pos = kRow;
+	auto put_back = [&](int num, char tag) {
+		row[--pos] = tag;
+		unsigned u = (unsigned) num;
+		do { row[--pos] = (char) ('0' + u % 10u); u /= 10u; } while (u);
+	};
+	bool decided = false;
+	int h = 0, v = 0, len_v = 0, n_match = 0, n_mis = 0, total = 0;
+	if (live) {
+		const uint32_t p = pair_of ? pair_of[j] : (uint32_t) j;
+		const int target = (int) scores[p];
+		const uint32_t ec = endcell[p];
+		h = (int) (ec >> 16); v = (int) (ec & 0xFFFFu);
+		len_v = (int) lens[p];
+		if (target <= 0) decided = true;
+		else if (len_v + corridor <= h_safe && v >= 1 && h >= v && v <= RW * 8) {
+			const uint32_t *pk = packed + (size_t) (p >> 6) * (RW + FW) * kSlots + (p & 63u);
+			const int d0 = h - v;
+			int sum = 0, r = v - 1;
+			auto spread = [](uint32_t x) -> unsigned long long { return (unsigned long long) (x & 0x0F0F0F0Fu) | ((unsigned long long) ((x >> 4) & 0x0F0F0F0Fu) << 32); };
+			const unsigned long long ones = 0x0101010101010101ull;
+			for (int g = r >> 3; g >= 0 && !decided; --g) {
+				const int f0 = (8 * g + d0) >> 3, o = (8 * g + d0) & 7;
+				const unsigned long long RB = spread(pk[(size_t) g * kSlots]);
+				const unsigned long long A = spread(f0 < FW ? pk[(size_t) (RW + f0) * kSlots] : 0x66666666u);
+				const unsigned long long B = spread((o && f0 + 1 < FW) ? pk[(size_t) (RW + f0 + 1) * kSlots] : 0x66666666u);
+				const unsigned long long WB = o ? (A >> (8 * o)) | (B << (64 - 8 * o)) : A;
+				const unsigned long long differ = (((RB ^ WB) + 0x0F0F0F0F0F0F0F0Full) >> 4) & ones;
+				const unsigned long long odd = (RB >> 2) & (~RB | (RB >> 1)) & ones;
+				const unsigned long long bad = differ | odd;
+				for (int k = r & 7; k >= 0; --k, --r) {
+					const bool mis = (bad >> (8 * k)) & 1ull;
+					sum += mis ? -mismatch : match;
+					n_mis += mis ? 1 : 0;
+					++total;
+					if (sum == target) { decided = true; break; }
+				}
+			}
+			if (decided) { n_match = total - n_mis; h -= total; v -= total; }
+		}
+	}
+	int co = 0;
+	const int qend = len_v - (v + total);
+	if (live && decided) {
+		if (qend > 0) put_back(qend, 'S');
+		if (total > 0) put_back(total, 'M');
+		if (v > 0) put_back(v, 'S');
+		co = kRow - pos;
+	}
+	constexpr int mo = 3;
+	const uint32_t need = (live && decided) ? (uint32_t) (co + mo) : 0u;
+	uint32_t incl = need;
+#pragma unroll
+	for (int d = 1; d < 64; d <<= 1) { const uint32_t t = __shfl_up(incl, d); if (lane >= d) incl += t; }
+	if (lane == 63) s_wave[wv] = incl;
+	__syncthreads();
+	uint32_t before = incl - need, total_b = 0;
+#pragma unroll
+	for (int w2 = 0; w2 < 4; ++w2) { if (w2 < wv) before += s_wave[w2]; total_b += s_wave[w2]; }
+	if (threadIdx.x == 0) s_base = total_b ? atomicAdd(&counters[0], (unsigned long long) total_b) : 0ull;
+	__syncthreads();
+	const unsigned long long base = s_base;
+	if (need && base + total_b > capacity) decided = false;
+	if (live && decided) {
+		const unsigned long long off = base + before;
+		const char *cg = row + pos;
+		for (int t = 0; t < co; ++t) bytes[off + t] = cg[t];
+		for (int t = 0; t < mo; ++t) bytes[off + co + t] = '!';
+		CigarDevOut *o = out + j;
+		o->cig_off = (uint32_t) off; o->md_off = (uint32_t) off + (uint32_t) co;
+		o->cig_len = (uint16_t) co; o->md_len = (uint16_t) mo;
+		o->position_offset = h; o->qstart = v; o->qend = qend; o->nm = n_mis;
+		o->identity = (float) n_match * 1.0f / (float) total;
+		o->score_token = 0.f;
+		o->flags = 3;
+	}
+	const bool und = live && !decided;
+	if (live) undecided[j] = und ? 1u : 0u;
+	const unsigned long long mu = __ballot(und);
+	if (lane == 0) s_und[wv] = (uint32_t) __popcll(mu);
+	__syncthreads();
+	if (threadIdx.x == 0) wg_undecided[blockIdx.x] = s_und[0] + s_und[1] + s_und[2] + s_und[3];
+}
+
+static __global__ __launch_bounds__(256) void affine_residual_collect_kernel(int n, const uint32_t *__restrict__ undecided, const uint32_t *__restrict__ wg_undecided,
+		const uint32_t *__restrict__ a_read, const uint32_t *__restrict__ a_loc, const uint32_t *__restrict__ a_sv, uint32_t *__restrict__ r_read,
+		uint32_t *__restrict__ r_loc, uint32_t *__restrict__ r_sv, uint32_t *__restrict__ residual, uint32_t *__restrict__ n_dev) {
+	__shared__ uint32_t s_part[4], s_wave[4];
+	const int j = blockIdx.x * blockDim.x + threadIdx.x;
+	const int lane = threadIdx.x & 63, wv = threadIdx.x >> 6;
+	uint32_t front = 0;
+	for (int b = threadIdx.x; b < (int) blockIdx.x; b += 256) front += wg_undecided[b];
+#pragma unroll
+	for (int d = 1; d < 64; d <<= 1) front += __shfl_xor(front, d);
+	const bool und = j < n && undecided[j] != 0u;
+	const unsigned long long mu = __ballot(und);
+	if (lane == 0) { s_part[wv] = front; s_wave[wv] = (uint32_t) __popcll(mu); }
+	__syncthreads();
+	uint32_t at = s_part[0] + s_part[1] + s_part[2] + s_part[3];
+	for (int w2 = 0; w2 < wv; ++w2) at += s_wave[w2];
+	at += (uint32_t) __popcll(mu & ((1ull << lane) - 1ull));
+	if (und) {
+		residual[at] = (uint32_t) j;
+		if (a_read) { r_read[at] = a_read[j]; r_loc[at] = a_loc[j]; r_sv[at] = a_sv[j]; }
+	}
+	if (blockIdx.x == gridDim.x - 1 && threadIdx.x == 0) *n_dev = s_part[0] + s_part[1] + s_part[2] + s_part[3] + s_wave[0] + s_wave[1] + s_wave[2] + s_wave[3];
+}
+
+static __global__ __launch_bounds__(256) void affine_residual_rows_kernel(const uint32_t *__restrict__ n_dev, const uint32_t *__restrict__ residual,
+		const uint8_t *__restrict__ ref, int rl, const uint8_t *__restrict__ qry, int q, uint8_t *__restrict__ r_ref, uint8_t *__restrict__ r_qry) {
+	const uint32_t k = blockIdx.x;
+	if (k >= *n_dev) return;
+	const uint32_t j = residual[k];
+	for (int t = threadIdx.x; t < rl; t += 256) r_ref[(size_t) k * rl + t] = ref[(size_t) j * rl + t];
+	for (int t = threadIdx.x; t < q; t += 256) r_qry[(size_t) k * q + t] = qry[(size_t) j * q + t];
+}
+
+}
diff --git a/nextgenmap_amd/csrc/engine_internal.h b/nextgenmap_amd/csrc/engine_internal.h
--- a/nextgenmap_amd/csrc/engine_internal.h
+++ b/nextgenmap_amd/csrc/engine_internal.h
@@ -82,12 +82,14 @@
 
 namespace ngm {
 int engine_reserve(ngm_hip_ctx *ctx, int n);
-int engine_score_packed(ngm_hip_ctx *ctx, int mode, int n, float *d_scores, hipStream_t st);
+int engine_score_packed(ngm_hip_ctx *ctx, int mode, int n, float *d_scores, hipStream_t st, uint32_t *d_endcell = nullptr);
+bool engine_score_endcell_available(const ngm_hip_ctx *ctx, int mode);
 struct AlignFinish {
 	CigarDevOut *out;
 	char *bytes;
 	unsigned long long capacity;
 	unsigned long long *counters;
+	const uint32_t *n_dev = nullptr, *residual = nullptr;
 };
 int engine_align_packed(ngm_hip_ctx *ctx, int mode, int n, int32_t *d_records, uint16_t *d_runs, int run_stride, hipStream_t st, const AlignFinish *fin = nullptr);
 int engine_affine_traceback_packed(ngm_hip_ctx *ctx, int n, int32_t *d_records, uint16_t *d_runs, int run_stride, hipStream_t st);
diff --git a/nextgenmap_amd/csrc/gather_device.h b/nextgenmap_amd/csrc/gather_device.h
--- a/nextgenmap_amd/csrc/gather_device.h
+++ b/nextgenmap_amd/csrc/gather_device.h
@@ -42,10 +42,11 @@
 __global__ __launch_bounds__(256) void gather_pairs_kernel(const uint8_t *__restrict__ reads, const uint16_t *__restrict__ read_len,
 		int q, const uint32_t *__restrict__ genome, WindowGeom G, const uint32_t *__restrict__ pair_read,
 		const uint32_t *__restrict__ pair_loc, const uint32_t *__restrict__ pair_sv, int n_pairs, int RW, int FW,
-		uint32_t *__restrict__ out, uint16_t *__restrict__ lens, uint16_t *__restrict__ blk_rows, int alt_dir = 0) {
+		uint32_t *__restrict__ out, uint16_t *__restrict__ lens, uint16_t *__restrict__ blk_rows, int alt_dir = 0, const uint32_t *__restrict__ n_dev = nullptr) {
 	__shared__ int s_rows;
 	const int tid = threadIdx.x;
 	const int blk = blockIdx.x;
+	if (n_dev) { n_pairs = min(n_pairs, (int) *n_dev); if (blk * kSlots >= n_pairs) return; }
 	const int slot = tid & 63, part = tid >> 6;
 	const int pair = blk * kSlots + slot;
 	if (tid == 0) s_rows = 0;
diff --git a/nextgenmap_amd/csrc/mapper.cpp b/nextgenmap_amd/csrc/mapper.cpp
--- a/nextgenmap_amd/csrc/mapper.cpp
+++ b/nextgenmap_amd/csrc/mapper.cpp
@@ -61,7 +61,7 @@
 }
 
 namespace ngm {
-int score_candidates(ngm_mapper *m, int n, uint64_t np, int alt_dir) {
+int score_candidates(ngm_mapper *m, int n, uint64_t np, int alt_dir, bool want_endcell) {
 	const ngm_ref *r = m->ref;
 	ngm_hip_ctx *eng = m->eng;
 	const int q = m->prm.qry_max_len, c = m->prm.corridor;
@@ -72,7 +72,9 @@
 			m->d_pair_read.p, m->d_out_loc.p, m->d_out_sv.p, (int) np, eng->RW, eng->FW, eng->packed.p, eng->lens.p, eng->blk_rows.p, alt_dir);
 	MAP_HIP_TRY(hipGetLastError());
 	MAP_HIP_TRY(hipEventRecord(m->ev[2], m->st));
-	if (int rc = ngm::engine_score_packed(eng, m->prm.mode, (int) np, m->d_scores.p, m->st)) { ngm::pipeline_set_error("%s", ngm_hip_last_error(eng)); return rc; }
+	const long factor = std::max<long>(0, test_limit("ungapped_max_cand_per_read", (long) kUngappedMaxCandidatesPerRead));
+	m->endcell_valid = want_endcell && np <= (uint64_t) factor * (uint64_t) n && m->d_endcell.cap >= np && ngm::engine_score_endcell_available(eng, m->prm.mode);
+	if (int rc = ngm::engine_score_packed(eng, m->prm.mode, (int) np, m->d_scores.p, m->st, m->endcell_valid ? m->d_endcell.p : nullptr)) { ngm::pipeline_set_error("%s", ngm_hip_last_error(eng)); return rc; }
 	MAP_HIP_TRY(hipEventRecord(m->ev[3], m->st));
 	return 0;
 }
@@ -144,6 +146,8 @@
 	for (auto &e : m->cev) (void) hipEventCreate(&e);
 	for (auto &e : m->oev) (void) hipEventCreate(&e);
 	if (const char *e = getenv("NGM_HIP_CS_EAGER_ARRAYS")) m->cs_eager_arrays = atoi(e) != 0;
+	if (const char *e = getenv("NGM_HIP_ALIGN_UNGAPPED")) m->ungapped_on = atoi(e) != 0;
+	if (getenv("NGM_HIP_ALIGN_TAIL_SPLIT") || getenv("NGM_HIP_HOST_CIGAR")) m->ungapped_on = false;
 	if (ngm::cs_configure(m, p) != 0) { ngm_mapper_destroy(m); return nullptr; }
 	return m;
 }
@@ -162,6 +166,7 @@
 	m->d_reads.release(); m->d_scores.release(); m->d_best.release(); m->d_pair_read.release();
 	m->d_winner.release(); m->d_a_read.release(); m->d_a_loc.release(); m->d_a_sv.release(); m->d_mapq.release(); m->d_nbest.release();
 	m->d_records.release(); m->d_runs.release(); m->d_runs_c.release();
+	m->d_endcell.release(); m->d_a_pair.release(); m->d_ung.release(); m->p_residual.release();
 	m->d_pair_info.release(); m->p_pair_info.release(); m->d_sam_contig_start.release();
 	m->d_pair_out.release(); m->d_pair_top.release(); m->d_pair_tied_n.release(); m->d_pair_list.release(); m->p_pair_out.release(); m->p_pair_top.release(); m->p_pair_tied_n.release();
 	m->d_sam_contig_names.release(); m->d_sam_rg.release(); m->d_sam_names.release(); m->d_sam_text.release(); m->d_sam_contig_off.release(); m->d_sam_len.release(); m->d_sam_off.release();
@@ -623,12 +628,17 @@
 	}
 	if (m->p_winner.reserve(n) || m->p_mapq.reserve(n) || m->p_nbest.reserve(n) || m->p_best.reserve(n)) { ngm::pipeline_set_error("out of pinned host memory"); return -12; }
 	if (m->d_winner.reserve(n) || m->d_mapq.reserve(n) || m->d_nbest.reserve(n) || m->d_best.reserve(n)) { ngm::pipeline_set_error("out of device memory (score stage)"); return -12; }
+	const bool want_endcell = m->ungapped_on && m->prm.personality == NGM_PERSONALITY_AFFINE && (paired || m->prm.topn <= 1) && !alt_cigar &&
+			ngm::engine_score_endcell_available(eng, m->prm.mode);
+	m->endcell_valid = false;
+	m->ung_dbg[0] = m->ung_dbg[1] = 0;
 	uint64_t regrown = 0;
 	auto reserve_for_candidates = [&](uint64_t cnt, bool device, bool count) -> int {
 		auto grow = [&](auto &buf, size_t want) { if (count && buf.cap < want) ++regrown; return buf.reserve(want); };
 		if (grow(m->p_loc, cnt + 1) || grow(m->p_sv, cnt + 1) || (paired && grow(m->p_scores, cnt + 1))) { ngm::pipeline_set_error("out of pinned host memory"); return -12; }
 		if (!device) return 0;
 		if (grow(m->d_pair_read, cnt) || grow(m->d_scores, cnt)) { ngm::pipeline_set_error("out of device memory (score stage)"); return -12; }
+		if (want_endcell && grow(m->d_endcell, cnt)) { ngm::pipeline_set_error("out of device memory (score stage)"); return -12; }
 		const size_t had = eng->packed.cap + eng->lens.cap + eng->blk_rows.cap;
 		if (int rc = ngm::engine_reserve(eng, (int) cnt)) { ngm::pipeline_set_error("%s", ngm_hip_last_error(eng)); return rc; }
 		if (count && eng->packed.cap + eng->lens.cap + eng->blk_rows.cap != had) ++regrown;
@@ -681,7 +691,7 @@
 	if (np == 0) { if (int rc = cs_host_arrays(m)) return rc; for (int i = 0; i < n; ++i) { h_winner[i] = 0xFFFFFFFFu; h_mapq[i] = 0; h_nbest[i] = 0; h_best[i] = 0.f; } }
 	if (np > 0) {
 		stage_cs.acquire();
-		if (int rc = ngm::score_candidates(m, n, np, alt_dir)) return rc;
+		if (int rc = ngm::score_candidates(m, n, np, alt_dir, want_endcell)) return rc;
 		hipLaunchKernelGGL(ngm::select_top1_kernel, dim3((n + 255) / 256), dim3(256), 0, m->st, n, m->d_cand_base.p, m->d_cand_count.p,
 				m->d_scores.p, m->d_out_loc.p, m->d_out_sv.p, m->d_winner.p, m->d_mapq.p, m->d_nbest.p, m->d_best.p);
 		MAP_HIP_TRY(hipGetLastError());
@@ -1062,6 +1072,7 @@
 	if (m->p_rec.reserve((size_t) na * 8 + 8)) { ngm::pipeline_set_error("out of pinned host memory"); return -12; }
 	int32_t *h_rec = m->p_rec.p;
 	uint16_t *h_runs = nullptr;
+	std::vector<int> rec_of;
 	const int align_buf_len = (q + c) | 2;
 	static const bool dev_strings = !getenv("NGM_HIP_HOST_CIGAR");
 	uint64_t str_base = 0;
@@ -1079,10 +1090,29 @@
 		const unsigned long long scap = (unsigned long long) na * 96ull + 4096ull;
 		if (dev_strings && (m->d_cigout.reserve(na) || m->d_str.reserve(scap) || m->p_cigout.reserve(na))) { ngm::pipeline_set_error("out of memory (CIGAR strings)"); return -12; }
 		if (finish) MAP_HIP_TRY(hipMemsetAsync(m->d_total.p + 8, 0, 16, m->st));
+		const bool ungapped = finish && m->endcell_valid && (mode & NGM_MODE_ALIGN_MASK) == NGM_MODE_LOCAL;
+		const int nwg = (na + 255) / 256;
+		uint32_t *u_undecided = nullptr, *u_residual = nullptr, *u_read = nullptr, *u_loc = nullptr, *u_sv = nullptr, *u_wg = nullptr, *u_ndev = nullptr;
+		if (ungapped) {
+			if (m->d_a_pair.reserve(na) || m->d_ung.reserve((size_t) 5 * na + nwg)) { ngm::pipeline_set_error("out of device memory (align stage)"); return -12; }
+			MAP_HIP_TRY(hipMemcpyAsync(m->d_a_pair.p, a_pair.data(), (size_t) na * 4, hipMemcpyHostToDevice, m->st));
+			u_undecided = m->d_ung.p; u_residual = u_undecided + na; u_read = u_residual + na; u_loc = u_read + na; u_sv = u_loc + na; u_wg = u_sv + na;
+			u_ndev = (uint32_t *) (m->d_total.p + 10);
+		}
 		MAP_HIP_TRY(hipStreamSynchronize(m->st));
 		stage_align.acquire();
 		MAP_HIP_TRY(hipEventRecord(m->ev[5], m->st));
 		ngm::WindowGeom Ga{r->n_bases - 1, align_buf_len, c >> 1};
+		if (ungapped) {
+			const int h_safe = std::min(align_buf_len, ((q + c) | 1) + 1) - 2;
+			hipLaunchKernelGGL(ngm::affine_ungapped_kernel, dim3(nwg), dim3(256), 0, m->st, na, (const uint32_t *) m->d_a_pair.p, (const float *) m->d_scores.p,
+					(const uint32_t *) m->d_endcell.p, (const uint32_t *) eng->packed.p, (const uint16_t *) eng->lens.p, eng->RW, eng->FW, c, h_safe, m->prm.match_bonus,
+					m->prm.mismatch_penalty, m->d_cigout.p, m->d_str.p, scap, (unsigned long long *) (m->d_total.p + 8), u_undecided, u_wg);
+			hipLaunchKernelGGL(ngm::affine_residual_collect_kernel, dim3(nwg), dim3(256), 0, m->st, na, (const uint32_t *) u_undecided, (const uint32_t *) u_wg,
+					(const uint32_t *) m->d_a_read.p, (const uint32_t *) m->d_a_loc.p, (const uint32_t *) m->d_a_sv.p, u_read, u_loc, u_sv, u_residual, u_ndev);
+			hipLaunchKernelGGL(ngm::gather_pairs_kernel, dim3((na + ngm::kSlots - 1) / ngm::kSlots), dim3(256), 0, m->st, m->d_reads.p, m->d_read_len.p, q,
+					r->d_genome, Ga, u_read, u_loc, u_sv, na, eng->RW, eng->FW, eng->packed.p, eng->lens.p, eng->blk_rows.p, alt_dir, (const uint32_t *) u_ndev);
+		} else
 		hipLaunchKernelGGL(ngm::gather_pairs_kernel, dim3((na + ngm::kSlots - 1) / ngm::kSlots), dim3(256), 0, m->st, m->d_reads.p, m->d_read_len.p, q,
 				r->d_genome, Ga, m->d_a_read.p, m->d_a_loc.p, m->d_a_sv.p, na, eng->RW, eng->FW, eng->packed.p, eng->lens.p, eng->blk_rows.p, alt_dir);
 		MAP_HIP_TRY(hipGetLastError());
@@ -1090,17 +1120,20 @@
 		const bool was_prof = eng->profiling;
 		unsigned long long n_runs_total = 0, n_str_total = 0;
 		if (finish) {
-			unsigned long long ctr[2] = {0, 0};
-			const ngm::AlignFinish fin{m->d_cigout.p, m->d_str.p, scap, m->d_total.p + 8};
+			unsigned long long ctr[3] = {0, 0, 0};
+			ngm::AlignFinish fin{m->d_cigout.p, m->d_str.p, scap, m->d_total.p + 8};
+			if (ungapped) { fin.n_dev = u_ndev; fin.residual = u_residual; }
 			eng->profiling = true;
 			if (int rc = ngm::engine_align_packed(eng, mode, na, m->d_records.p, m->d_runs.p, rs, m->st, &fin)) { eng->profiling = was_prof; ngm::pipeline_set_error("%s", ngm_hip_last_error(eng)); return rc; }
 			eng->profiling = was_prof;
 			MAP_HIP_TRY(hipEventRecord(m->ev[7], m->st));
 			MAP_HIP_TRY(hipEventRecord(m->ev[8], m->st));
 			MAP_HIP_TRY(hipMemcpyAsync(m->p_cigout.p, m->d_cigout.p, (size_t) na * sizeof(ngm::CigarDevOut), hipMemcpyDeviceToHost, m->st));
-			MAP_HIP_TRY(hipMemcpyAsync(ctr, m->d_total.p + 8, 16, hipMemcpyDeviceToHost, m->st));
+			MAP_HIP_TRY(hipMemcpyAsync(ctr, m->d_total.p + 8, ungapped ? 24 : 16, hipMemcpyDeviceToHost, m->st));
 			stage_align.done_after(m->ev[8]);
 			MAP_HIP_TRY(hipStreamSynchronize(m->st));
+			const int n_dp = ungapped ? (int) std::min<unsigned long long>(ctr[2] & 0xFFFFFFFFull, (unsigned long long) na) : na;
+			if (ungapped) { m->ung_dbg[0] = (uint64_t) (na - n_dp); m->ung_dbg[1] = (uint64_t) n_dp; }
 			n_str_total = std::min<unsigned long long>(ctr[0], scap);
 			str_base = n_str_total;
 			if (m->p_str.reserve(n_str_total + 1)) { ngm::pipeline_set_error("out of pinned host memory"); return -12; }
@@ -1108,13 +1141,18 @@
 			if (ctr[1]) {
 				if (m->d_runs_c.reserve((size_t) na * rs)) { ngm::pipeline_set_error("out of device memory (runs)"); return -12; }
 				MAP_HIP_TRY(hipMemsetAsync(m->d_total.p, 0, 8, m->st));
-				if (int rc = ngm::engine_affine_traceback_packed(eng, na, m->d_records.p, m->d_runs.p, rs, m->st)) { ngm::pipeline_set_error("%s", ngm_hip_last_error(eng)); return rc; }
-				hipLaunchKernelGGL(ngm::compact_runs_kernel, dim3((na + 255) / 256), dim3(256), 0, m->st, na, m->d_records.p, m->d_runs.p, rs,
+				if (int rc = ngm::engine_affine_traceback_packed(eng, n_dp, m->d_records.p, m->d_runs.p, rs, m->st)) { ngm::pipeline_set_error("%s", ngm_hip_last_error(eng)); return rc; }
+				hipLaunchKernelGGL(ngm::compact_runs_kernel, dim3((n_dp + 255) / 256), dim3(256), 0, m->st, n_dp, m->d_records.p, m->d_runs.p, rs,
 						m->d_runs_c.p, m->d_total.p);
 				MAP_HIP_TRY(hipGetLastError());
-				MAP_HIP_TRY(hipMemcpyAsync(h_rec, m->d_records.p, (size_t) na * 8 * 4, hipMemcpyDeviceToHost, m->st));
+				MAP_HIP_TRY(hipMemcpyAsync(h_rec, m->d_records.p, (size_t) n_dp * 8 * 4, hipMemcpyDeviceToHost, m->st));
 				MAP_HIP_TRY(hipMemcpyAsync(&n_runs_total, m->d_total.p, 8, hipMemcpyDeviceToHost, m->st));
+				if (ungapped) {
+					if (m->p_residual.reserve((size_t) n_dp + 1)) { ngm::pipeline_set_error("out of pinned host memory"); return -12; }
+					MAP_HIP_TRY(hipMemcpyAsync(m->p_residual.p, u_residual, (size_t) n_dp * 4, hipMemcpyDeviceToHost, m->st));
+				}
 				MAP_HIP_TRY(hipStreamSynchronize(m->st));
+				if (ungapped) { rec_of.assign((size_t) na, -1); for (int k = 0; k < n_dp; ++k) rec_of[m->p_residual.p[k]] = k; }
 				if (m->p_runs.reserve(n_runs_total + 1)) { ngm::pipeline_set_error("out of pinned host memory"); return -12; }
 				h_runs = m->p_runs.p;
 				MAP_HIP_TRY(hipMemcpy(h_runs, m->d_runs_c.p, n_runs_total * 2, hipMemcpyDeviceToHost));
@@ -1207,7 +1245,8 @@
 				ao.identity = dv->identity; ao.nm = dv->nm; ao.qstart = dv->qstart; ao.qend = dv->qend; ao.position_offset = dv->position_offset;
 				ao.score_token = dv->score_token;
 			} else if (m->prm.personality == NGM_PERSONALITY_AFFINE) {
-				ngm::build_cigar_affine(&h_rec[(size_t) j * 8], &h_runs[(size_t) (uint32_t) h_rec[(size_t) j * 8 + 6]], nullptr, nullptr, q, &ao, read_length());
+				const size_t jr = rec_of.empty() ? (size_t) j : (size_t) rec_of[j];
+				ngm::build_cigar_affine(&h_rec[jr * 8], &h_runs[(size_t) (uint32_t) h_rec[jr * 8 + 6]], nullptr, nullptr, q, &ao, read_length());
 				memcpy(ao.md, "!!!", 4);
 			} else {
 				const uint64_t offset = (uint64_t) a_loc[j] - (uint64_t) (c >> 1);
@@ -1665,6 +1704,12 @@
 	return 0;
 }
 
+int ngm_mapper_align_ungapped_counters(ngm_mapper *m, uint64_t out[2]) {
+	if (!m || !out) return -22;
+	out[0] = m->ung_dbg[0]; out[1] = m->ung_dbg[1];
+	return 0;
+}
+
 int ngm_mapper_search_turn_counters(ngm_mapper *m, uint64_t out[3]) {
 	if (!m || !out) return -22;
 	out[0] = m->turn_dbg[0]; out[1] = m->turn_dbg[1]; out[2] = m->turn_dbg[2];
diff --git a/nextgenmap_amd/csrc/mapper_internal.h b/nextgenmap_amd/csrc/mapper_internal.h
--- a/nextgenmap_amd/csrc/mapper_internal.h
+++ b/nextgenmap_amd/csrc/mapper_internal.h
@@ -173,6 +173,11 @@
 	size_t canon_lds = 0;
 	uint64_t np_seen_max = 0;
 	uint64_t turn_dbg[3] = {0, 0, 0};
+	bool ungapped_on = true;
+	bool endcell_valid = false;
+	ngm::DevBuf<uint32_t> d_endcell, d_a_pair, d_ung;
+	ngm::PinnedBuf<uint32_t> p_residual;
+	uint64_t ung_dbg[2] = {0, 0};
 	hipEvent_t ev[10] = {};
 	float ms[8] = {};
 };
@@ -227,7 +232,8 @@
 void cs_release(ngm_mapper *m);
 long test_limit(const char *key, long dflt);
 
-int score_candidates(ngm_mapper *m, int n, uint64_t np, int alt_dir);
+constexpr uint64_t kUngappedMaxCandidatesPerRead = 4;
+int score_candidates(ngm_mapper *m, int n, uint64_t np, int alt_dir, bool want_endcell = false);
 void argos_release(ngm_mapper *m);
 
 }
diff --git a/nextgenmap_amd/csrc/ngm_hip.cpp b/nextgenmap_amd/csrc/ngm_hip.cpp
--- a/nextgenmap_amd/csrc/ngm_hip.cpp
+++ b/nextgenmap_amd/csrc/ngm_hip.cpp
@@ -83,6 +83,20 @@
 	return nullptr;
 }
 
+template <int CP> const void *pk_affine_score_endcell_ptr() {
+	if constexpr (CP <= 32) return (const void *) ngm::sw_affine_score_pk_kernel<CP, false, true>; else return nullptr;
+}
+const void *find_pk_affine_score_endcell_kernel(int c) {
+#define X(C) if (c == C) return pk_affine_score_endcell_ptr<C + 1>();
+	NGM_CORRIDORS(X)
+#undef X
+	return nullptr;
+}
+
+bool affine_fits_16bit(const ngm_hip_ctx *ctx) {
+	return (long) ctx->q * ctx->KA.tM < 30000 && ctx->prm.gap_read_penalty + (long) ctx->q * (ctx->prm.gap_extend_penalty + ctx->KA.tZ) < 19000;
+}
+
 const void *find_pk_affine_score_split_kernel(int c) {
 	if (c == 80) return (const void *) ngm::sw_affine_score_pk_split_kernel<81>;
 	return nullptr;
@@ -138,9 +152,24 @@
 	return 0;
 }
 
-int engine_score_packed(ngm_hip_ctx *ctx, int mode, int n, float *d_scores, hipStream_t st) {
+bool engine_score_endcell_available(const ngm_hip_ctx *ctx, int mode) {
+	static const bool force32 = getenv("NGM_HIP_SCORE_32BIT") != nullptr || getenv("NGM_HIP_ALIGN_32BIT") != nullptr;
+	if (force32 || ctx->prm.personality != NGM_PERSONALITY_AFFINE || (mode & NGM_MODE_ALIGN_MASK) == NGM_MODE_END_TO_END) return false;
+	if (!(ctx->KA.open < 0 && ctx->KA.ext < 0 && affine_fits_16bit(ctx))) return false;
+	if (!((long) ctx->q * ctx->prm.match_bonus < 2048 && ctx->c + 1 <= 32)) return false;
+	return find_pk_affine_score_endcell_kernel(ctx->c) != nullptr && find_pk_affine_align_kernel(ctx->c, false) != nullptr;
+}
+
+int engine_score_packed(ngm_hip_ctx *ctx, int mode, int n, float *d_scores, hipStream_t st, uint32_t *d_endcell) {
 	const int nb = n_blocks_of(n);
 	static const bool force32 = getenv("NGM_HIP_SCORE_32BIT") != nullptr;
+	if (d_endcell) {
+		if (!engine_score_endcell_available(ctx, mode)) { set_error(ctx, "no score kernel with the end cell for this engine"); return -22; }
+		KernelRef kp; kp.aot = find_pk_affine_score_endcell_kernel(ctx->c);
+		HIP_TRY(ctx, launch_kernel(kp, dim3((nb + 7) / 8), dim3(256), st, (const uint32_t *) ctx->packed.p, (const uint16_t *) ctx->lens.p,
+				(const uint16_t *) ctx->blk_rows.p, d_scores, n, nb, ctx->RW, ctx->KA, d_endcell));
+		return 0;
+	}
 	if (ctx->prm.personality == NGM_PERSONALITY_AFFINE) {
 		const bool ef = (mode & NGM_MODE_ALIGN_MASK) == NGM_MODE_END_TO_END;
 		if (!force32 && (long) ctx->q * ctx->KA.tM < 30000 && ctx->prm.gap_read_penalty + (long) ctx->q * (ctx->prm.gap_extend_penalty + ctx->KA.tZ) < 19000) {
@@ -154,7 +183,7 @@
 			if (const void *pk = find_pk_affine_score_kernel(ctx->c, ef)) {
 				KernelRef kp; kp.aot = pk;
 				HIP_TRY(ctx, launch_kernel(kp, dim3((nb + 7) / 8), dim3(256), st, (const uint32_t *) ctx->packed.p, (const uint16_t *) ctx->lens.p,
-						(const uint16_t *) ctx->blk_rows.p, d_scores, n, nb, ctx->RW, ctx->KA));
+						(const uint16_t *) ctx->blk_rows.p, d_scores, n, nb, ctx->RW, ctx->KA, (uint32_t *) nullptr));
 				return 0;
 			}
 		}
@@ -193,6 +222,7 @@
 		if (ctx->dirs.reserve((size_t) nb * ctx->q * ADW * ngm::kSlots)) { set_error(ctx, "out of device memory for the trace matrix"); return -12; }
 		static const bool force32 = getenv("NGM_HIP_ALIGN_32BIT") != nullptr;
 		const void *pk = nullptr;
+		const uint32_t *n_dev = fin ? fin->n_dev : nullptr, *residual = fin ? fin->residual : nullptr;
 		if (!force32 && am != NGM_MODE_END_TO_END && ctx->KA.open < 0 && ctx->KA.ext < 0 && (long) ctx->q * ctx->KA.tM < 30000 &&
 				ctx->prm.gap_read_penalty + (long) ctx->q * (ctx->prm.gap_extend_penalty + ctx->KA.tZ) < 19000) {
 			const bool plain_key = (long) ctx->q * ctx->prm.match_bonus < 2048 && ctx->c + 1 <= 32;
@@ -202,8 +232,9 @@
 		if (pk) {
 			KernelRef kp; kp.aot = pk;
 			HIP_TRY(ctx, launch_kernel(kp, dim3((nb + 7) / 8), dim3(256), st, (const uint32_t *) ctx->packed.p, (const uint16_t *) ctx->lens.p,
-					(const uint16_t *) ctx->blk_rows.p, ctx->dirs.p, d_records, n, nb, ctx->RW, ctx->q, ctx->KA));
+					(const uint16_t *) ctx->blk_rows.p, ctx->dirs.p, d_records, n, nb, ctx->RW, ctx->q, ctx->KA, n_dev));
 		} else {
+			if (n_dev) { set_error(ctx, "a device-side pair count needs the packed align kernel"); return -22; }
 			const KernelRef ka = find_kernel(ctx, 6 + (am == NGM_MODE_END_TO_END ? 1 : 0));
 			HIP_TRY(ctx, launch_kernel(ka, dim3((nb + 3) / 4), dim3(256), st, (const uint32_t *) ctx->packed.p, (const uint16_t *) ctx->lens.p,
 					(const uint16_t *) ctx->blk_rows.p, (float *) nullptr, ctx->dirs.p, d_records, n, nb, ctx->RW, ctx->q, ctx->KA));
@@ -212,7 +243,7 @@
 		ctx->trace_nibbles = pk != nullptr;
 		if (!fin) return engine_affine_traceback_packed(ctx, n, d_records, d_runs, run_stride, st);
 		if (pk) hipLaunchKernelGGL(ngm::affine_finish_kernel<true>, dim3((n + 255) / 256), dim3(256), 0, st, n, (const uint32_t *) ctx->dirs.p, (const int32_t *) d_records,
-				(const uint32_t *) ctx->packed.p, (const uint16_t *) ctx->lens.p, ctx->q, CP, ctx->RW, ctx->FW, fin->out, fin->bytes, fin->capacity, fin->counters);
+				(const uint32_t *) ctx->packed.p, (const uint16_t *) ctx->lens.p, ctx->q, CP, ctx->RW, ctx->FW, fin->out, fin->bytes, fin->capacity, fin->counters, n_dev, residual);
 		else hipLaunchKernelGGL(ngm::affine_finish_kernel<false>, dim3((n + 255) / 256), dim3(256), 0, st, n, (const uint32_t *) ctx->dirs.p, (const int32_t *) d_records,
 				(const uint32_t *) ctx->packed.p, (const uint16_t *) ctx->lens.p, ctx->q, CP, ctx->RW, ctx->FW, fin->out, fin->bytes, fin->capacity, fin->counters);
 		HIP_TRY(ctx, hipGetLastError());
@@ -561,4 +592,148 @@
 	return n;
 }
 
-}
+int ngm_debug_align_ungapped(void *engine, int mode, int n, const char *const *ref, const char *const *qry, void *out_records, uint64_t *n_fallback, uint64_t *n_ungapped) {
+	ngm_hip_ctx *ctx = (ngm_hip_ctx *) engine;
+	ngm_hip_align_out *out = (ngm_hip_align_out *) out_records;
+	if (!ctx || !out || !n_fallback || !n_ungapped) return -22;
+	*n_fallback = 0; *n_ungapped = 0;
+	if (n <= 0) return 0;
+	if (!ngm::engine_score_endcell_available(ctx, mode)) { set_error(ctx, "ngm_debug_align_ungapped: affine personality, local mode, plain row key only"); return -22; }
+	ScopedDevice sd(ctx->device);
+	const size_t rl = ctx->rl, q = ctx->q;
+	const int rs = ngm::run_stride(ctx->q, ctx->c);
+	if (ctx->h_ref.reserve((size_t) n * rl) || ctx->h_qry.reserve((size_t) n * q) || ctx->d_ref.reserve((size_t) n * rl) ||
+			ctx->d_qry.reserve((size_t) n * q) || ctx->d_records.reserve((size_t) n * 8) || ctx->d_runs.reserve((size_t) n * rs) ||
+			ctx->h_records.reserve((size_t) n * 8) || ctx->h_runs.reserve((size_t) n * rs) || ctx->d_scores.reserve(n)) {
+		set_error(ctx, "out of memory staging %d pairs", n);
+		return -12;
+	}
+	for (int i = 0; i < n; ++i) {
+		memcpy(ctx->h_ref.p + (size_t) i * rl, ref[i], rl);
+		memcpy(ctx->h_qry.p + (size_t) i * q, qry[i], q);
+	}
+	const unsigned long long scap = (unsigned long long) n * ngm::kCigarRow + 4096ull;
+	const int nwg = (n + 255) / 256;
+	ngm::DevBuf<ngm::CigarDevOut> d_out;
+	ngm::DevBuf<char> d_str;
+	ngm::DevBuf<unsigned long long> d_ctr;
+	ngm::DevBuf<uint32_t> d_end, d_ung;
+	ngm::DevBuf<uint8_t> r_ref, r_qry;
+	std::vector<ngm::CigarDevOut> h_out((size_t) n);
+	std::vector<char> h_str((size_t) scap);
+	std::vector<uint32_t> h_res;
+	unsigned long long ctr[3] = {0, 0, 0};
+	auto run = [&]() -> int {
+		if (d_out.reserve(n) || d_str.reserve(scap) || d_ctr.reserve(4) || d_end.reserve(n) || d_ung.reserve((size_t) 2 * n + nwg) || r_ref.reserve((size_t) n * rl) ||
+				r_qry.reserve((size_t) n * q)) { set_error(ctx, "out of device memory (ngm_debug_align_ungapped)"); return -12; }
+		uint32_t *undecided = d_ung.p, *residual = d_ung.p + n, *wg = d_ung.p + 2 * (size_t) n, *n_dev = (uint32_t *) (d_ctr.p + 2);
+		hipStream_t st = ctx->stream;
+		HIP_TRY(ctx, hipMemcpyAsync(ctx->d_ref.p, ctx->h_ref.p, (size_t) n * rl, hipMemcpyHostToDevice, st));
+		HIP_TRY(ctx, hipMemcpyAsync(ctx->d_qry.p, ctx->h_qry.p, (size_t) n * q, hipMemcpyHostToDevice, st));
+		HIP_TRY(ctx, hipMemsetAsync(d_ctr.p, 0, 32, st));
+		HIP_TRY(ctx, hipMemsetAsync(r_ref.p, 0, (size_t) n * rl, st));
+		HIP_TRY(ctx, hipMemsetAsync(r_qry.p, 0, (size_t) n * q, st));
+		if (int r = engine_reserve(ctx, n)) return r;
+		if (int r = launch_pack(ctx, n, ctx->d_ref.p, ctx->d_qry.p, st)) return r;
+		if (int r = ngm::engine_score_packed(ctx, mode, n, ctx->d_scores.p, st, d_end.p)) return r;
+		hipLaunchKernelGGL(ngm::affine_ungapped_kernel, dim3(nwg), dim3(256), 0, st, n, (const uint32_t *) nullptr, (const float *) ctx->d_scores.p, (const uint32_t *) d_end.p,
+				(const uint32_t *) ctx->packed.p, (const uint16_t *) ctx->lens.p, ctx->RW, ctx->FW, ctx->c, 1 << 30, ctx->prm.match_bonus, ctx->prm.mismatch_penalty,
+				d_out.p, d_str.p, scap, d_ctr.p, undecided, wg);
+		hipLaunchKernelGGL(ngm::affine_residual_collect_kernel, dim3(nwg), dim3(256), 0, st, n, (const uint32_t *) undecided, (const uint32_t *) wg, (const uint32_t *) nullptr,
+				(const uint32_t *) nullptr, (const uint32_t *) nullptr, (uint32_t *) nullptr, (uint32_t *) nullptr, (uint32_t *) nullptr, residual, n_dev);
+		hipLaunchKernelGGL(ngm::affine_residual_rows_kernel, dim3(n), dim3(256), 0, st, (const uint32_t *) n_dev, (const uint32_t *) residual, (const uint8_t *) ctx->d_ref.p, (int) rl,
+				(const uint8_t *) ctx->d_qry.p, (int) q, r_ref.p, r_qry.p);
+		HIP_TRY(ctx, hipGetLastError());
+		if (int r = launch_pack(ctx, n, r_ref.p, r_qry.p, st)) return r;
+		ngm::AlignFinish fin{d_out.p, d_str.p, scap, d_ctr.p};
+		fin.n_dev = n_dev; fin.residual = residual;
+		if (int r = ngm::engine_align_packed(ctx, mode, n, ctx->d_records.p, ctx->d_runs.p, rs, st, &fin)) return r;
+		HIP_TRY(ctx, hipMemcpyAsync(h_out.data(), d_out.p, (size_t) n * sizeof(ngm::CigarDevOut), hipMemcpyDeviceToHost, st));
+		HIP_TRY(ctx, hipMemcpyAsync(ctr, d_ctr.p, 24, hipMemcpyDeviceToHost, st));
+		HIP_TRY(ctx, hipStreamSynchronize(st));
+		const unsigned long long used = std::min(ctr[0], scap);
+		if (used) HIP_TRY(ctx, hipMemcpy(h_str.data(), d_str.p, (size_t) used, hipMemcpyDeviceToHost));
+		const int n_res = (int) std::min<unsigned long long>(ctr[2] & 0xFFFFFFFFull, (unsigned long long) n);
+		if (ctr[1] && n_res > 0) {
+			h_res.resize((size_t) n_res);
+			if (int r = ngm::engine_affine_traceback_packed(ctx, n_res, ctx->d_records.p, ctx->d_runs.p, rs, st)) return r;
+			HIP_TRY(ctx, hipMemcpyAsync(ctx->h_records.p, ctx->d_records.p, sizeof(int32_t) * 8 * (size_t) n_res, hipMemcpyDeviceToHost, st));
+			HIP_TRY(ctx, hipMemcpyAsync(ctx->h_runs.p, ctx->d_runs.p, sizeof(uint16_t) * (size_t) rs * n_res, hipMemcpyDeviceToHost, st));
+			HIP_TRY(ctx, hipMemcpyAsync(h_res.data(), residual, (size_t) n_res * 4, hipMemcpyDeviceToHost, st));
+			HIP_TRY(ctx, hipStreamSynchronize(st));
+		}
+		*n_ungapped = (uint64_t) (n - n_res);
+		return 0;
+	};
+	const int rc = run();
+	d_out.release(); d_str.release(); d_ctr.release(); d_end.release(); d_ung.release(); r_ref.release(); r_qry.release();
+	if (rc) return rc;
+	*n_fallback = ctr[1];
+	std::vector<int> k_of(h_res.empty() ? 0 : (size_t) n, -1);
+	for (size_t k = 0; k < h_res.size(); ++k) k_of[h_res[k]] = (int) k;
+	for (int i = 0; i < n; ++i) {
+		const ngm::CigarDevOut &dv = h_out[(size_t) i];
+		if (!(dv.flags & 1)) {
+			const int k = k_of.empty() ? -1 : k_of[(size_t) i];
+			if (k < 0) { set_error(ctx, "ngm_debug_align_ungapped: pair %d has neither strings nor a place in the residual", i); return -5; }
+			ngm::build_cigar_affine(ctx->h_records.p + (size_t) k * 8, ctx->h_runs.p + (size_t) k * rs, ref[i], qry[i], ctx->q, &out[i]);
+			continue;
+		}
+		memcpy(out[i].cigar, h_str.data() + dv.cig_off, dv.cig_len); out[i].cigar[dv.cig_len] = 0;
+		memcpy(out[i].md, h_str.data() + dv.md_off, dv.md_len); out[i].md[dv.md_len] = 0;
+		out[i].position_offset = dv.position_offset; out[i].qstart = dv.qstart; out[i].qend = dv.qend;
+		out[i].score_token = dv.score_token; out[i].identity = dv.identity; out[i].nm = dv.nm;
+	}
+	return n;
+}
+
+int ngm_debug_score_endcell(void *engine, int mode, int n, const char *const *ref, const char *const *qry, int32_t *out6) {
+	ngm_hip_ctx *ctx = (ngm_hip_ctx *) engine;
+	if (!ctx || !out6) return -22;
+	if (n <= 0) return 0;
+	if (!ngm::engine_score_endcell_available(ctx, mode)) { set_error(ctx, "ngm_debug_score_endcell: affine personality, local mode, plain row key only"); return -22; }
+	ScopedDevice sd(ctx->device);
+	const size_t rl = ctx->rl, q = ctx->q;
+	const int rs = ngm::run_stride(ctx->q, ctx->c);
+	if (ctx->h_ref.reserve((size_t) n * rl) || ctx->h_qry.reserve((size_t) n * q) || ctx->d_ref.reserve((size_t) n * rl) || ctx->d_qry.reserve((size_t) n * q) ||
+			ctx->d_records.reserve((size_t) n * 8) || ctx->d_runs.reserve((size_t) n * rs) || ctx->h_records.reserve((size_t) n * 8) || ctx->d_scores.reserve(n) ||
+			ctx->h_scores.reserve(n)) { set_error(ctx, "out of memory staging %d pairs", n); return -12; }
+	for (int i = 0; i < n; ++i) {
+		memcpy(ctx->h_ref.p + (size_t) i * rl, ref[i], rl);
+		memcpy(ctx->h_qry.p + (size_t) i * q, qry[i], q);
+	}
+	const unsigned long long scap = (unsigned long long) n * ngm::kCigarRow + 4096ull;
+	ngm::DevBuf<ngm::CigarDevOut> d_out;
+	ngm::DevBuf<char> d_str;
+	ngm::DevBuf<unsigned long long> d_ctr;
+	ngm::DevBuf<uint32_t> d_end;
+	std::vector<uint32_t> h_end((size_t) n);
+	auto run = [&]() -> int {
+		if (d_out.reserve(n) || d_str.reserve(scap) || d_ctr.reserve(2) || d_end.reserve(n)) { set_error(ctx, "out of device memory (ngm_debug_score_endcell)"); return -12; }
+		hipStream_t st = ctx->stream;
+		HIP_TRY(ctx, hipMemcpyAsync(ctx->d_ref.p, ctx->h_ref.p, (size_t) n * rl, hipMemcpyHostToDevice, st));
+		HIP_TRY(ctx, hipMemcpyAsync(ctx->d_qry.p, ctx->h_qry.p, (size_t) n * q, hipMemcpyHostToDevice, st));
+		HIP_TRY(ctx, hipMemsetAsync(d_ctr.p, 0, 16, st));
+		if (int r = engine_reserve(ctx, n)) return r;
+		if (int r = launch_pack(ctx, n, ctx->d_ref.p, ctx->d_qry.p, st)) return r;
+		if (int r = ngm::engine_score_packed(ctx, mode, n, ctx->d_scores.p, st, d_end.p)) return r;
+		const ngm::AlignFinish fin{d_out.p, d_str.p, scap, d_ctr.p};
+		if (int r = ngm::engine_align_packed(ctx, mode, n, ctx->d_records.p, ctx->d_runs.p, rs, st, &fin)) return r;
+		HIP_TRY(ctx, hipMemcpyAsync(ctx->h_records.p, ctx->d_records.p, sizeof(int32_t) * 8 * (size_t) n, hipMemcpyDeviceToHost, st));
+		HIP_TRY(ctx, hipMemcpyAsync(ctx->h_scores.p, ctx->d_scores.p, sizeof(float) * (size_t) n, hipMemcpyDeviceToHost, st));
+		HIP_TRY(ctx, hipMemcpyAsync(h_end.data(), d_end.p, (size_t) n * 4, hipMemcpyDeviceToHost, st));
+		HIP_TRY(ctx, hipStreamSynchronize(st));
+		return 0;
+	};
+	const int rc = run();
+	d_out.release(); d_str.release(); d_ctr.release(); d_end.release();
+	if (rc) return rc;
+	for (int i = 0; i < n; ++i) {
+		int32_t *o = out6 + (size_t) i * 6;
+		o[0] = (int32_t) ctx->h_scores.p[i]; o[1] = (int32_t) (h_end[(size_t) i] >> 16); o[2] = (int32_t) (h_end[(size_t) i] & 0xFFFFu);
+		o[3] = ctx->h_records.p[(size_t) i * 8 + 5]; o[4] = ctx->h_records.p[(size_t) i * 8 + 6]; o[5] = ctx->h_records.p[(size_t) i * 8 + 7];
+	}
+	return n;
+}
+
+}
diff --git a/nextgenmap_amd/csrc/sw_device.h b/nextgenmap_amd/csrc/sw_device.h
--- a/nextgenmap_amd/csrc/sw_device.h
+++ b/nextgenmap_amd/csrc/sw_device.h
@@ -280,6 +280,12 @@
 	asm("v_pk_mad_u16 %0, %1, %2, %3" : "=v"(r) : "v"(a), "v"(b), "s"(kk));
 	return r;
 }
+__device__ __forceinline__ v2s pk_mad32_k(v2s a, int k) {
+	v2s r;
+	const uint32_t kk = ((uint32_t) k & 0xFFFFu) * 0x10001u;
+	asm("v_pk_mad_u16 %0, %1, 32, %2 op_sel_hi:[1,0,1]" : "=v"(r) : "v"(a), "s"(kk));
+	return r;
+}
 __device__ __forceinline__ v2s pk_min1_op(v2s a) {
 	v2s r;
 	asm("v_pk_min_i16 %0, %1, 1 op_sel_hi:[1,0]" : "=v"(r) : "v"(a));
diff --git a/nextgenmap_amd/engine.py b/nextgenmap_amd/engine.py
--- a/nextgenmap_amd/engine.py
+++ b/nextgenmap_amd/engine.py
@@ -67,6 +67,8 @@
     lib.ngm_hip_last_kernel_ms.argtypes = [C.c_void_p, C.POINTER(C.c_float)]
     lib.ngm_hip_set_profiling.argtypes = [C.c_void_p, C.c_int]
     lib.ngm_debug_align_finish.argtypes = [C.c_void_p, C.c_int, C.c_int, C.c_void_p, C.c_void_p, C.c_void_p, C.POINTER(C.c_uint64)]
+    lib.ngm_debug_align_ungapped.argtypes = [C.c_void_p, C.c_int, C.c_int, C.c_void_p, C.c_void_p, C.c_void_p, C.POINTER(C.c_uint64), C.POINTER(C.c_uint64)]
+    lib.ngm_debug_score_endcell.argtypes = [C.c_void_p, C.c_int, C.c_int, C.c_void_p, C.c_void_p, C.c_void_p]
     _lib = lib
     return lib
 
@@ -132,7 +134,7 @@
         assert r == n
         return out
 
-    def BatchAlign(self, mode, ref, qry, dirs=None, finish=False):
+    def BatchAlign(self, mode, ref, qry, dirs=None, finish=False, ungapped=False):
         n, ref, qry, rp, qp = self._ptr_lists(ref, qry)
         stride = 4 * max(1, self.q)
         cig = np.zeros((n, stride), dtype=np.uint8)
@@ -144,7 +146,11 @@
             outs[i].cigar = cig.ctypes.data + i * stride
             outs[i].md = md.ctypes.data + i * stride
         d = None if dirs is None else np.ascontiguousarray(dirs, dtype=np.uint8)
-        if finish:
+        if finish and ungapped:
+            fb, ug = C.c_uint64(0), C.c_uint64(0)
+            r = self._check(self.lib.ngm_debug_align_ungapped(self.h, mode, n, rp, qp, outs, C.byref(fb), C.byref(ug)), n)
+            self.last_fallback, self.last_ungapped = int(fb.value), int(ug.value)
+        elif finish:
             fb = C.c_uint64(0)
             r = self._check(self.lib.ngm_debug_align_finish(self.h, mode, n, rp, qp, outs, C.byref(fb)), n)
             self.last_fallback = int(fb.value)
@@ -158,6 +164,13 @@
                             position_offset=o.position_offset, qstart=o.qstart, qend=o.qend,
                             score_token=o.score_token, identity=o.identity, nm=o.nm))
         return res
+
+    def ScoreEndCell(self, mode, ref, qry):
+        n, ref, qry, rp, qp = self._ptr_lists(ref, qry)
+        out = np.zeros((n, 6), dtype=np.int32)
+        r = self._check(self.lib.ngm_debug_score_endcell(self.h, mode, n, rp, qp, out.ctypes.data), n)
+        assert r == n
+        return out
 
     def set_profiling(self, on):
         self.lib.ngm_hip_set_profiling(self.h, 1 if on else 0)
diff --git a/nextgenmap_amd/pipeline.py b/nextgenmap_amd/pipeline.py
--- a/nextgenmap_amd/pipeline.py
+++ b/nextgenmap_amd/pipeline.py
@@ -91,6 +91,7 @@
         lib.ngm_mapper_order_table_reads.argtypes = [C.c_void_p, C.c_void_p]
         lib.ngm_mapper_heavy_counters.argtypes = [C.c_void_p, C.c_void_p]
         lib.ngm_mapper_search_turn_counters.argtypes = [C.c_void_p, C.c_void_p]
+        lib.ngm_mapper_align_ungapped_counters.argtypes = [C.c_void_p, C.c_void_p]
         lib.ngm_mapper_last_kernel_ms.argtypes = [C.c_void_p, C.POINTER(C.c_float)]
         lib.ngm_mapper_last_order_replay_ms.restype = C.c_float
         lib.ngm_mapper_last_order_replay_ms.argtypes = [C.c_void_p]
@@ -658,6 +659,11 @@
         self.lib.ngm_mapper_heavy_counters(self.h, out.ctypes.data)
         return dict(zip(("second_passes", "table_pass_restarts", "sent_on", "pool_regrown"), (int(x) for x in out)))
 
+    def align_ungapped_counters(self):
+        out = np.zeros(2, np.uint64)
+        self.lib.ngm_mapper_align_ungapped_counters(self.h, out.ctypes.data)
+        return dict(zip(("ungapped", "residual"), (int(x) for x in out)))
+
     def search_turn_counters(self):
         out = np.zeros(3, np.uint64)
         self.lib.ngm_mapper_search_turn_counters(self.h, out.ctypes.data)
```

Result: slower. 57.39 million (-4.2%).
